# daxiongpro/EPNet

Hardware: AMD Instinct MI355X
Metric: SA-stack points/sec per GPU (16384-pt KITTI scene) + % HBM roofline (higher is better)
Workload: dtype f32; 1 GPU; 256 x 16384-pt kitti scenes per GPU per step through the 4-level SA op stack (4 samplings [FPS + centre gather; levels 2-4 nested in level 1 where tie-free] + 8 ball_query + 8 fused groupings [xyz - centre ; features]), pyramid 16384>4096>1024>256>64, radii [[.1,.5],[.5,1],[1,2],[2,4]], nsample [16,32], C=0/96/256/512, HIP-graph launch; levels=4, scenes_per_gpu=256, software_pipelined=True, pipeline_stages=2, parallelism=scene-parallel x1

## Files before the change

epnet_amd/_lib.py:

```python
import contextlib
import ctypes
import os

_HERE = os.path.dirname(os.path.abspath(__file__))
LIB_PATH = os.environ.get("EPNET_HIP_LIB") or os.path.join(_HERE, "lib", "libepnet_hip.so")

_vp = ctypes.c_void_p
_i = ctypes.c_int
_f = ctypes.c_float
_d = ctypes.c_double
_sz = ctypes.c_size_t
_i64 = ctypes.c_int64

SIGNATURES = {
    "epnet_abi_version": (_i, []),
    "epnet_strerror": (ctypes.c_char_p, [_i]),
    "epnet_last_hip_error": (ctypes.c_char_p, []),
    "epnet_set_tuning": (_i, [ctypes.c_char_p, _i]),
    "epnet_get_tuning": (_i, [ctypes.c_char_p, ctypes.POINTER(_i)]),
    "epnet_furthest_point_sampling": (_i, [_i, _i, _i, _vp, _vp, _vp, _vp]),
    "epnet_gather_points": (_i, [_i, _i, _i, _i, _vp, _vp, _vp, _vp]),
    "epnet_gather_points_grad": (_i, [_i, _i, _i, _i, _vp, _vp, _vp, _vp]),
    "epnet_ball_query": (_i, [_i, _i, _i, _f, _i, _vp, _vp, _vp, _vp]),
    "epnet_ball_query_workspace_bytes": (_sz, [_i, _i, _i]),
    "epnet_ball_query_ws": (_i, [_i, _i, _i, _f, _i, _vp, _vp, _vp, _vp, _sz, _vp]),
    "epnet_group_points": (_i, [_i, _i, _i, _i, _i, _vp, _vp, _vp, _vp]),
    "epnet_group_points_grad": (_i, [_i, _i, _i, _i, _i, _vp, _vp, _vp, _vp]),
    "epnet_group_concat": (_i, [_i, _i, _i, _i, _i, _vp, _vp, _vp, _vp, _vp, _i, _vp]),
    "epnet_group_concat_workspace_bytes": (_sz, [_i, _i, _i, _i, _i]),
    "epnet_group_concat_ws": (_i, [_i, _i, _i, _i, _i, _vp, _vp, _vp, _vp, _vp, _i, _vp, _sz, _vp]),
    "epnet_group_concat_grad": (_i, [_i, _i, _i, _i, _i, _vp, _vp, _vp, _i, _vp]),
    "epnet_group_points_grad_workspace_bytes": (_sz, [_i, _i, _i, _i]),
    "epnet_group_points_grad_ws": (_i, [_i, _i, _i, _i, _i, _vp, _vp, _vp, _vp, _sz, _vp]),
    "epnet_group_concat_grad_ws": (_i, [_i, _i, _i, _i, _i, _vp, _vp, _vp, _i, _vp, _sz, _vp]),
    "epnet_three_nn": (_i, [_i, _i, _i, _vp, _vp, _vp, _vp, _vp]),
    "epnet_three_nn_workspace_bytes": (_sz, [_i, _i, _i]),
    "epnet_three_nn_ws": (_i, [_i, _i, _i, _vp, _vp, _vp, _vp, _vp, _sz, _vp]),
    "epnet_three_interpolate": (_i, [_i, _i, _i, _i, _vp, _vp, _vp, _vp, _vp]),
    "epnet_three_interpolate_grad": (_i, [_i, _i, _i, _i, _vp, _vp, _vp, _vp, _vp]),
    "epnet_three_interpolate_grad_workspace_bytes": (_sz, [_i, _i, _i]),
    "epnet_three_interpolate_grad_ws": (_i, [_i, _i, _i, _i, _vp, _vp, _vp, _vp, _vp, _sz, _vp]),
    "epnet_group_linear": (_i, [_i, _i, _i, _i, _i, _vp, _vp, _vp, _vp, _vp, _vp, _vp, _vp]),
    "epnet_group_linear_grad_w": (_i, [_i, _i, _i, _i, _i, _vp, _vp, _vp, _vp, _vp, _vp]),
    "epnet_feature_gather": (_i, [_i, _i, _i, _i, _i, _i, _i, _vp, _vp, _vp, _vp, _vp, _vp]),
    "epnet_feature_gather_grad": (_i, [_i, _i, _i, _i, _i, _i, _vp, _vp, _vp, _vp]),
    "epnet_gather_points_grad_det_workspace_bytes": (_sz, [_i, _i, _i]),
    "epnet_gather_points_grad_det": (_i, [_i, _i, _i, _i, _vp, _vp, _vp, _vp, _sz, _vp]),
    "epnet_group_points_grad_det_workspace_bytes": (_sz, [_i, _i, _i, _i]),
    "epnet_group_points_grad_det": (_i, [_i, _i, _i, _i, _i, _vp, _vp, _vp, _vp, _sz, _vp]),
    "epnet_group_concat_grad_det_workspace_bytes": (_sz, [_i, _i, _i, _i]),
    "epnet_group_concat_grad_det": (_i, [_i, _i, _i, _i, _i, _vp, _vp, _vp, _i, _vp, _sz, _vp]),
    "epnet_three_interpolate_grad_det_workspace_bytes": (_sz, [_i, _i, _i]),
    "epnet_three_interpolate_grad_det": (_i, [_i, _i, _i, _i, _vp, _vp, _vp, _vp, _vp, _sz, _vp]),
    "epnet_feature_gather_grad_det_workspace_bytes": (_sz, [_i, _i, _i, _i]),
    "epnet_feature_gather_grad_det": (_i, [_i, _i, _i, _i, _i, _i, _vp, _vp, _vp, _vp, _sz, _vp]),
    "epnet_group_linear_grad_w_det_workspace_bytes": (_sz, [_i, _i, _i, _i]),
    "epnet_group_linear_grad_w_det": (_i, [_i, _i, _i, _i, _i, _vp, _vp, _vp, _vp, _vp, _vp, _sz, _vp]),
    "epnet_pool_max": (_i, [ctypes.c_longlong, _i, _vp, _vp, _vp, _vp]),
    "epnet_pool_max_grad": (_i, [ctypes.c_longlong, _i, _vp, _vp, _vp, _vp]),
    "epnet_group_linear_h": (_i, [_i, _i, _i, _i, _i, _vp, _vp, _vp, _vp, _vp, _vp, _vp, _i, _vp]),
    "epnet_pool_max_h": (_i, [ctypes.c_longlong, _i, _vp, _vp, _vp, _i, _vp]),
    "epnet_pool_max_grad_h": (_i, [ctypes.c_longlong, _i, _vp, _vp, _vp, _i, _vp]),
    "epnet_three_interpolate_h": (_i, [_i, _i, _i, _i, _vp, _vp, _vp, _vp, _i, _vp]),
    "epnet_scene_index_bytes": (_sz, [_i, _i]),
    "epnet_scene_index_build": (_i, [_i, _i, _vp, _vp, _sz, _vp]),
    "epnet_scene_index_build_gathered": (_i, [_i, _i, _i, _vp, _vp, _vp, _vp, _sz, _vp]),
    "epnet_furthest_point_sampling_indexed": (_i, [_i, _i, _i, _vp, _vp, _sz, _vp, _vp, _vp]),
    "epnet_sample_centres": (_i, [_i, _i, _i, _vp, _vp, _sz, _vp, _vp, _vp, _vp]),
    "epnet_sample_centres_chain": (_i, [_i, _i, _i, _vp, _vp, _sz, _vp, _vp, _vp, _vp, _vp, _i, _vp]),
    "epnet_group_concat_multi": (_i, [_i, _i, _i, _i, _i, _vp, _vp, _vp, _vp, _vp, _vp, _i, _vp]),
    "epnet_ball_query_indexed_multi": (_i, [_i, _i, _i, _i, _vp, _vp, _vp, _vp, _vp, _sz, _vp, _vp]),
    "epnet_ball_query_ordered": (_i, [_i, _i, _i, _i, _vp, _vp, _vp, _vp, _vp, _sz, _vp, _sz, _vp, _vp]),
    "epnet_three_nn_indexed": (_i, [_i, _i, _i, _vp, _vp, _vp, _sz, _vp, _sz, _vp, _vp, _vp]),
    "epnet_ball_query_indexed": (_i, [_i, _i, _i, _f, _i, _vp, _vp, _vp, _sz, _vp, _vp]),
    "epnet_boxes_overlap_bev": (_i, [_i, _vp, _i, _vp, _vp, _vp]),
    "epnet_boxes_iou_bev": (_i, [_i, _vp, _i, _vp, _vp, _vp]),
    "epnet_boxes_iou3d": (_i, [_i, _vp, _i, _vp, _vp, _vp]),
    "epnet_boxes_iou3d_pairs": (_i, [_i, _vp, _vp, _vp, _vp]),
    "epnet_aug_roi_by_noise": (_i, [_i, _i, _f, _vp, _vp, _vp, _vp, _vp, _vp, _vp, _vp]),
    "epnet_rcnn_sample_rois_workspace_bytes": (_sz, [_i, _i, _i, _i]),
    "epnet_rcnn_sample_rois": (_i, [_i, _i, _i, _i, _i, _i, _f, _f, _f, _d, _i, _vp, _vp, _vp, _vp, _vp, _vp, _vp, _sz, _vp, _vp, _vp,
                                    _vp, _vp, _vp, _vp, _vp, _vp, _vp]),
    "epnet_rpn_proposals_workspace_bytes": (_sz, [_i, _i, _i, _i]),
    "epnet_rpn_proposals": (_i, [_i, _i, _vp, _vp, _vp, _i, _i, _i, _f, _i, _vp, _sz, _vp, _vp, _vp, _vp]),
    "epnet_decode_bbox_target": (_i, [ctypes.c_longlong, _i, _vp, _vp, _i, _i, _i, _d, _d, _d, _d, _i, _vp, _i, _i, _i, _i, _i, _i, _vp, _vp]),
    "epnet_score_order": (_i, [_i, _i, _vp, _vp, _vp]),
    "epnet_rpn_handover_workspace_bytes": (_sz, [_i, _i, _i, _i, _i]),
    "epnet_rpn_handover": (_i, [_i, _i, _i, _vp, _vp, _vp, _i, _i, _d, _d, _d, _d, _i, _vp, _i, _i, _i, _i, _i, _f, _i, _i, _i, _f, _i, _vp,
                                _sz, _vp, _vp, _vp, _vp, _vp, _vp, _vp, _vp]),
    "epnet_rcnn_detections_workspace_bytes": (_sz, [_i, _i]),
    "epnet_rcnn_detections": (_i, [_i, _i, _vp, _vp, _vp, _f, _f, _vp, _sz, _vp, _vp, _vp, _vp]),
    "epnet_eval_recall_workspace_bytes": (_sz, [_i, _i, _i]),
    "epnet_eval_recall": (_i, [_i, _i, _i, _i, _i, _i, _vp, _vp, _vp, _vp, _vp, _vp, _vp, _sz, _vp, _vp, _vp, _vp, _vp, _vp, _vp]),
    "epnet_kitti_records": (_i, [_i, _i, _vp, _vp, _vp, _vp, _vp, _vp, _vp, _vp, _vp, _vp]),
    "epnet_nms_workspace_bytes": (_sz, [_i]),
    "epnet_nms": (_i, [_vp, _i, _f, _vp, _sz, _vp, _vp, _vp]),
    "epnet_nms_normal": (_i, [_vp, _i, _f, _vp, _sz, _vp, _vp, _vp]),
    "epnet_roipool3d_workspace_bytes": (_sz, [_i, _i, _i]),
    "epnet_roipool3d": (_i, [_i, _i, _i, _i, _i, _vp, _vp, _vp, _vp, _vp, _vp, _sz, _vp]),
    "epnet_roipool3d_canonical": (_i, [_i, _i, _i, _i, _i, _f, _vp, _vp, _vp, _vp, _vp, _vp]),
    "epnet_roipool3d_train": (_i, [_i, _i, _i, _i, _i, _f, _f, _f, _f, _vp, _vp, _vp, _vp, _vp, _vp, _vp, _vp, _vp, _vp, _vp, _vp, _vp,
                                   _vp, _vp]),
    "epnet_box_loss_workspace_bytes": (_sz, [ctypes.c_longlong, _i]),
    "epnet_box_loss": (_i, [ctypes.c_longlong, _i, _d, _d, _i, _i, _i, _i, _d, _d, _d, _d, _d, _d, _d, _vp, _vp, _vp, _vp, _vp, _vp, _vp,
                            _vp, _vp, _vp, _vp, _vp, _sz, _vp]),
    "epnet_adam_onecycle_workspace_bytes": (_sz, [ctypes.c_longlong]),
    "epnet_adam_onecycle_step": (_i, [_i, ctypes.c_longlong, ctypes.c_longlong, _vp, _vp, _vp, ctypes.c_longlong, _d, _d, _d, _i, _vp, _vp,
                                      _vp, _vp, _vp, _sz, _vp]),
    "epnet_rpn_targets": (_i, [_i, _i, _i, _f, _vp, _vp, _vp, _vp, _vp, _vp, _vp, _vp, _vp]),
    "epnet_scan_prepare_workspace_bytes": (_sz, [_i, _i, _i]),
    "epnet_scan_prepare": (_i, [_i, _i, _i, _i, _vp, _f, _vp, _vp, _vp, _vp, _vp, _vp, _vp, _vp, _vp, _sz, _vp, _vp, _vp, _vp, _vp, _vp, _vp]),
    "epnet_image_normalise": (_i, [_i, _i, _i, _i, _i, _vp, _vp, _vp, _vp, _vp, _vp]),
    "epnet_kitti_overlaps": (_i, [_i, _i, _i, _i, _i, _vp, _vp, _vp, _vp, _vp, _vp, _vp]),
    "epnet_kitti_match": (_i, [_i, _i, _i, _i, _i, _i, _i, _vp, _vp, _vp, _vp, _vp, _vp, _vp, _vp, _vp, _vp, _vp]),
    "epnet_kitti_pr_workspace_bytes": (_sz, [_i, _i, _i]),
    "epnet_kitti_pr": (_i, [_i, _i, _i, _i, _i, _i, _i, _i, _i, _i, _i, _vp, _vp, _vp, _vp, _vp, _vp, _vp, _vp, _vp, _vp, _vp, _vp,
                            _vp, _vp, _vp, _vp, _vp, _sz, _vp, _vp, _vp]),
    "epnet_kitti_thresholds_host": (_i, [_vp, _i64, _i64, _i, _vp, _i, ctypes.POINTER(_i)]),
    "epnet_pts_in_boxes3d_host": (_i, [_vp, _vp, _vp, _i64, _i64]),
    "epnet_roipool3d_host": (_i, [_vp, _vp, _vp, _vp, _vp, _vp, _i64, _i64, _i64, _i64]),
}

_lib = None


class EpnetError(RuntimeError):
    pass


def lib():
    global _lib
    if _lib is None:
        if not os.path.exists(LIB_PATH):
            raise RuntimeError(
                "epnet_amd: %s not found -- build it with `python -c 'import __graft_entry__ as g; g.build()'` "
                "or `make -C epnet_amd/csrc` (there is no CPU fallback)" % LIB_PATH)
        handle = ctypes.CDLL(LIB_PATH)
        for name, (res, args) in SIGNATURES.items():
            try:
                fn = getattr(handle, name)
            except AttributeError:
                raise RuntimeError("epnet_amd: %s does not export %s (stale build?)" % (LIB_PATH, name))
            fn.restype = res
            fn.argtypes = args
        if handle.epnet_abi_version() != 1:
            raise RuntimeError("epnet_amd: ABI version mismatch in %s" % LIB_PATH)
        _lib = handle
    return _lib


def check(code, what):
    if code != 0:
        l = lib()
        msg = l.epnet_strerror(code).decode()
        hip = l.epnet_last_hip_error().decode()
        raise EpnetError("%s failed: %s%s" % (what, msg, (" [" + hip + "]") if (code == -2 and hip) else ""))


@contextlib.contextmanager
def tuning(**overrides):
    l = lib()
    saved = []
    try:
        for name, value in overrides.items():
            old = _i()
            check(l.epnet_get_tuning(name.encode(), ctypes.byref(old)), "epnet_get_tuning(%s)" % name)
            check(l.epnet_set_tuning(name.encode(), int(value)), "epnet_set_tuning(%s, %r)" % (name, value))
            saved.append((name, old.value))
        yield
    finally:
        for name, old in reversed(saved):
            l.epnet_set_tuning(name.encode(), old)
```

epnet_amd/csrc/ball_query.hip:

```cpp

#include "common.h"
#include "dpp.h"
#include "spatial.h"

namespace epnet {

constexpr int kBqTile = 2048;
constexpr int kBqThreads = 256;

template <int CPW>
__global__ __launch_bounds__(kBqThreads) void ball_query_kernel(int n, int m, float radius2, int nsample,
                                                                const float *__restrict__ new_xyz,
                                                                const float *__restrict__ xyz,
                                                                int *__restrict__ idx) {
    __shared__ float tile[kBqTile * 3];
    const int lane = threadIdx.x & 63, wave = threadIdx.x >> 6;
    const int bs = blockIdx.y;
    xyz += (size_t)bs * n * 3;
    new_xyz += (size_t)bs * m * 3;
    idx += (size_t)bs * m * nsample;

    const int c0 = (blockIdx.x * (kBqThreads / 64) + wave) * CPW;
    float cx[CPW], cy[CPW], cz[CPW];
    int cnt[CPW], first[CPW];
#pragma unroll
    for (int i = 0; i < CPW; ++i) {
        const int ci = c0 + i;
        const bool ok = ci < m;
        cx[i] = ok ? new_xyz[ci * 3 + 0] : 0.f;
        cy[i] = ok ? new_xyz[ci * 3 + 1] : 0.f;
        cz[i] = ok ? new_xyz[ci * 3 + 2] : 0.f;
        cnt[i] = ok ? 0 : nsample;
        first[i] = 0;
    }

    for (int t0 = 0; t0 < n; t0 += kBqTile) {
        const int tn = min(kBqTile, n - t0);
        for (int e = threadIdx.x; e < tn * 3; e += kBqThreads) tile[e] = xyz[(size_t)t0 * 3 + e];
        __syncthreads();

        bool wave_done = true;
#pragma unroll
        for (int i = 0; i < CPW; ++i) wave_done = wave_done && (cnt[i] >= nsample);

        if (!wave_done) {
            for (int p0 = 0; p0 < tn; p0 += 64) {
                const int p = p0 + lane;
                const bool valid = p < tn;
                const float x = valid ? tile[p * 3 + 0] : 0.f;
                const float y = valid ? tile[p * 3 + 1] : 0.f;
                const float z = valid ? tile[p * 3 + 2] : 0.f;
                bool all_full = true;
#pragma unroll
                for (int i = 0; i < CPW; ++i) {
                    if (cnt[i] < nsample) {
                        const float dx = cx[i] - x, dy = cy[i] - y, dz = cz[i] - z;
                        const float d2 = dx * dx + dy * dy + dz * dz;
                        const bool hit = valid && (d2 < radius2);
                        const unsigned long long mask = __ballot(hit);
                        if (mask) {
                            const int pos = cnt[i] + popc_below(mask);
                            if (hit && pos < nsample) idx[(size_t)(c0 + i) * nsample + pos] = t0 + p;
                            if (cnt[i] == 0) first[i] = t0 + p0 + (int)__builtin_ctzll(mask);
                            cnt[i] += (int)__popcll(mask);
                        }
                        all_full = all_full && (cnt[i] >= nsample);
                    }
                }
                if (all_full) {
                    wave_done = true;
                    break;
                }
            }
        }
        if (__syncthreads_and(wave_done ? 1 : 0)) break;
    }

#pragma unroll
    for (int i = 0; i < CPW; ++i) {
        const int ci = c0 + i;
        if (ci < m && cnt[i] < nsample) {
            const int fill = cnt[i] > 0 ? first[i] : 0;
            for (int l = cnt[i] + lane; l < nsample; l += 64) idx[(size_t)ci * nsample + l] = fill;
        }
    }
}



#ifdef EPNET_BQ_STATS
__device__ unsigned long long g_bq_stats[16];
#endif
#ifdef EPNET_IX_STATS
__device__ unsigned long long g_ix_stats[8];
#define EPNET_IX_STAMP(var) const unsigned long long var = __builtin_amdgcn_s_memtime()
#else
#define EPNET_IX_STAMP(var)
#endif

template <int kIxThreads, int BITS>
__global__ __launch_bounds__(kIxThreads) void bq_index_kernel(int n, int np, const float *__restrict__ xyz,
                                                              float4 *__restrict__ sorted, float *__restrict__ boxes,
                                                              float *__restrict__ qboxes, int n_src = 0,
                                                              const int *__restrict__ src_idx = nullptr,
                                                              float *__restrict__ gathered = nullptr) {
    constexpr int kCells = 1 << BITS;
    extern __shared__ int s_hist[];
    __shared__ float s_box[6][16];
    __shared__ int s_part[16];
    const int q = threadIdx.x, lane = q & 63, wave = q >> 6;
    __builtin_amdgcn_s_setprio(3);
    xyz += (size_t)blockIdx.x * (src_idx ? n_src : n) * 3;
    if (src_idx) {
        src_idx += (size_t)blockIdx.x * n;
        gathered += (size_t)blockIdx.x * n * 3;
    }
    sorted += (size_t)blockIdx.x * np;
    boxes += (size_t)blockIdx.x * (np / 64) * 6;
    constexpr int per = kCells / kIxThreads;
    constexpr int per_shift = per == 16 ? 4 : per == 8 ? 3 : per == 4 ? 2 : -1;
    static_assert(per_shift > 0, "scan layout");
    constexpr int kIxPerThread = 16;
    const bool in_regs = n <= kIxThreads * kIxPerThread;
    float px[kIxPerThread], py[kIxPerThread], pz[kIxPerThread];
    float lo[3], ext[3];
    EPNET_IX_STAMP(t_0);
    if (in_regs) {
        float mn[3] = {3.4e38f, 3.4e38f, 3.4e38f}, mx[3] = {-3.4e38f, -3.4e38f, -3.4e38f};
        int row[kIxPerThread];
#pragma unroll
        for (int i = 0; i < kIxPerThread; ++i) {
            const int k = q + i * kIxThreads;
            const int kk = k < n ? k : 0;
            row[i] = src_idx ? src_idx[kk] : kk;
        }
#pragma unroll
        for (int i = 0; i < kIxPerThread; ++i) {
            px[i] = xyz[row[i] * 3 + 0];
            py[i] = xyz[row[i] * 3 + 1];
            pz[i] = xyz[row[i] * 3 + 2];
        }
        if (src_idx) {
#pragma unroll
            for (int i = 0; i < kIxPerThread; ++i) {
                const int k = q + i * kIxThreads;
                if (k < n) {
                    gathered[k * 3 + 0] = px[i];
                    gathered[k * 3 + 1] = py[i];
                    gathered[k * 3 + 2] = pz[i];
                }
            }
        }
#pragma unroll
        for (int i = 0; i < kIxPerThread; ++i) {
            const bool ok = q + i * kIxThreads < n;
            mn[0] = fminf(mn[0], ok ? px[i] : 3.4e38f); mx[0] = fmaxf(mx[0], ok ? px[i] : -3.4e38f);
            mn[1] = fminf(mn[1], ok ? py[i] : 3.4e38f); mx[1] = fmaxf(mx[1], ok ? py[i] : -3.4e38f);
            mn[2] = fminf(mn[2], ok ? pz[i] : 3.4e38f); mx[2] = fmaxf(mx[2], ok ? pz[i] : -3.4e38f);
        }
#pragma unroll
        for (int a = 0; a < 3; ++a) {
            const float l = wave_minf_all(mn[a]), h = wave_maxf_all(mx[a]);
            if (lane == 0) {
                s_box[a][wave] = l;
                s_box[3 + a][wave] = h;
            }
        }
        __syncthreads();
#pragma unroll
        for (int a = 0; a < 3; ++a) {
            float l = s_box[a][0], h = s_box[3 + a][0];
            for (int w = 1; w < kIxThreads / 64; ++w) {
                l = fminf(l, s_box[a][w]);
                h = fmaxf(h, s_box[3 + a][w]);
            }
            lo[a] = l;
            ext[a] = h - l;
        }
    } else {
        block_bbox3(xyz, n, s_box, lo, ext);
    }
    const CellGrid g = make_cell_grid(lo, ext, BITS);
    EPNET_IX_STAMP(t_1);
    for (int i = q; i < kCells + kCells / per + 64; i += kIxThreads) s_hist[i] = 0;
    __syncthreads();
    EPNET_IX_STAMP(t_2);
    int code[kIxPerThread], rank[kIxPerThread];
    if (in_regs) {
#pragma unroll
        for (int i = 0; i < kIxPerThread; ++i) code[i] = hist_at((int)cell_code(g, px[i], py[i], pz[i]), per_shift);
#pragma unroll
        for (int i = 0; i < kIxPerThread; ++i)
            rank[i] = atomicAdd(&s_hist[q + i * kIxThreads < n ? code[i] : kCells + kCells / per + lane], 1);
    } else {
        for (int k = q; k < n; k += kIxThreads)
            atomicAdd(&s_hist[hist_at((int)cell_code(g, xyz[k * 3 + 0], xyz[k * 3 + 1], xyz[k * 3 + 2]), per_shift)], 1);
    }
    __syncthreads();
    EPNET_IX_STAMP(t_3);
    int sum = 0;
    for (int i = 0; i < per; ++i) sum += s_hist[hist_at(q * per + i, per_shift)];
    const int incl = wave_inclusive_scan(sum);
    if (lane == 63) s_part[wave] = incl;
    __syncthreads();
    int base = incl - sum;
    for (int w = 0; w < wave; ++w) base += s_part[w];
    for (int i = 0; i < per; ++i) {
        const int at = hist_at(q * per + i, per_shift);
        const int c = s_hist[at];
        s_hist[at] = base;
        base += c;
    }
    __syncthreads();
    EPNET_IX_STAMP(t_4);
    auto bucket_box = [&](int p, const float4 v) {
        const bool real = p < n;
        const float cx_ = canonical(v.x), cy_ = canonical(v.y), cz_ = canonical(v.z);
        float mnx = real ? cx_ : 3.4e38f, mxx = real ? cx_ : -3.4e38f, mny = real ? cy_ : 3.4e38f, mxy = real ? cy_ : -3.4e38f,
              mnz = real ? cz_ : 3.4e38f, mxz = real ? cz_ : -3.4e38f;
        wave_box(mnx, mxx, mny, mxy, mnz, mxz);
        if (lane == 0) {
            float *bx = boxes + (p >> 6) * 6;
            const bool any = mnx <= mxx;
            bx[0] = any ? mnx : 3.0e38f; bx[1] = any ? mxx : 3.0e38f;
            bx[2] = any ? mny : 3.0e38f; bx[3] = any ? mxy : 3.0e38f;
            bx[4] = any ? mnz : 3.0e38f; bx[5] = any ? mxz : 3.0e38f;
        }
    };
    const bool staged = in_regs && (np & 255) == 0;
    if (staged) {
        float4 *s_stage = reinterpret_cast<float4 *>(s_hist + kCells + kCells / per + 64);
        int pos[kIxPerThread];
#pragma unroll
        for (int i = 0; i < kIxPerThread; ++i) pos[i] = s_hist[code[i]] + rank[i];
        const int quarter = kIxThreads == 256 ? min(np >> 2, 512) : np >> 2;
        for (int h = 0; h * quarter < np; ++h) {
            const int base = h * quarter, len = min(quarter, np - base);
            for (int p = q; p < len; p += kIxThreads)
                if (base + p >= n) s_stage[p] = make_float4(3.0e38f, 3.0e38f, 3.0e38f, __int_as_float(-1));
#pragma unroll
            for (int i = 0; i < kIxPerThread; ++i) {
                const int k = q + i * kIxThreads;
                if (k < n && (unsigned)(pos[i] - base) < (unsigned)quarter)
                    s_stage[pos[i] - base] = make_float4(px[i], py[i], pz[i], __int_as_float(k));
            }
            __syncthreads();
            for (int p = q; p < len; p += kIxThreads) {
                const float4 v = s_stage[p];
                sorted[base + p] = v;
                bucket_box(base + p, v);
            }
            __syncthreads();
        }
    } else {
        if (in_regs) {
#pragma unroll
            for (int i = 0; i < kIxPerThread; ++i) {
                const int k = q + i * kIxThreads;
                if (k < n) sorted[s_hist[code[i]] + rank[i]] = make_float4(px[i], py[i], pz[i], __int_as_float(k));
            }
        } else {
            for (int k = q; k < n; k += kIxThreads) {
                const float x = xyz[k * 3 + 0], y = xyz[k * 3 + 1], z = xyz[k * 3 + 2];
                const int pos = atomicAdd(&s_hist[hist_at((int)cell_code(g, x, y, z), per_shift)], 1);
                sorted[pos] = make_float4(x, y, z, __int_as_float(k));
            }
        }
        for (int p = n + q; p < np; p += kIxThreads)
            sorted[p] = make_float4(3.0e38f, 3.0e38f, 3.0e38f, __int_as_float(-1));
        __threadfence_block();
        __syncthreads();
        for (int p = q; p < np; p += kIxThreads) bucket_box(p, sorted[p]);
    }
#ifdef EPNET_IX_STATS
    {
        EPNET_IX_STAMP(t_6);
        if (q == 0) {
            atomicAdd(&g_ix_stats[0], t_1 - t_0); atomicAdd(&g_ix_stats[1], t_2 - t_1); atomicAdd(&g_ix_stats[2], t_3 - t_2);
            atomicAdd(&g_ix_stats[3], t_4 - t_3); atomicAdd(&g_ix_stats[4], t_6 - t_4);
            atomicAdd(&g_ix_stats[7], 1ull);
        }
    }
#endif
    if (!qboxes) return;
    qboxes += (size_t)blockIdx.x * (np / 256) * 6;
    __threadfence_block();
    __syncthreads();
    for (int g = q; g < np / 256; g += kIxThreads) {
        float mn[3] = {3.4e38f, 3.4e38f, 3.4e38f}, mx[3] = {-3.4e38f, -3.4e38f, -3.4e38f};
        for (int k = 0; k < 4; ++k) {
            const float *bx = boxes + (g * 4 + k) * 6;
            if (bx[0] < 3.0e38f)
#pragma unroll
                for (int a = 0; a < 3; ++a) {
                    mn[a] = fminf(mn[a], bx[2 * a]);
                    mx[a] = fmaxf(mx[a], bx[2 * a + 1]);
                }
        }
        const bool any = mn[0] <= mx[0];
#pragma unroll
        for (int a = 0; a < 3; ++a) {
            qboxes[g * 6 + 2 * a] = any ? mn[a] : 3.0e38f;
            qboxes[g * 6 + 2 * a + 1] = any ? mx[a] : 3.0e38f;
        }
    }
}

constexpr int kQThreads = 256;

__device__ __forceinline__ bool box_near(const float *__restrict__ bx, float cx, float cy, float cz, float radius2) {
    const float2 bxx = *reinterpret_cast<const float2 *>(bx), byy = *reinterpret_cast<const float2 *>(bx + 2),
                 bzz = *reinterpret_cast<const float2 *>(bx + 4);
    const float px = __builtin_amdgcn_fmed3f(cx, bxx.x, bxx.y), py = __builtin_amdgcn_fmed3f(cy, byy.x, byy.y),
                pz = __builtin_amdgcn_fmed3f(cz, bzz.x, bzz.y);
    const float dx = cx - px, dy = cy - py, dz = cz - pz;
    return (dx * dx + dy * dy + dz * dz) < radius2;
}


template <int DPL, typename F>
__device__ __forceinline__ void bq_walk(int lane, int np, float r2, float cx, float cy, float cz,
                                        const float4 *__restrict__ sorted, const float *__restrict__ boxes,
                                        const float *__restrict__ qboxes, int *quads, F &&visit) {
    auto scan_buckets = [&](unsigned long long cand, auto &&bucket_of) {
        while (cand) {
            float4 p[4];
            int nb = 0;
#pragma unroll
            for (int k = 0; k < 4; ++k)
                if (cand) {
                    const int bb = bucket_of((int)__builtin_ctzll(cand));
                    cand &= cand - 1ull;
                    p[k] = sorted[(bb << 6) + lane];
                    nb = k + 1;
                }
#pragma unroll
            for (int k = 0; k < 4; ++k)
                if (k < nb) {
                    const float dx = cx - p[k].x, dy = cy - p[k].y, dz = cz - p[k].z;
                    visit(p[k], dx * dx + dy * dy + dz * dz);
                }
        }
    };
    if constexpr (DPL <= 2) {
        const bool bnear = lane < (np >> 6) && box_near(boxes + lane * 6, cx, cy, cz, r2);
        scan_buckets(__ballot(bnear), [](int l) { return l; });
    } else {
        const int nq = np >> 8;
        for (int q0 = 0; q0 < nq; q0 += 64) {
            const int qd = q0 + lane;
            const bool qnear = qd < nq && box_near(qboxes + qd * 6, cx, cy, cz, r2);
            const unsigned long long qmask = __ballot(qnear);
            if (!qmask) continue;
            const int nqc = (int)__popcll(qmask);
            if (qnear) quads[popc_below(qmask)] = qd;
            __builtin_amdgcn_wave_barrier();
            for (int s0 = 0; s0 < nqc; s0 += 16) {
                const int slot = s0 + (lane >> 2);
                int bid = 0;
                bool bnear = false;
                if (slot < nqc) {
                    bid = quads[slot] * 4 + (lane & 3);
                    bnear = box_near(boxes + bid * 6, cx, cy, cz, r2);
                }
                scan_buckets(__ballot(bnear), [&](int l) { return __builtin_amdgcn_readlane(bid, l); });
            }
            __builtin_amdgcn_wave_barrier();
        }
    }
}

__device__ __forceinline__ void bq_emit_list(int lane, const int *hits, int cnt, int nsample, int *__restrict__ out) {
    __builtin_amdgcn_wave_barrier();
    const int mine = lane < cnt ? hits[lane] : 0x7fffffff;
    int rank = 0;
    for (int j = 0; j < cnt; ++j) rank += __builtin_amdgcn_readlane(mine, j) < mine ? 1 : 0;
    if (lane < cnt && rank < nsample) out[rank] = mine;
    int first = 0;
    if (cnt) first = __builtin_amdgcn_readlane(mine, (int)__builtin_ctzll(__ballot(lane < cnt && rank == 0)));
    for (int l = cnt + lane; l < nsample; l += 64) out[l] = first;
}


__device__ __forceinline__ void bq_emit_shared(int lane, const int *hits, int cnt, int ns_big, int ns_small, int *__restrict__ out_big,
                                               int *__restrict__ out_small) {
    __builtin_amdgcn_wave_barrier();
    const bool valid = lane < cnt;
    const int mine = valid ? hits[lane] : 0x7fffffff;
    int rank = 0, rin = 0;
    for (int j = 0; j < cnt; ++j) {
        const int v = __builtin_amdgcn_readlane(mine, j);
        rank += v < mine ? 1 : 0;
        rin += v < mine ? (v & 1) : 0;
    }
    const bool inner = valid && (mine & 1);
    if (valid && rank < ns_big) out_big[rank] = mine >> 1;
    if (inner && rin < ns_small) out_small[rin] = mine >> 1;
    int first = 0;
    if (cnt) first = __builtin_amdgcn_readlane(mine, (int)__builtin_ctzll(__ballot(valid && rank == 0))) >> 1;
    for (int l = cnt + lane; l < ns_big; l += 64) out_big[l] = first;
    const unsigned long long im = __ballot(inner);
    const int cin = (int)__popcll(im);
    first = 0;
    if (cin) first = __builtin_amdgcn_readlane(mine, (int)__builtin_ctzll(__ballot(inner && rin == 0))) >> 1;
    for (int l = cin + lane; l < ns_small; l += 64) out_small[l] = first;
}

template <int NS>
__device__ __forceinline__ void bq_store_rows(int lane, bool two, const int *ord, int c0, int c1, int ns_rt, int *__restrict__ row0,
                                              int *__restrict__ row1) {
    const int ns = NS ? NS : ns_rt;
    if (NS == 16 && lane >= 32) return;
    const int e = NS == 16 ? lane >> 4 : lane >> 5, s = NS == 16 ? lane & 15 : lane & 31;
    const int c = e ? c1 : c0;
    int v = ord[e * 32 + (s < c ? s : 0)];
    v = c ? v : 0;
    if (e == 0) {
        if (s < ns) row0[s] = v;
    } else if (two) {
        if (s < ns) row1[s] = v;
    }
    if (NS == 0 && ns > 32 && (e == 0 || two)) {
        int *row = e ? row1 : row0;
        const int first = c ? ord[e * 32] : 0;
        for (int l = s + 32; l < ns; l += 32) row[l] = first;
    }
}

template <int NSB, int NSS>
__device__ __forceinline__ void bq_emit_pair(int lane, bool two, int *lists, int c0, int c1, int ns_big, int ns_small,
                                             int *__restrict__ big0, int *__restrict__ big1, int *__restrict__ small0,
                                             int *__restrict__ small1) {
    const int half = lane >> 5, sl = lane & 31;
    const int c = half ? c1 : c0;
    int *raw = lists + half * 64;
    const bool valid = sl < c;
    __builtin_amdgcn_wave_barrier();
    int mine = raw[sl];
    if (!valid) {
        mine = 0x7fffffff;
        raw[sl] = mine;
    }
    __builtin_amdgcn_wave_barrier();
    int rank = 0, rin = 0;
    const int nmax = max(c0, c1);
#pragma unroll 1
    for (int j = 0; j < nmax; j += 4) {
        const int4 v = *reinterpret_cast<const int4 *>(raw + j);
        rank += (v.x < mine ? 1 : 0) + (v.y < mine ? 1 : 0) + (v.z < mine ? 1 : 0) + (v.w < mine ? 1 : 0);
        rin += (v.x < mine ? v.x & 1 : 0) + (v.y < mine ? v.y & 1 : 0) + (v.z < mine ? v.z & 1 : 0) + (v.w < mine ? v.w & 1 : 0);
    }
    const bool inner = valid && (mine & 1);
    if (valid) lists[128 + half * 32 + rank] = mine >> 1;
    if (inner) lists[192 + half * 32 + rin] = mine >> 1;
    const unsigned long long im = __ballot(inner);
    __builtin_amdgcn_wave_barrier();
    bq_store_rows<NSB>(lane, two, lists + 128, c0, c1, ns_big, big0, big1);
    bq_store_rows<NSS>(lane, two, lists + 192, (int)__popc((unsigned)im), (int)__popc((unsigned)(im >> 32)), ns_small, small0, small1);
// ... 140 lines not shown
        const int nwg = gx * (int)gridDim.y, orig = (int)blockIdx.y * gx + (int)blockIdx.x;
        const int xcd = orig & 7, qq = nwg >> 3, rr = nwg & 7;
        const int wgid = (xcd < rr ? xcd * (qq + 1) : rr * (qq + 1) + (xcd - rr) * qq) + (orig >> 3);
        bs = wgid >> __builtin_ctz(gx);
        wg_x = wgid & (gx - 1);
        return;
    }
#endif
    xcd_scene_map(wg_x, bs);
    wg_x = __builtin_amdgcn_readfirstlane(wg_x);
    bs = __builtin_amdgcn_readfirstlane(bs);
}

template <int DPL, int K, bool kStream, bool kSpec = false>
__global__ __launch_bounds__(kQThreads) void bq_query2_kernel(int np, int m, BqScales<K> sc,
                                                              const float *__restrict__ new_xyz,
                                                              const float4 *__restrict__ sorted,
                                                              const float *__restrict__ boxes,
                                                              const float *__restrict__ qboxes,
                                                              const float4 *__restrict__ order, int npc) {
    constexpr int kRowsPerStep = 2;
    constexpr int CAP = kStream ? (K == 1 ? 512 : 256) : 64, kStepAppends = kRowsPerStep * 64;
    static_assert(CAP % 64 == 0, "the lists are selected and emitted in whole waves");
    static_assert(!kStream || CAP - kStepAppends >= 64,
                  "a cut list keeps nsample <= 64 entries (the launcher streams for nsample <= 64 only) and must take a step's appends");
    constexpr int kBitWords = kStream ? 0 : 64 * DPL;
    constexpr bool kShared = K == 2 && !kStream;
    static_assert(!kSpec || kShared, "the compile-time pair is one of the shared-list kernel");
    __shared__ __attribute__((aligned(16))) unsigned s_pool[kQThreads / 64][kBitWords + 2 * K * CAP];
    __shared__ int s_quads[kQThreads / 64][2][64];
    const int lane = threadIdx.x & 63, wave = threadIdx.x >> 6;
    int wg_x, bs;
    xcd_scene_map_uniform(wg_x, bs);
    const int ci0 = (wg_x * (kQThreads / 64) + wave) * 2;
    if (ci0 >= m) return;
    const bool two = ci0 + 1 < m;
    sorted += (size_t)bs * np;
    boxes += (size_t)bs * (np / 64) * 6;
    qboxes += (size_t)bs * (np / 256) * 6;
    float ax, ay, az, bx_, by_, bz_;
    int out0 = ci0, out1 = ci0 + 1;
    if (order) {
        const float4 e0 = order[(size_t)bs * npc + ci0], e1 = order[(size_t)bs * npc + ci0 + (two ? 1 : 0)];
        ax = e0.x; ay = e0.y; az = e0.z;
        bx_ = e1.x; by_ = e1.y; bz_ = e1.z;
        out0 = __float_as_int(e0.w);
        out1 = __float_as_int(e1.w);
    } else {
        const float *c0 = new_xyz + ((size_t)bs * m + ci0) * 3;
        const float *c1 = two ? c0 + 3 : c0;
        ax = c0[0]; ay = c0[1]; az = c0[2];
        bx_ = c1[0]; by_ = c1[1]; bz_ = c1[2];
    }
    auto uniform = [](float v) { return __int_as_float(__builtin_amdgcn_readfirstlane(__float_as_int(v))); };
    ax = uniform(ax); ay = uniform(ay); az = uniform(az);
    bx_ = uniform(bx_); by_ = uniform(by_); bz_ = uniform(bz_);
    out0 = __builtin_amdgcn_readfirstlane(out0);
    out1 = __builtin_amdgcn_readfirstlane(out1);
    const int half = lane >> 5;
    const float hx = half ? bx_ : ax, hy = half ? by_ : ay, hz = half ? bz_ : az;
    float r2max = sc.r2[0];
#pragma unroll
    for (int k = 1; k < K; ++k) r2max = fmaxf(r2max, sc.r2[k]);
    const bool big1 = kSpec || (kShared && (sc.r2[K - 1] >= sc.r2[0] || sc.r2[0] != sc.r2[0]));
    const float r2small = kShared ? (big1 ? sc.r2[0] : sc.r2[K - 1]) : r2max;
    if constexpr (kShared) r2max = big1 ? sc.r2[K - 1] : sc.r2[0];
    int cnt[2][K];
    int below[2][K];
#pragma unroll
    for (int e = 0; e < 2; ++e)
#pragma unroll
        for (int k = 0; k < K; ++k) {
            cnt[e][k] = 0;
            below[e][k] = 0x7fffffff;
        }
    int *hits_of = reinterpret_cast<int *>(s_pool[wave]) + kBitWords;
#ifdef EPNET_BQ_STATS
    const unsigned long long st_0 = __builtin_amdgcn_s_memtime();
    unsigned st_rows = 0;
    bool st_sel = false, st_again = false;
#endif

    auto visit = [&](int e, const float4 &p) {
#ifdef EPNET_BQ_STATS
        ++st_rows;
#endif
        const float cx = e ? bx_ : ax, cy = e ? by_ : ay, cz = e ? bz_ : az;
        const float dx = cx - p.x, dy = cy - p.y, dz = cz - p.z;
        const float d2 = dx * dx + dy * dy + dz * dz;
        if constexpr (kShared) {
            const bool hit = d2 < r2max;
            const unsigned long long hm = __ballot(hit);
            if (!hm) return;
            const int pos = cnt[e][0] + popc_below(hm);
            if (hit && pos < 64) hits_of[e * 64 + pos] = (__float_as_int(p.w) << 1) | (d2 < r2small ? 1 : 0);
            cnt[e][0] += (int)__popcll(hm);
            return;
        }
        if (!__ballot(d2 < r2max)) return;
#pragma unroll
        for (int k = 0; k < K; ++k) {
            const bool hit = d2 < sc.r2[k] && (!kStream || __float_as_int(p.w) < below[e][k]);
            const unsigned long long hm = __ballot(hit);
            if (hm) {
                const int pos = cnt[e][k] + popc_below(hm);
                if (hit && pos < CAP) hits_of[(e * K + k) * CAP + pos] = __float_as_int(p.w);
                cnt[e][k] += (int)__popcll(hm);
            }
        }
    };
    auto make_room = [&]() {
        if constexpr (kStream) {
#pragma unroll
            for (int e = 0; e < 2; ++e)
#pragma unroll
                for (int k = 0; k < K; ++k)
                    if (cnt[e][k] > CAP - kStepAppends) {
                        below[e][k] = bq_select_smallest<CAP / 64>(lane, hits_of + (e * K + k) * CAP, cnt[e][k], sc.nsample[k], np);
                        cnt[e][k] = sc.nsample[k];
#ifdef EPNET_BQ_STATS
                        st_sel = true;
#endif
                    }
        }
    };
    auto row_of = [&](int bucket) { return (sorted + ((size_t)(unsigned)bucket << 6))[(unsigned)lane]; };
    auto scan_pairs = [&](unsigned long long cand0, unsigned long long cand1, auto &&bucket_of) {
        static_assert(kRowsPerStep == 2, "the step below loads two rows of each centre");
        while (cand0 | cand1) {
            make_room();
            float4 p0, p1, p2, p3;
            const bool h0 = cand0 != 0ull, h1 = cand1 != 0ull;
            if (h0) { p0 = row_of(bucket_of(0, (int)__builtin_ctzll(cand0))); cand0 &= cand0 - 1ull; }
            if (h1) { p1 = row_of(bucket_of(1, (int)__builtin_ctzll(cand1))); cand1 &= cand1 - 1ull; }
            const bool h2 = cand0 != 0ull, h3 = cand1 != 0ull;
            if (h2) { p2 = row_of(bucket_of(0, (int)__builtin_ctzll(cand0))); cand0 &= cand0 - 1ull; }
            if (h3) { p3 = row_of(bucket_of(1, (int)__builtin_ctzll(cand1))); cand1 &= cand1 - 1ull; }
            if (h0) visit(0, p0);
            if (h1) visit(1, p1);
            if (h2) visit(0, p2);
            if (h3) visit(1, p3);
            __builtin_amdgcn_s_waitcnt(0x0F70);
        }
    };
    if constexpr (DPL <= 2) {
        bool n0 = false, n1 = false;
        if (lane < (np >> 6)) {
            n0 = box_near(boxes + lane * 6, ax, ay, az, r2max);
            n1 = box_near(boxes + lane * 6, bx_, by_, bz_, r2max);
        }
        scan_pairs(__ballot(n0), __ballot(n1), [](int, int bit) { return bit; });
    } else {
        const int nq = np >> 8;
        for (int q0 = 0; q0 < nq; q0 += 64) {
            const int qd = q0 + lane;
            const float *qb = qboxes + __umul24(min(qd, nq - 1), 6);
            const bool n0 = box_near(qb, ax, ay, az, r2max) && qd < nq, n1 = box_near(qb, bx_, by_, bz_, r2max) && qd < nq;
            const unsigned long long qm0 = __builtin_amdgcn_ballot_w64(n0), qm1 = __builtin_amdgcn_ballot_w64(n1);
            if (!(qm0 | qm1)) continue;
            const int nq0 = (int)__popcll(qm0), nq1 = (int)__popcll(qm1);
            if (n0) s_quads[wave][0][popc_below(qm0)] = qd;
            if (n1) s_quads[wave][1][popc_below(qm1)] = qd;
            __builtin_amdgcn_wave_barrier();
            const int nmine = half ? nq1 : nq0;
            for (int s0 = 0; s0 < max(nq0, nq1); s0 += 8) {
                const int slot = s0 + ((lane & 31) >> 2);
                int bid = 0;
                bool bnear = false;
                if (slot < nmine) {
                    bid = s_quads[wave][half][slot] * 4 + (lane & 3);
                    bnear = box_near(boxes + __umul24(bid, 6), hx, hy, hz, r2max);
                }
                const unsigned long long cand = __builtin_amdgcn_ballot_w64(bnear);
                scan_pairs(cand & 0xFFFFFFFFull, cand >> 32,
                           [&](int e, int bit) { return __builtin_amdgcn_readlane(bid, bit + 32 * e); });
            }
            __builtin_amdgcn_wave_barrier();
        }
    }
#ifdef EPNET_BQ_STATS
    const unsigned long long st_1 = __builtin_amdgcn_s_memtime();
#endif
    if constexpr (kShared) {
        const int ns0 = kSpec ? 16 : sc.nsample[0], ns1 = kSpec ? 32 : sc.nsample[K - 1];
        const int ns_big = big1 ? ns1 : ns0, ns_small = big1 ? ns0 : ns1;
        int *idx_big = big1 ? sc.idx[K - 1] : sc.idx[0], *idx_small = big1 ? sc.idx[0] : sc.idx[K - 1];
        const size_t row0 = (size_t)bs * m + out0, row1 = (size_t)bs * m + out1;
        const int c0 = cnt[0][0], c1 = cnt[1][0];
        if (c0 <= 32 && c1 <= 32) {
            bq_emit_pair<kSpec ? 32 : 0, kSpec ? 16 : 0>(lane, two, hits_of, c0, c1, ns_big, ns_small, idx_big + row0 * ns_big,
                                                         idx_big + row1 * ns_big, idx_small + row0 * ns_small, idx_small + row1 * ns_small);
        } else {
#pragma unroll
            for (int e = 0; e < 2; ++e) {
                if (e == 1 && !two) break;
                const size_t row = e ? row1 : row0;
                if (cnt[e][0] <= 64) {
                    bq_emit_shared(lane, hits_of + e * 64, cnt[e][0], ns_big, ns_small, idx_big + row * ns_big, idx_small + row * ns_small);
                } else {
#ifdef EPNET_BQ_STATS
                    st_again = true;
#endif
                    const float cx = e ? bx_ : ax, cy = e ? by_ : ay, cz = e ? bz_ : az;
                    bq_bitmap_search<DPL>(lane, np, r2max, ns_big, cx, cy, cz, sorted, boxes, qboxes, idx_big + row * ns_big, s_pool[wave],
                                          s_quads[wave][0]);
                    bq_bitmap_search<DPL>(lane, np, r2small, ns_small, cx, cy, cz, sorted, boxes, qboxes, idx_small + row * ns_small,
                                          s_pool[wave], s_quads[wave][0]);
                }
            }
        }
    } else {
#pragma unroll
        for (int e = 0; e < 2; ++e) {
            if (e == 1 && !two) break;
            const float cx = e ? bx_ : ax, cy = e ? by_ : ay, cz = e ? bz_ : az;
#pragma unroll
            for (int k = 0; k < K; ++k) {
                int *out = sc.idx[k] + ((size_t)bs * m + (e ? out1 : out0)) * sc.nsample[k];
                int *hits = hits_of + (e * K + k) * CAP;
                if constexpr (kStream) {
                    if (cnt[e][k] > 64) {
                        bq_select_smallest<CAP / 64>(lane, hits, cnt[e][k], sc.nsample[k], np);
                        cnt[e][k] = sc.nsample[k];
#ifdef EPNET_BQ_STATS
                        st_sel = true;
#endif
                    }
                    bq_emit_list(lane, hits, cnt[e][k], sc.nsample[k], out);
                } else {
                    if (cnt[e][k] <= 64) {
                        bq_emit_list(lane, hits, cnt[e][k], sc.nsample[k], out);
                    } else {
#ifdef EPNET_BQ_STATS
                        st_again = true;
#endif
                        bq_bitmap_search<DPL>(lane, np, sc.r2[k], sc.nsample[k], cx, cy, cz, sorted, boxes, qboxes, out, s_pool[wave],
                                              s_quads[wave][0]);
                    }
                }
            }
        }
    }
#ifdef EPNET_BQ_STATS
    {
        const unsigned long long st_3 = __builtin_amdgcn_s_memtime();
        if (lane == 0) {
            const int o = st_again ? 8 : (st_sel ? 4 : 0);
            atomicAdd(&g_bq_stats[o + 0], 1ull);
            atomicAdd(&g_bq_stats[o + 1], st_1 - st_0);
            atomicAdd(&g_bq_stats[o + 2], st_3 - st_1);
            atomicAdd(&g_bq_stats[o + 3], (unsigned long long)st_rows);
            atomicMax(&g_bq_stats[12], st_3 - st_0);
        }
    }
#endif
}

}

using namespace epnet;

extern "C" int epnet_ball_query(int b, int n, int m, float radius, int nsample, const float *new_xyz,
                                const float *xyz, int *idx, epnet_stream_t stream) {
    EPNET_REQUIRE(b >= 0 && n >= 0 && m >= 0 && nsample >= 0);
    if (b == 0 || m == 0 || nsample == 0) return EPNET_OK;
    EPNET_REQUIRE(new_xyz && xyz && idx);
    EPNET_REQUIRE(b <= 65535);
    const float radius2 = radius * radius;
    hipStream_t s = (hipStream_t)stream;
    constexpr int waves = kBqThreads / 64;
    if ((long long)m * b >= 8192) {
        dim3 grid(div_up(m, waves * 2), b);
        hipLaunchKernelGGL(ball_query_kernel<2>, grid, dim3(kBqThreads), 0, s, n, m, radius2, nsample, new_xyz, xyz, idx);
    } else {
        dim3 grid(div_up(m, waves), b);
        hipLaunchKernelGGL(ball_query_kernel<1>, grid, dim3(kBqThreads), 0, s, n, m, radius2, nsample, new_xyz, xyz, idx);
    }
    return check_launch("ball_query");
}


int epnet::spatial_index_launch(int b, int n, int np, const float *xyz, float4 *sorted, float *boxes, float *qboxes,
                                hipStream_t s, int n_src, const int *src_idx, float *gathered) {
    if (n <= 4096) {
        constexpr int T = 256, cells = 1 << 12;
        const size_t stage = (np & 255) == 0 ? (size_t)(np / 4 < 512 ? np / 4 : 512) * sizeof(float4) : 0;
        hipLaunchKernelGGL((bq_index_kernel<T, 12>), dim3(b), dim3(T), (size_t)(cells + cells / (cells / T) + 64) * sizeof(int) + stage, s,
                           n, np, xyz, sorted, boxes, qboxes, n_src, src_idx, gathered);
    } else {
        constexpr int T = 1024, cells = 1 << 14;
        const size_t stage = (n <= T * 16 && (np & 255) == 0) ? (size_t)(np / 4) * sizeof(float4) : 0;
        hipLaunchKernelGGL((bq_index_kernel<T, 14>), dim3(b), dim3(T), (size_t)(cells + cells / (cells / T) + 64) * sizeof(int) + stage, s,
                           n, np, xyz, sorted, boxes, qboxes, n_src, src_idx, gathered);
    }
    return check_launch("spatial index");
}

template <int K>
static int bq_query_launch(int b, int np, int m, const BqScales<K> &sc, const float *new_xyz, const float4 *sorted,
                           hipStream_t s, const float4 *order = nullptr, int npc = 0) {
    const float *boxes = (const float *)(sorted + (size_t)b * np);
    const float *qboxes = boxes + (size_t)b * (np / 64) * 6;
    const int pair_force = tuning(kBqPair);
    const bool pair = pair_force >= 0 ? pair_force != 0 : (long long)b * m >= 65536;
    if (pair) {
        dim3 grid(div_up(div_up(m, 2), kQThreads / 64), b);
        const int stream_force = tuning(kBqStream);
        bool stream = stream_force >= 0 ? stream_force != 0 : np > 16384;
        for (int k = 0; k < K; ++k) stream = stream && sc.nsample[k] <= 64;
        const bool spec = K == 2 && !stream && sc.nsample[0] == 16 && sc.nsample[K - 1] == 32 && sc.r2[0] <= sc.r2[K - 1];
#define EPNET_BQ2(D_)                                                                                                                   \
    do {                                                                                                                                \
        if (stream)                                                                                                                     \
            hipLaunchKernelGGL((bq_query2_kernel<D_, K, true>), grid, dim3(kQThreads), 0, s, np, m, sc, new_xyz, sorted, boxes, qboxes,   \
                               order, npc);                                                                                             \
        else if (spec)                                                                                                                  \
            hipLaunchKernelGGL((bq_query2_kernel<D_, K, false, K == 2>), grid, dim3(kQThreads), 0, s, np, m, sc, new_xyz, sorted, boxes, \
                               qboxes, order, npc);                                                                                     \
        else                                                                                                                            \
            hipLaunchKernelGGL((bq_query2_kernel<D_, K, false>), grid, dim3(kQThreads), 0, s, np, m, sc, new_xyz, sorted, boxes,         \
                               qboxes, order, npc);                                                                                     \
    } while (0)
        switch (np / 2048) {
            case 1: EPNET_BQ2(1); break;
            case 2: EPNET_BQ2(2); break;
            case 4: EPNET_BQ2(4); break;
// ... 155 lines not shown
```

epnet_amd/csrc/fps.hip:

```cpp
#include <math.h>

#include <type_traits>

#include "common.h"
#include "dpp.h"
#include "spatial.h"

extern "C" __device__ int epnet_llvm_writelane_i32(int, int, int) __asm("llvm.amdgcn.writelane.i32");

namespace epnet {

__device__ __forceinline__ int writelane_i32(int value, int lane, int old) {
    return epnet_llvm_writelane_i32(value, lane, old);
}

__device__ __forceinline__ unsigned bitrev_lg(unsigned v, int lg) {
    return lg == 0 ? 0u : (__brev(v) >> (32 - lg));
}

__device__ __forceinline__ int wave_max_i32(int v) {
    const int r = row16_max(v);
    const int a = __builtin_amdgcn_readlane(r, 0), b = __builtin_amdgcn_readlane(r, 16);
    const int c = __builtin_amdgcn_readlane(r, 32), d = __builtin_amdgcn_readlane(r, 48);
    return max(max(a, b), max(c, d));
// ... 134 lines not shown
        int slot;
        float sx, sy, sz;
        find_slot<PPT>(t, x, y, z, g, wl, wbest, slot, sx, sy, sz);
        const int code = ((wave * 64 + wl) << 8) | slot;
        if constexpr (W == 1) {
            x1 = sx;
            y1 = sy;
            z1 = sz;
            s_idx[it & (kIdxBuf - 1)] = code;
        } else {
            const int buf = it & 1;
            if (lane == 0) {
                s_val[buf][wave] = wbest;
                s_rec[buf][wave] = make_float4(sx, sy, sz, __int_as_float(code));
            }
            __syncthreads();
            const int wv = s_val[buf][lane & 15];
            const float4 rec = s_rec[buf][lane & 15];
            const int bm = row16_max(wv);
            const unsigned long long wtied = __ballot(wv == bm) & 0xFFFFull;
            const int ww = (int)__builtin_ctzll(wtied);
            x1 = __int_as_float(__builtin_amdgcn_readlane(__float_as_int(rec.x), ww));
            y1 = __int_as_float(__builtin_amdgcn_readlane(__float_as_int(rec.y), ww));
            z1 = __int_as_float(__builtin_amdgcn_readlane(__float_as_int(rec.z), ww));
            const int wcode = __builtin_amdgcn_readlane(__float_as_int(rec.w), ww);
            if (wave == 0) s_idx[it & (kIdxBuf - 1)] = wcode;
        }
        if ((it & (kIdxBuf - 1)) == kIdxBuf - 1 && wave == 0) {
            const int base = it - (kIdxBuf - 1);
            for (int e = lane; e < kIdxBuf; e += 64) {
                const int c = s_idx[e];
                const int k = fps_point_of(c >> 8, c & 0xFF, R, J, lg_bs);
                idxs[base + e] = k;
                if (new_xyz) {
                    float *dst = new_xyz + (size_t)(base + e) * 3;
                    dst[0] = xyz[k * 3 + 0];
                    dst[1] = xyz[k * 3 + 1];
                    dst[2] = xyz[k * 3 + 2];
                }
            }
        }
    }
    if (wave == 0) {
        const int base = (m - 1) & ~(kIdxBuf - 1);
        for (int e = lane; base + e < m; e += 64) {
            const int c = s_idx[e];
            const int k = fps_point_of(c >> 8, c & 0xFF, R, J, lg_bs);
            idxs[base + e] = k;
            if (new_xyz) {
                float *dst = new_xyz + (size_t)(base + e) * 3;
                dst[0] = xyz[k * 3 + 0];
                dst[1] = xyz[k * 3 + 1];
                dst[2] = xyz[k * 3 + 2];
            }
        }
    }
    if (temp) {
#pragma unroll
        for (int s = 0; s < PPT; ++s) {
            const int k = s < used ? fps_point_of(q, s, R, J, lg_bs) : n;
            if (k < n) temp[k] = __int_as_float(t[s]);
        }
    }
}

namespace pruned {

#ifndef EPNET_FPS_PRIO
#define EPNET_FPS_PRIO 3
#endif

#ifdef EPNET_FPS_STATS
__device__ unsigned long long g_stats[16];
#define EPNET_STAMP(var) const unsigned long long var = __builtin_amdgcn_s_memtime()
#define EPNET_ACC(slot, a, b) st_acc[slot] += (unsigned long long)((b) - (a))
#define EPNET_CNT(slot, v) st_acc[slot] += (unsigned long long)(v)
#define EPNET_STATS_BEGIN unsigned long long st_acc[8] = {0, 0, 0, 0, 0, 0, 0, 0}
#define EPNET_STATS_END if ((threadIdx.x & 63) == 0) for (int s_ = 0; s_ < 8; ++s_) atomicAdd(&g_stats[s_], st_acc[s_])
#else
#define EPNET_STAMP(var)
#define EPNET_ACC(slot, a, b)
#define EPNET_CNT(slot, v)
#define EPNET_STATS_BEGIN
#define EPNET_STATS_END
#endif

__device__ __forceinline__ unsigned rank14(int k) { return (bitrev_lg((unsigned)k & 1023u, 10) << 4) | ((unsigned)k >> 10); }
__device__ __forceinline__ int unrank14(unsigned r) { return (int)(bitrev_lg(r >> 4, 10) + ((r & 15u) << 10)); }

template <int G>
__device__ __forceinline__ int group_max(int v) {
    v = max(v, dpp_i32<0xB1>(v));
    v = max(v, dpp_i32<0x4E>(v));
    v = max(v, dpp_i32<0x141>(v));
    if (G >= 16) v = max(v, dpp_i32<0x140>(v));
    if (G >= 32) {
        const auto a = __builtin_amdgcn_permlane16_swap((unsigned)v, (unsigned)v, false, false);
        v = max((int)a[0], (int)a[1]);
    }
    return v;
}
template <int G>
__device__ __forceinline__ float group_minf(float v) {
    v = fminf(v, __int_as_float(dpp_i32<0xB1>(__float_as_int(v))));
    v = fminf(v, __int_as_float(dpp_i32<0x4E>(__float_as_int(v))));
    v = fminf(v, __int_as_float(dpp_i32<0x141>(__float_as_int(v))));
    if (G >= 16) v = fminf(v, __int_as_float(dpp_i32<0x140>(__float_as_int(v))));
    if (G >= 32) {
        const auto a = __builtin_amdgcn_permlane16_swap(__float_as_uint(v), __float_as_uint(v), false, false);
        v = fminf(__uint_as_float(a[0]), __uint_as_float(a[1]));
    }
    return v;
}
template <int G>
__device__ __forceinline__ float group_maxf(float v) { return -group_minf<G>(-v); }

template <int P>
__device__ __forceinline__ int period_max(int v) {
    if (P > 1) v = max(v, dpp_i32<0xB1>(v));
    if (P > 2) v = max(v, dpp_i32<0x4E>(v));
    if (P > 4) v = max(v, dpp_i32<0x124>(v));
    if (P > 8) v = max(v, dpp_i32<0x128>(v));
    return v;
}
template <int P>
__device__ __forceinline__ unsigned period_min(unsigned v) {
    if (P > 1) v = min(v, dpp_u32<0xB1>(v));
    if (P > 2) v = min(v, dpp_u32<0x4E>(v));
    if (P > 4) v = min(v, dpp_u32<0x124>(v));
    if (P > 8) v = min(v, dpp_u32<0x128>(v));
    return v;
}

template <int PPT>
__device__ __forceinline__ unsigned fold_parts(unsigned long long a) {
    if (PPT <= 32) a |= a >> 32;
    if (PPT <= 16) a |= a >> 16;
    if (PPT <= 8) a |= a >> 8;
    return (unsigned)a & (PPT >= 32 ? 0xFFFFFFFFu : ((1u << PPT) - 1u));
}

constexpr int kIdxBufP = 1024;

template <typename VH>
__device__ __forceinline__ unsigned rank_of(const VH &rk2, int j) {
    return ((unsigned)rk2[j >> 1] >> ((j & 1) << 4)) & 0xFFFFu;
}
template <typename VH>
__device__ __forceinline__ void set_rank(VH &rk2, int j, unsigned r) {
    rk2[j >> 1] = (j & 1) ? (int)(((unsigned)rk2[j >> 1] & 0xFFFFu) | (r << 16)) : (int)r;
}

template <int kW, int PPT, typename VF, typename VI, typename VH>
__device__ __forceinline__ void fps_rounds(int m, const VF &x, const VF &y, const VF &z, VI &t, const VH &rk2,
                                           float cx, float cy, float cz, int *__restrict__ idxs,
                                           int *__restrict__ tie_free = nullptr, int known = 0,
                                           const float *__restrict__ xyz_in_order = nullptr, int detect_upto = 0x7fffffff) {
    __shared__ unsigned long long s_key[3];
    __shared__ float4 s_rec[2][64 * kW];
    __shared__ int s_idx[kIdxBufP];
    const int q = threadIdx.x;
    const int lane = q & 63, wave = q >> 6;
    const int sub = lane & (PPT - 1);
    const int kNeg1 = __float_as_int(-1.f);

    int bm = kNeg1;
    float lox = 0.f, hix = 0.f, loy = 0.f, hiy = 0.f, loz = 0.f, hiz = 0.f;
    for (int j = 0; j < PPT; ++j) {
        const float xj = x[j], yj = y[j], zj = z[j];
        const int tj = t[j];
        const bool real = tj != kNeg1;
        const float mnx = group_minf<PPT>(real ? xj : 3.4e38f), mxx = group_maxf<PPT>(real ? xj : -3.4e38f);
        const float mny = group_minf<PPT>(real ? yj : 3.4e38f), mxy = group_maxf<PPT>(real ? yj : -3.4e38f);
        const float mnz = group_minf<PPT>(real ? zj : 3.4e38f), mxz = group_maxf<PPT>(real ? zj : -3.4e38f);
        const int gm = group_max<PPT>(tj);
        if (sub == j) {
            const bool any = gm != kNeg1;
            bm = gm;
            lox = any ? mnx : 0.f; hix = any ? mxx : 0.f;
            loy = any ? mny : 0.f; hiy = any ? mxy : 0.f;
            loz = any ? mnz : 0.f; hiz = any ? mxz : 0.f;
        }
    }
    if (q < 3) s_key[q] = 0ull;
    if (q == 0) s_idx[0] = 0;
    if (known > kIdxBufP || known > m || !xyz_in_order) known = 0;
    for (int i = q; i < known; i += 64 * kW) s_idx[i] = (int)rank14(i);
    __syncthreads();
    for (int it = 1; it < known; ++it) {
        const float px = __builtin_amdgcn_fmed3f(cx, lox, hix), py = __builtin_amdgcn_fmed3f(cy, loy, hiy),
                    pz = __builtin_amdgcn_fmed3f(cz, loz, hiz);
        const float bdx = px - cx, bdy = py - cy, bdz = pz - cz;
        const float L = bdx * bdx + bdy * bdy + bdz * bdz;
        unsigned active = fold_parts<PPT>(__ballot(__float_as_int(L) < bm));
        const float nx = xyz_in_order[it * 3 + 0], ny = xyz_in_order[it * 3 + 1], nz = xyz_in_order[it * 3 + 2];
        while (active) {
            const int j = (int)__builtin_ctz(active);
            active &= active - 1u;
            const float xj = x[j], yj = y[j], zj = z[j];
            const int told = t[j];
            __builtin_amdgcn_sched_barrier(0);
            const float dx = xj - cx, dy = yj - cy, dz = zj - cz;
            const float d = dx * dx + dy * dy + dz * dz;
            const int tj = min(__float_as_int(d), told);
            t[j] = tj;
            const int gm = group_max<PPT>(tj);
            bm = (sub == j) ? gm : bm;
        }
        cx = nx;
        cy = ny;
        cz = nz;
    }

    __builtin_amdgcn_s_setprio(EPNET_FPS_PRIO);
    EPNET_STATS_BEGIN;
    EPNET_STAMP(t_loop0);
    bool stale = true;
    int wbest = kNeg1;
    unsigned long long hbuckets = 0ull;
    unsigned racc = 0xFFFFFFFFu;
    float xa = 0.f, ya = 0.f, za = 0.f;
    int kb = 1;
    bool wave_multi = false;
    int tied_v = 0x7fffffff;
    auto round = [&](auto ties_tag, const int it) __attribute__((always_inline)) {
        constexpr bool kTies = decltype(ties_tag)::value;
        EPNET_STAMP(t0);
        const float px = __builtin_amdgcn_fmed3f(cx, lox, hix), py = __builtin_amdgcn_fmed3f(cy, loy, hiy),
                    pz = __builtin_amdgcn_fmed3f(cz, loz, hiz);
        const float bdx = px - cx, bdy = py - cy, bdz = pz - cz;
        const float L = bdx * bdx + bdy * bdy + bdz * bdz;
        const unsigned long long act64 = __ballot(__float_as_int(L) < bm);
        unsigned active = fold_parts<PPT>(act64);
        EPNET_CNT(0, __popc(active));
        stale = stale || __ballot((hbuckets & act64) != 0ull) != 0ull;
        EPNET_STAMP(t1);
        while (active) {
            const int j = (int)__builtin_ctz(active);
            active &= active - 1u;
            const float xj = x[j], yj = y[j], zj = z[j];
            const int told = t[j];
            __builtin_amdgcn_sched_barrier(0);
            const float dx = xj - cx, dy = yj - cy, dz = zj - cz;
            const float d = dx * dx + dy * dy + dz * dz;
            const int tj = min(__float_as_int(d), told);
            t[j] = tj;
            const int gm = group_max<PPT>(tj);
            bm = (sub == j) ? gm : bm;
        }
        EPNET_STAMP(t2);
        if (stale) {
            stale = false;
            wbest = wave_max_all(bm);
            unsigned cand = fold_parts<PPT>(__ballot(bm == wbest));
            racc = 0xFFFFFFFFu;
            hbuckets = 0ull;
            do {
                const int j = (int)__builtin_ctz(cand);
                cand &= cand - 1u;
                const int tj = t[j];
                const float xj = x[j], yj = y[j], zj = z[j];
                const unsigned rw = (unsigned)rk2[j >> 1];
                __builtin_amdgcn_sched_barrier(0);
                const unsigned r = tj == wbest ? ((rw >> ((j & 1) << 4)) & 0xFFFFu) : 0xFFFFFFFFu;
                if (r != 0xFFFFFFFFu) hbuckets |= 1ull << ((lane & ~(PPT - 1)) | j);
                const bool take = r < racc;
                racc = take ? r : racc;
                xa = take ? xj : xa;
                ya = take ? yj : ya;
                za = take ? zj : za;
            } while (cand);
            if (wbest == kNeg1) {
                racc = 0xFFFFFFFFu;
                hbuckets = 0ull;
            }
            if (kTies) {
                const unsigned long long holders = __ballot(hbuckets != 0ull);
                wave_multi = (holders & (holders - 1ull)) != 0ull || __ballot((hbuckets & (hbuckets - 1ull)) != 0ull) != 0ull;
            }
        }
        const int buf = it & 1;
        if (racc != 0xFFFFFFFFu) {
            s_rec[buf][q] = make_float4(xa, ya, za, 0.f);
            const unsigned long long key =
                ((unsigned long long)(unsigned)wbest << 32) | (unsigned long long)(((0x3FFFu - racc) << 10) | (unsigned)q);
            __hip_atomic_fetch_max(&s_key[kb], key, __ATOMIC_RELAXED, __HIP_MEMORY_SCOPE_WORKGROUP);
        }
        EPNET_STAMP(t3);
        __syncthreads();
        EPNET_STAMP(t4);
        const unsigned long long kfull = s_key[kb];
        const unsigned klo = (unsigned)kfull;
        const float4 rec = s_rec[buf][klo & 1023u];
        cx = rec.x;
        cy = rec.y;
        cz = rec.z;
        if (kTies) {
            const bool mine = (int)((klo & 1023u) >> 6) == wave;
            const int wd = (int)(unsigned)(kfull >> 32);
            const bool suspect = (wbest == wd && (!mine || wave_multi)) || wd == 0;
            if (__builtin_amdgcn_readfirstlane(suspect ? 1 : 0)) {
                bool differs = false;
                const unsigned mine_slots = (unsigned)((hbuckets >> (lane & ~(PPT - 1))) & ((1ull << PPT) - 1ull));
                unsigned any_slots = mine_slots;
                for (int off = 32; off >= 1; off >>= 1) any_slots |= (unsigned)__shfl_xor((int)any_slots, off, 64);
#pragma unroll 1
                while (any_slots) {
                    const int j = (int)__builtin_ctz(any_slots);
                    any_slots &= any_slots - 1u;
                    const float xj = x[j], yj = y[j], zj = z[j];
                    __builtin_amdgcn_sched_barrier(0);
                    differs = differs || (((mine_slots >> j) & 1u) && (xj != cx || yj != cy || zj != cz));
                }
                if (wd == 0 || __ballot(differs)) tied_v = min(tied_v, it);
            }
        }
        const int kb2 = kb == 0 ? 2 : kb - 1;
        kb = kb == 2 ? 0 : kb + 1;
        if (wave == 0) {
            s_idx[it & (kIdxBufP - 1)] = (int)(0x3FFFu - (klo >> 10));
            if (lane == 0) s_key[kb2] = 0ull;
            if ((it & (kIdxBufP - 1)) == kIdxBufP - 1) {
                const int base = it - (kIdxBufP - 1);
                for (int e = lane; e < kIdxBufP; e += 64) idxs[base + e] = unrank14((unsigned)s_idx[e]);
            }
        }
        EPNET_STAMP(t5);
        EPNET_ACC(1, t0, t1); EPNET_ACC(2, t1, t2); EPNET_ACC(3, t2, t3); EPNET_ACC(4, t3, t4); EPNET_ACC(5, t4, t5);
    };
    int it0 = max(1, known);
    if (tie_free) {
        const int upto = min(m, detect_upto);
        for (; it0 < upto; ++it0) round(std::true_type{}, it0);
    }
    for (; it0 < m; ++it0) round(std::false_type{}, it0);
    EPNET_STAMP(t_loop1);
    EPNET_ACC(6, t_loop0, t_loop1);
    EPNET_STATS_END;
    if (tie_free && lane == 0) atomicMin(tie_free, min(min(tied_v, m), detect_upto));
    if (wave == 0) {
        const int base = (m - 1) & ~(kIdxBufP - 1);
        for (int e = lane; base + e < m; e += 64) idxs[base + e] = unrank14((unsigned)s_idx[e]);
    }
}

template <int kW, int PPT>
__global__ __launch_bounds__(64 * kW) void fps_pruned_kernel(int n, int m, const float *__restrict__ xyz,
                                                             float *__restrict__ temp, int *__restrict__ idxs,
                                                             const int *__restrict__ skip, int *__restrict__ prefix_out,
                                                             int prefix_cap) {
    if (skip && skip[blockIdx.x] >= m) return;
    typedef float vecf __attribute__((ext_vector_type(PPT)));
    typedef int veci __attribute__((ext_vector_type(PPT)));
    constexpr int kT = 64 * kW;
    extern __shared__ int s_dyn[];
    int *hist = s_dyn;
    unsigned short *perm = reinterpret_cast<unsigned short *>(s_dyn + kCells + kCells / (kCells / kT) + 64);
    __shared__ int s_part[16];
    __shared__ float s_box[6][16];
    const int q = threadIdx.x;
    const int lane = q & 63, wave = q >> 6;
    xyz += (size_t)blockIdx.x * n * 3;
    if (temp) temp += (size_t)blockIdx.x * n;
    idxs += (size_t)blockIdx.x * m;

    float lo[3], ext[3];
    block_bbox3(xyz, n, s_box, lo, ext);
    const CellGrid grid = make_cell_grid(lo, ext);
    cell_sort_lds(xyz, n, grid, hist, s_part, perm);

    veci kk;
#pragma unroll
    for (int j = 0; j < PPT; ++j) {
        const int p = ((j * kW + wave) << 6) | lane;
        kk[j] = p < n ? (int)perm[p] : -1;
    }
    typedef int vech __attribute__((ext_vector_type(PPT / 2)));
    vecf x, y, z;
    veci t;
    vech rk2;
#pragma unroll
    for (int j = 0; j < PPT; ++j) {
        const int k = kk[j];
        if (k >= 0) {
            x[j] = xyz[k * 3 + 0];
            y[j] = xyz[k * 3 + 1];
            z[j] = xyz[k * 3 + 2];
            t[j] = __float_as_int(temp ? temp[k] : 1e10f);
            set_rank(rk2, j, rank14(k));
        } else {
            x[j] = y[j] = z[j] = 0.f;
            t[j] = __float_as_int(-1.f);
            set_rank(rk2, j, 0xFFFFu);
        }
    }
    fps_rounds<kW, PPT>(m, x, y, z, t, rk2, xyz[0], xyz[1], xyz[2], idxs, prefix_out ? prefix_out + blockIdx.x : nullptr, 0,
                        nullptr, prefix_cap);
    if (temp) {
#pragma unroll
        for (int j = 0; j < PPT; ++j) {
            const unsigned r = rank_of(rk2, j);
            if (r != 0xFFFFu) temp[unrank14(r)] = __int_as_float(t[j]);
        }
    }
}

template <int kW, int PPT>
__global__ __launch_bounds__(64 * kW) void fps_indexed_kernel(int n, int m, const float4 *__restrict__ sorted,
                                                              float *__restrict__ temp, int *__restrict__ idxs,
                                                              const int *__restrict__ prefix_in,
                                                              int *__restrict__ prefix_out, const float *__restrict__ xyz,
                                                              int prefix_cap, int prologue_init) {
    typedef float vecf __attribute__((ext_vector_type(PPT)));
    typedef int veci __attribute__((ext_vector_type(PPT)));
    constexpr int NP = 64 * kW * PPT;
    __shared__ float s_first[4];
    const int q = threadIdx.x;
    const int lane = q & 63, wave = q >> 6;
    const int known = prefix_in ? prefix_in[blockIdx.x] : 0;
    if (fps_prologue(m, prefix_in, idxs + (size_t)blockIdx.x * m, prefix_out, prologue_init)) return;
    sorted += (size_t)blockIdx.x * NP;
    if (temp) temp += (size_t)blockIdx.x * n;
    idxs += (size_t)blockIdx.x * m;
    typedef int vech __attribute__((ext_vector_type(PPT / 2)));
    vecf x, y, z;
    veci t;
    vech rk2;
#pragma unroll
    for (int j = 0; j < PPT; ++j) {
        const float4 v = sorted[((j * kW + wave) << 6) | lane];
        const int k = __float_as_int(v.w);
        if (k >= 0) {
            x[j] = v.x;
            y[j] = v.y;
            z[j] = v.z;
            t[j] = __float_as_int(temp ? temp[k] : 1e10f);
            set_rank(rk2, j, rank14(k));
            if (k == 0) {
                s_first[0] = v.x;
                s_first[1] = v.y;
                s_first[2] = v.z;
            }
        } else {
            x[j] = y[j] = z[j] = 0.f;
            t[j] = __float_as_int(-1.f);
            set_rank(rk2, j, 0xFFFFu);
        }
    }
    __syncthreads();
    fps_rounds<kW, PPT>(m, x, y, z, t, rk2, s_first[0], s_first[1], s_first[2], idxs, prefix_out ? prefix_out + blockIdx.x : nullptr,
                        known, xyz ? xyz + (size_t)blockIdx.x * n * 3 : nullptr, prefix_cap);
    if (temp) {
#pragma unroll
        for (int j = 0; j < PPT; ++j) {
            const unsigned r = rank_of(rk2, j);
            if (r != 0xFFFFu) temp[unrank14(r)] = __int_as_float(t[j]);
        }
    }
}

__device__ __forceinline__ unsigned rank16(int k) { return (bitrev_lg((unsigned)k & 1023u, 10) << 6) | ((unsigned)k >> 10); }
__device__ __forceinline__ int unrank16(unsigned r) { return (int)(bitrev_lg(r >> 6, 10) + ((r & 63u) << 10)); }

template <int kW>
__global__ __launch_bounds__(64 * kW) void fps_bigscene_kernel(int n, int np, int m, const float *__restrict__ xyz,
                                                               const float4 *__restrict__ sorted,
                                                               const float *__restrict__ boxes,
                                                               float *__restrict__ temp, float *__restrict__ tsort,
                                                               int *__restrict__ idxs, const int *__restrict__ skip) {
    if (skip && skip[blockIdx.x] >= m) return;
    constexpr int kT = 64 * kW;
    constexpr int kBPL = 1024 / kT;
    constexpr int kLgW = kW == 16 ? 4 : (kW == 8 ? 3 : 2);
    static_assert(kW == 4 || kW == 8 || kW == 16, "bucket dealing assumes 4, 8 or 16 waves");
    __shared__ unsigned long long s_key[3];
    __shared__ float4 s_rec[2][kW];
    __shared__ int s_idx[kIdxBufP];
    const int q = threadIdx.x;
    const int lane = q & 63, wave = q >> 6;
    const int nb = np >> 6;
    xyz += (size_t)blockIdx.x * n * 3;
    sorted += (size_t)blockIdx.x * np;
    boxes += (size_t)blockIdx.x * nb * 6;
    temp += (size_t)blockIdx.x * n;
    tsort += (size_t)blockIdx.x * np;
    idxs += (size_t)blockIdx.x * m;
    const int kNeg1 = __float_as_int(-1.f);
    auto bid = [&](int e) { return (e << kLgW) | wave; };

    float lox[kBPL], hix[kBPL], loy[kBPL], hiy[kBPL], loz[kBPL], hiz[kBPL];
    bool own[kBPL];
    int bm[kBPL];
    unsigned brank[kBPL];
    float bxx[kBPL], byy[kBPL], bzz[kBPL];
#pragma unroll
    for (int s_ = 0; s_ < kBPL; ++s_) {
        const int b_ = bid(s_ * 64 + lane);
        own[s_] = b_ < nb;
        lox[s_] = hix[s_] = loy[s_] = hiy[s_] = loz[s_] = hiz[s_] = 0.f;
        if (own[s_]) {
            const float *bx = boxes + b_ * 6;
            lox[s_] = bx[0]; hix[s_] = bx[1]; loy[s_] = bx[2]; hiy[s_] = bx[3]; loz[s_] = bx[4]; hiz[s_] = bx[5];
        }
        bm[s_] = kNeg1;
        brank[s_] = 0xFFFFu;
        bxx[s_] = byy[s_] = bzz[s_] = 0.f;
    }
    const int nmine = 64 * kBPL;

    for (int e = 0; e < nmine; ++e) {
        const int pos = (bid(e) << 6) + lane;
        if (pos < n) tsort[pos] = temp[__float_as_int(sorted[pos].w)];
    }

    struct Row {
        float4 p;
        int t;
    };
    auto load_row = [&](int e) {
        Row r;
        const int pos = (bid(e) << 6) + lane;
        r.p = sorted[pos];
        r.t = pos < n ? __float_as_int(tsort[pos]) : kNeg1;
        return r;
    };
    auto finish = [&](int e, Row r, bool update, float cx, float cy, float cz) {
        const int pos = (bid(e) << 6) + lane;
        const int k = __float_as_int(r.p.w);
        const bool real = pos < n;
        int t = r.t;
        if (real && update) {
            const float dx = r.p.x - cx, dy = r.p.y - cy, dz = r.p.z - cz;
            const float d = dx * dx + dy * dy + dz * dz;
            const int tn = min(__float_as_int(d), t);
            if (tn != t) tsort[pos] = __int_as_float(tn);
            t = tn;
        }
        const int mx = wave_max_all(t);
        const unsigned rk = (t == mx && real) ? rank16(k) : 0xFFFFFFFFu;
        unsigned long long holders = __ballot(rk != 0xFFFFFFFFu);
        unsigned rwin = 0xFFFFu;
        int wl = 0;
        if (holders) {
            if (holders & (holders - 1ull)) holders = __ballot(rk == wave_min_all(rk));
            wl = (int)__builtin_ctzll(holders);
            rwin = (unsigned)__builtin_amdgcn_readlane((int)rk, wl);
        }
        const float wx = __int_as_float(__builtin_amdgcn_readlane(__float_as_int(r.p.x), wl));
        const float wy = __int_as_float(__builtin_amdgcn_readlane(__float_as_int(r.p.y), wl));
        const float wz = __int_as_float(__builtin_amdgcn_readlane(__float_as_int(r.p.z), wl));
        const bool mine = lane == (e & 63);
        const int slot = e >> 6;
#pragma unroll
        for (int s_ = 0; s_ < kBPL; ++s_)
            if (mine && s_ == slot) {
                bm[s_] = mx;
                brank[s_] = rwin;
                bxx[s_] = wx; byy[s_] = wy; bzz[s_] = wz;
            }
    };

    for (int e = 0; e < nmine; ++e)
        if (bid(e) < nb) finish(e, load_row(e), false, 0.f, 0.f, 0.f);
    if (q < 3) s_key[q] = 0ull;
    if (q == 0) s_idx[0] = 0;
    float cx = xyz[0], cy = xyz[1], cz = xyz[2];
    __syncthreads();

    __builtin_amdgcn_s_setprio(EPNET_FPS_PRIO);
    bool stale = true;
    int wbest = kNeg1;
    bool publisher = false;
    unsigned pub_rank = 0xFFFFu;
    float pub_x = 0.f, pub_y = 0.f, pub_z = 0.f;
    int kb = 1;
    for (int it = 1; it < m; ++it) {
        unsigned long long active[kBPL];
        bool any = false;
#pragma unroll
        for (int s_ = 0; s_ < kBPL; ++s_) {
            const float px = __builtin_amdgcn_fmed3f(cx, lox[s_], hix[s_]), py = __builtin_amdgcn_fmed3f(cy, loy[s_], hiy[s_]),
                        pz = __builtin_amdgcn_fmed3f(cz, loz[s_], hiz[s_]);
            const float bdx = px - cx, bdy = py - cy, bdz = pz - cz;
            const float L = bdx * bdx + bdy * bdy + bdz * bdz;
            active[s_] = __ballot(own[s_] && __float_as_int(L) < bm[s_]);
            any = any || active[s_] != 0ull;
        }
        stale = stale || any;
#pragma unroll
        for (int s_ = 0; s_ < kBPL; ++s_) {
            unsigned long long act = active[s_];
            while (act) {
                const int e0 = s_ * 64 + (int)__builtin_ctzll(act);
                act &= act - 1ull;
                const bool two = act != 0ull;
                const int e1 = two ? s_ * 64 + (int)__builtin_ctzll(act) : e0;
                act &= act - 1ull;
                const Row r0 = load_row(e0);
                Row r1 = r0;
                if (two) r1 = load_row(e1);
                finish(e0, r0, true, cx, cy, cz);
                if (two) finish(e1, r1, true, cx, cy, cz);
            }
        }
        if (stale) {
            stale = false;
            int lmax = bm[0];
#pragma unroll
            for (int s_ = 1; s_ < kBPL; ++s_) lmax = max(lmax, bm[s_]);
// ... 120 lines not shown

static int ref_block_lg(int work_size) {
    int pow_2 = (int)(std::log(static_cast<double>(work_size)) / std::log(2.0));
    if (pow_2 > 10) pow_2 = 10;
    if (pow_2 < 0) pow_2 = 0;
    return pow_2;
}

}

using namespace epnet;

__global__ void fps_prefix_kernel(int m, const int *__restrict__ skip, int *__restrict__ idx, int *__restrict__ prefix_out, int init);

static bool fps_prune_applies(int n, int m) {
    return tuning(kFpsPrune) != 0 && n > 1024 && n > tuning(kFpsPruneMin) && n <= 16384 && m > 1;
}

static int fps_plain(int b, int n, int m, const float *xyz, float *temp, int *idx, const int *skip, int *prefix_out,
                     epnet_stream_t stream, int prefix_cap = 0x7fffffff, int prologue_init = -1, float *new_xyz = nullptr,
                     bool *wrote_centres = nullptr) {
    if (wrote_centres) *wrote_centres = false;
    EPNET_REQUIRE(b >= 0 && n >= 1 && m >= 0);
    if (b == 0 || m == 0) return EPNET_OK;
    EPNET_REQUIRE(xyz && idx);
    if ((long long)n > (1ll << 20) * 1024) return EPNET_ELIMIT;
    hipStream_t s = (hipStream_t)stream;
    const int lg = ref_block_lg(n);
    const int bs_ref = 1 << lg;
    dim3 grid(b);
    const int J = div_up(n, bs_ref);
    auto prefix_first = [&]() -> int {
        if (prologue_init < 0) return EPNET_OK;
        hipLaunchKernelGGL(fps_prefix_kernel, dim3(b), dim3(256), 0, s, m, skip, idx, prefix_out, prologue_init);
        return check_launch("sampling prefix");
    };
    if (fps_prune_applies(n, m)) {
        if (int rc = prefix_first()) return rc;
        int waves = n > 8192 ? 8 : 4;
        const int w = tuning(kFpsPwaves);
        if (w > 0 && div_up(n, 64 * w) <= 32) waves = w;
        const int ppt_need = div_up(n, 64 * waves);
        const int ppt = ppt_need <= 8 ? 8 : ppt_need <= 16 ? 16 : 32;
        const size_t lds = (size_t)(kCells + kCells / (kCells / (64 * waves)) + 64) * sizeof(int) + (size_t)64 * waves * ppt * 2;
#define EPNET_FPS_PRUNED(W_, P_) \
    hipLaunchKernelGGL((pruned::fps_pruned_kernel<W_, P_>), grid, dim3(64 * W_), lds, s, n, m, xyz, temp, idx, skip, prefix_out, prefix_cap)
        if (waves == 8) {
            if (ppt == 8) EPNET_FPS_PRUNED(8, 8);
            else if (ppt == 16) EPNET_FPS_PRUNED(8, 16);
            else EPNET_FPS_PRUNED(8, 32);
        } else {
            if (ppt == 8) EPNET_FPS_PRUNED(4, 8);
            else if (ppt == 16) EPNET_FPS_PRUNED(4, 16);
            else EPNET_FPS_PRUNED(4, 32);
        }
#undef EPNET_FPS_PRUNED
        return check_launch("furthest_point_sampling");
    }
    if (bs_ref >= 64 && J <= 16) {
        int waves = bs_ref / 64;
        for (int w = 1; w <= bs_ref / 64; w *= 2)
            if ((bs_ref / (64 * w)) * J <= 16) {
                waves = w;
                break;
            }
        if (n > 512 && b <= 512 && bs_ref / 64 >= 8 && waves < 8) waves = 8;
        const int w = tuning(kFpsWaves);
        if (w >= 1 && w <= bs_ref / 64 && (bs_ref / (64 * w)) * J <= 16) waves = w;
        const int ppt = (bs_ref / (64 * waves)) * J;
#define EPNET_FPS_LAUNCH(W_, P_) \
    hipLaunchKernelGGL((fps_wave_kernel<W_, P_>), grid, dim3(64 * W_), 0, s, n, m, lg, xyz, temp, idx, skip, prefix_out, prologue_init, \
                       new_xyz)
#define EPNET_FPS_PPT(W_)                      \
    do {                                       \
        if (ppt <= 1) EPNET_FPS_LAUNCH(W_, 1); \
        else if (ppt <= 2) EPNET_FPS_LAUNCH(W_, 2); \
        else if (ppt <= 4) EPNET_FPS_LAUNCH(W_, 4); \
        else if (ppt <= 8) EPNET_FPS_LAUNCH(W_, 8); \
        else EPNET_FPS_LAUNCH(W_, 16);         \
    } while (0)
        switch (waves) {
            case 1: EPNET_FPS_PPT(1); break;
            case 2: EPNET_FPS_PPT(2); break;
            case 4: EPNET_FPS_PPT(4); break;
            case 8: EPNET_FPS_PPT(8); break;
            default: EPNET_FPS_PPT(16); break;
        }
#undef EPNET_FPS_PPT
#undef EPNET_FPS_LAUNCH
        if (wrote_centres) *wrote_centres = new_xyz != nullptr;
        return check_launch("furthest_point_sampling");
    }
    float *tbuf = temp;
    if (!tbuf) return EPNET_EINVAL;
    if (int rc = prefix_first()) return rc;
    const int bs = bs_ref < 64 ? 64 : bs_ref;
    hipLaunchKernelGGL(fps_stream_kernel, grid, dim3(bs), 0, s, n, m, lg, xyz, tbuf, idx, skip);
    return check_launch("furthest_point_sampling");
}

extern "C" int epnet_furthest_point_sampling(int b, int n, int m, const float *xyz, float *temp, int *idx,
                                             epnet_stream_t stream) {
    return fps_plain(b, n, m, xyz, temp, idx, nullptr, nullptr, stream, 0x7fffffff);
}

static bool fps_detects_ties(int n, int m, bool indexed) {
    if (indexed) return m > 1 && n > 1024 && n <= 16384;
    return fps_prune_applies(n, m);
}

__global__ __launch_bounds__(256) void fps_prefix_kernel(int m, const int *__restrict__ skip, int *__restrict__ idx,
                                                         int *__restrict__ prefix_out, int init) {
    const int bs = blockIdx.x;
    const int have = skip ? skip[bs] : 0;
    const bool known = have >= m;
    if (threadIdx.x == 0 && prefix_out) prefix_out[bs] = known ? have : init;
    for (int i = threadIdx.x; i < min(have, m); i += 256) idx[(size_t)bs * m + i] = i;
}

__global__ __launch_bounds__(256) void gather_centres_kernel(int n, int m, const float *__restrict__ xyz,
                                                             const int *__restrict__ idx, float *__restrict__ out) {
    const int bs = blockIdx.y;
    const int e = blockIdx.x * 256 + threadIdx.x;
    if (e >= m * 3) return;
    const int i = e / 3, a = e - i * 3;
    out[(size_t)bs * m * 3 + e] = xyz[((size_t)bs * n + idx[(size_t)bs * m + i]) * 3 + a];
}

__global__ __launch_bounds__(256) void gather_centres4_kernel(int n, int m, const float *__restrict__ xyz,
                                                              const int *__restrict__ idx, float *__restrict__ out) {
    const int bs = blockIdx.y;
    const int i4 = blockIdx.x * 256 + threadIdx.x;
    if (i4 * 4 >= m) return;
    const int4 ids = reinterpret_cast<const int4 *>(idx + (size_t)bs * m)[i4];
    const float *src = xyz + (size_t)bs * n * 3;
    const float *p0 = src + (size_t)ids.x * 3, *p1 = src + (size_t)ids.y * 3, *p2 = src + (size_t)ids.z * 3, *p3 = src + (size_t)ids.w * 3;
    const float a0 = p0[0], a1 = p0[1], a2 = p0[2], b0 = p1[0], b1 = p1[1], b2 = p1[2];
    const float c0 = p2[0], c1 = p2[1], c2 = p2[2], d0 = p3[0], d1 = p3[1], d2 = p3[2];
    float4 *dst = reinterpret_cast<float4 *>(out + ((size_t)bs * m + (size_t)i4 * 4) * 3);
    dst[0] = make_float4(a0, a1, a2, b0);
    dst[1] = make_float4(b1, b2, c0, c1);
    dst[2] = make_float4(c2, d0, d1, d2);
}

static void launch_gather_centres(int b, int n, int m, const float *xyz, const int *idx, float *new_xyz, hipStream_t s) {
    if ((m & 3) == 0 && (((uintptr_t)idx | (uintptr_t)new_xyz) & 15) == 0)
        hipLaunchKernelGGL(gather_centres4_kernel, dim3(div_up(m / 4, 256), b), dim3(256), 0, s, n, m, xyz, idx, new_xyz);
    else
        hipLaunchKernelGGL(gather_centres_kernel, dim3(div_up(m * 3, 256), b), dim3(256), 0, s, n, m, xyz, idx, new_xyz);
}

static int fps_over_index(int b, int n, int m, const float *xyz, void *index, size_t index_bytes, float *temp, int *idx,
                          float *new_xyz, hipStream_t s, const int *skip = nullptr, int *prefix_out = nullptr,
                          int prefix_cap = 0x7fffffff) {
    const size_t need = scene_index_bytes(b, n);
    int rc;
    const bool plain = need == 0 || !index || n <= 1024 || m <= 1 || (n > 16384 && !temp);
    int fold_init = -1;
    bool wrote_centres = false;
    if (skip || prefix_out) {
        EPNET_REQUIRE(idx && b <= 65535);
        if (prefix_cap < 1) prefix_cap = 0x7fffffff;
        fold_init = fps_detects_ties(n, m, !plain) ? m : 0;
    }
    if (fold_init >= 0 && m == 0) {
        hipLaunchKernelGGL(fps_prefix_kernel, dim3(b), dim3(256), 0, s, m, skip, idx, prefix_out, fold_init);
        return check_launch("sampling prefix");
    }
    if (plain) {
        rc = fps_plain(b, n, m, xyz, temp, idx, skip, prefix_out, (epnet_stream_t)s, prefix_cap, fold_init, new_xyz, &wrote_centres);
    } else {
        EPNET_REQUIRE(idx);
        if (index_bytes < need) return EPNET_ENOMEM;
        const float4 *sorted = (const float4 *)index;
        dim3 grid(b);
        if (n > 16384) {
            EPNET_REQUIRE(xyz);
            if (fold_init >= 0) {
                hipLaunchKernelGGL(fps_prefix_kernel, dim3(b), dim3(256), 0, s, m, skip, idx, prefix_out, fold_init);
                rc = check_launch("sampling prefix");
                if (rc) return rc;
            }
            const int np = scene_index_np(n);
            const float *bucket_boxes = (const float *)(sorted + (size_t)b * np);
            float *tsort = scene_index_sampling_scratch(b, n, index);
            hipLaunchKernelGGL(pruned::fps_bigscene_kernel<16>, grid, dim3(1024), 0, s, n, np, m, xyz, sorted, bucket_boxes, temp, tsort, idx, skip);
        } else {
#define EPNET_FPS_INDEXED(W_, P_)                                                                                                     \
    hipLaunchKernelGGL((pruned::fps_indexed_kernel<W_, P_>), grid, dim3(64 * W_), 0, s, n, m, sorted, temp, idx, skip, prefix_out, xyz, \
                       prefix_cap, fold_init)
            switch (scene_index_np(n)) {
                case 2048: EPNET_FPS_INDEXED(4, 8); break;
                case 4096: EPNET_FPS_INDEXED(4, 16); break;
                case 8192: EPNET_FPS_INDEXED(4, 32); break;
                default: EPNET_FPS_INDEXED(8, 32); break;
            }
#undef EPNET_FPS_INDEXED
        }
        rc = check_launch("furthest_point_sampling");
    }
    if (rc || !new_xyz || wrote_centres) return rc;
    if (m == 0) return EPNET_OK;
    EPNET_REQUIRE(xyz && b <= 65535);
    launch_gather_centres(b, n, m, xyz, idx, new_xyz, s);
    return check_launch("sample_centres gather");
}

extern "C" int epnet_furthest_point_sampling_indexed(int b, int n, int m, const float *xyz, void *index,
                                                     size_t index_bytes, float *temp, int *idx,
                                                     epnet_stream_t stream) {
    return fps_over_index(b, n, m, xyz, index, index_bytes, temp, idx, nullptr, (hipStream_t)stream);
}

extern "C" int epnet_sample_centres(int b, int n, int m, const float *xyz, void *index, size_t index_bytes,
                                    float *temp, int *idx, float *new_xyz, epnet_stream_t stream) {
    EPNET_REQUIRE(b >= 0 && n >= 1 && m >= 0);
    if (b == 0 || m == 0) return EPNET_OK;
    EPNET_REQUIRE(xyz && idx && new_xyz);
    return fps_over_index(b, n, m, xyz, index, index_bytes, temp, idx, new_xyz, (hipStream_t)stream);
}

extern "C" int epnet_sample_centres_chain(int b, int n, int m, const float *xyz, void *index, size_t index_bytes,
                                          float *temp, int *idx, float *new_xyz, const int *prefix_in, int *prefix_out,
                                          int prefix_cap, epnet_stream_t stream) {
    EPNET_REQUIRE(b >= 0 && n >= 1 && m >= 0);
    if (b == 0 || m == 0) return EPNET_OK;
    EPNET_REQUIRE(xyz && idx);
    if (m > n) prefix_in = nullptr;
    return fps_over_index(b, n, m, xyz, index, index_bytes, temp, idx, new_xyz, (hipStream_t)stream, prefix_in, prefix_out,
                          prefix_cap);
}
```

epnet_amd/csrc/spatial.h:

```cpp
#pragma once
#include "common.h"

namespace epnet {

__device__ __forceinline__ unsigned spread10(unsigned v) {
    v &= 0x3FFu;
    v = (v | (v << 16)) & 0x030000FFu;
    v = (v | (v << 8)) & 0x0300F00Fu;
    v = (v | (v << 4)) & 0x030C30C3u;
    v = (v | (v << 2)) & 0x09249249u;
    return v;
}

__device__ __forceinline__ unsigned morton30(float px, float py, float pz, const float (&lo)[3], float scale) {
    const unsigned ix = (unsigned)fminf((px - lo[0]) * scale, 1023.f);
    const unsigned iy = (unsigned)fminf((py - lo[1]) * scale, 1023.f);
    const unsigned iz = (unsigned)fminf((pz - lo[2]) * scale, 1023.f);
    return spread10(ix) | (spread10(iy) << 1) | (spread10(iz) << 2);
}

__device__ __forceinline__ void bitonic_sort_lds(unsigned long long *keys, int np) {
    const int q = threadIdx.x, T = blockDim.x;
    for (int k2 = 2; k2 <= np; k2 <<= 1)
        for (int j2 = k2 >> 1; j2 > 0; j2 >>= 1) {
            for (int i = q; i < np / 2; i += T) {
                const int a = ((i & ~(j2 - 1)) << 1) | (i & (j2 - 1));
                const int b = a | j2;
                const unsigned long long ka = keys[a], kb = keys[b];
                const bool up = (a & k2) == 0;
                if ((ka > kb) == up) {
                    keys[a] = kb;
                    keys[b] = ka;
                }
            }
            __syncthreads();
        }
}

__device__ __forceinline__ int wave_inclusive_scan(int v) {
    v += __builtin_amdgcn_update_dpp(0, v, 0x111, 0xF, 0xF, true);
    v += __builtin_amdgcn_update_dpp(0, v, 0x112, 0xF, 0xF, true);
    v += __builtin_amdgcn_update_dpp(0, v, 0x114, 0xF, 0xF, true);
    v += __builtin_amdgcn_update_dpp(0, v, 0x118, 0xF, 0xF, true);
    v += __builtin_amdgcn_update_dpp(0, v, 0x142, 0xA, 0xF, true);
    v += __builtin_amdgcn_update_dpp(0, v, 0x143, 0xC, 0xF, true);
    return v;
}

__device__ __forceinline__ void block_bbox3(const float *__restrict__ xyz, int n, float (*s_box)[16], float (&lo)[3],
                                            float (&ext)[3]) {
    const int q = threadIdx.x, T = blockDim.x, lane = q & 63, wave = q >> 6, nw = T >> 6;
    float hi[3] = {-3.4e38f, -3.4e38f, -3.4e38f};
    lo[0] = lo[1] = lo[2] = 3.4e38f;
    for (int k = q; k < n; k += T)
#pragma unroll
        for (int a = 0; a < 3; ++a) {
            const float v = xyz[k * 3 + a];
            lo[a] = fminf(lo[a], v);
            hi[a] = fmaxf(hi[a], v);
        }
#pragma unroll
    for (int a = 0; a < 3; ++a) {
#pragma unroll
        for (int off = 32; off >= 1; off >>= 1) {
            lo[a] = fminf(lo[a], __shfl_xor(lo[a], off, 64));
            hi[a] = fmaxf(hi[a], __shfl_xor(hi[a], off, 64));
        }
        if (lane == 0) {
            s_box[a][wave] = lo[a];
            s_box[3 + a][wave] = hi[a];
        }
    }
    __syncthreads();
#pragma unroll
    for (int a = 0; a < 3; ++a) {
        float l = s_box[a][0], h = s_box[3 + a][0];
        for (int w = 1; w < nw; ++w) {
            l = fminf(l, s_box[a][w]);
            h = fmaxf(h, s_box[3 + a][w]);
        }
        lo[a] = l;
        ext[a] = h - l;
    }
}

constexpr int kCellBits = 14;
constexpr int kCells = 1 << kCellBits;

struct CellGrid {
    float lo[3];
    float inv;
    int bits[3];
};

__device__ __forceinline__ CellGrid make_cell_grid(const float (&lo)[3], const float (&ext)[3], int max_bits = kCellBits) {
    CellGrid g;
    const float big = fmaxf(ext[0], fmaxf(ext[1], ext[2]));
    float cell = big > 0.f ? big / 64.f : 1.f;
    for (int iter = 0; iter < 8; ++iter) {
        int total = 0;
#pragma unroll
        for (int a = 0; a < 3; ++a) {
            const int cells = (int)(ext[a] / cell) + 1;
            int b = 0;
            while ((1 << b) < cells && b < 6) ++b;
            g.bits[a] = b;
            total += b;
        }
        if (total <= max_bits) break;
        cell *= 1.26f;
    }
    g.lo[0] = lo[0]; g.lo[1] = lo[1]; g.lo[2] = lo[2];
    g.inv = 1.f / cell;
    return g;
}

__device__ __forceinline__ unsigned cell_code(const CellGrid &g, float px, float py, float pz) {
    const float p[3] = {px, py, pz};
    unsigned c[3];
#pragma unroll
    for (int a = 0; a < 3; ++a) {
        const int hi = (1 << g.bits[a]) - 1;
        const int v = (int)((p[a] - g.lo[a]) * g.inv);
        c[a] = (unsigned)min(max(v, 0), hi);
    }
    unsigned code = 0;
    int pos = 0;
#pragma unroll
    for (int b = 0; b < 6; ++b)
#pragma unroll
        for (int a = 0; a < 3; ++a)
            if (b < g.bits[a]) {
                code |= ((c[a] >> b) & 1u) << pos;
                ++pos;
            }
    return code;
}

__device__ __forceinline__ int hist_at(int b, int per_shift) { return b + (b >> per_shift); }
__device__ __forceinline__ int cell_hist_words(int threads) { return kCells + kCells / (kCells / threads) + 64; }

__device__ __forceinline__ void cell_sort_lds(const float *__restrict__ xyz, int n, const CellGrid &g, int *hist,
                                              int *s_part, unsigned short *perm) {
    const int q = threadIdx.x, T = blockDim.x, lane = q & 63, wave = q >> 6, nw = T >> 6;
    const int per = kCells / T;
    int per_shift = 0;
    while ((1 << per_shift) < per) ++per_shift;
    for (int i = q; i < cell_hist_words(T); i += T) hist[i] = 0;
    __syncthreads();
    for (int k = q; k < n; k += T)
        atomicAdd(&hist[hist_at((int)cell_code(g, xyz[k * 3 + 0], xyz[k * 3 + 1], xyz[k * 3 + 2]), per_shift)], 1);
    __syncthreads();
    int sum = 0;
    for (int i = 0; i < per; ++i) sum += hist[hist_at(q * per + i, per_shift)];
    const int incl = wave_inclusive_scan(sum);
    if (lane == 63) s_part[wave] = incl;
    __syncthreads();
    int base = incl - sum;
    for (int w = 0; w < wave; ++w) base += s_part[w];
    (void)nw;
    for (int i = 0; i < per; ++i) {
        const int at = hist_at(q * per + i, per_shift);
        const int c = hist[at];
        hist[at] = base;
        base += c;
    }
    __syncthreads();
    for (int k = q; k < n; k += T) {
        const int pos = atomicAdd(&hist[hist_at((int)cell_code(g, xyz[k * 3 + 0], xyz[k * 3 + 1], xyz[k * 3 + 2]), per_shift)], 1);
        perm[pos] = (unsigned short)k;
    }
    __syncthreads();
}

inline int scene_index_np(int n) {
    int np = 2048;
    while (np < n) np <<= 1;
    return np;
}
inline size_t scene_index_bytes(int b, int n) {
    if (b <= 0 || n < 1024 || n > 65536) return 0;
    const size_t np = (size_t)scene_index_np(n);
    return (size_t)b * (np * sizeof(float4) + (np / 64 + np / 256) * 6 * sizeof(float) + (n > 16384 ? np * sizeof(float) : 0));
}
inline float *scene_index_sampling_scratch(int b, int n, void *index) {
    const size_t np = (size_t)scene_index_np(n);
    return (float *)((char *)index + (size_t)b * (np * sizeof(float4) + (np / 64 + np / 256) * 6 * sizeof(float)));
}

int spatial_index_launch(int b, int n, int np, const float *xyz, float4 *sorted, float *boxes, float *qboxes, hipStream_t s,
                         int n_src = 0, const int *src_idx = nullptr, float *gathered = nullptr);

}
```

epnet_amd/pointnet2_cuda.py:

```python
import torch

from . import _lib
from ._tensor import ROWS16, dev_ptr, dev_ptr16, need, on_device_of, writes

_F, _I = torch.float32, torch.int32


def _deterministic():
    return torch.are_deterministic_algorithms_enabled()


def _det_call(l, name, ws_bytes, like, args, s, what):
    ws = torch.empty((max(int(ws_bytes), 1),), dtype=torch.uint8, device=like.device)
    _lib.check(getattr(l, "epnet_%s_det" % name)(*args, ws.data_ptr(), int(ws_bytes), s), "%s (deterministic)" % what)


@writes("idx")
def ball_query_wrapper(b, n, m, radius, nsample, new_xyz, xyz, idx):
    pn, px, pi = dev_ptr(new_xyz, "new_xyz", _F), dev_ptr(xyz, "xyz", _F), dev_ptr(idx, "idx", _I)
    need(new_xyz, b * m * 3, "new_xyz"); need(xyz, b * n * 3, "xyz"); need(idx, b * m * nsample, "idx")
    l = _lib.lib()
    ws_bytes = l.epnet_ball_query_workspace_bytes(b, n, m)
    with on_device_of(xyz) as s:
        if ws_bytes:
# ... 55 lines not shown
                      (b, c, n, npoints, pg, pi, pp), s, "gather_points_grad")
        return 1
    with on_device_of(grad_out) as s:
        _lib.check(_lib.lib().epnet_gather_points_grad(b, c, n, npoints, pg, pi, pp, s), "gather_points_grad")
    return 1


@writes("temp", "idx")
def furthest_point_sampling_wrapper(b, n, m, points, temp, idx):
    pp, pt, pi = dev_ptr(points, "points", _F), dev_ptr(temp, "temp", _F), dev_ptr(idx, "idx", _I)
    need(points, b * n * 3, "points"); need(temp, b * n, "temp"); need(idx, b * m, "idx")
    l = _lib.lib()
    with on_device_of(points) as s:
        if 16384 < n <= 65536:
            nbytes = l.epnet_scene_index_bytes(b, n)
            index = torch.empty((nbytes,), dtype=torch.uint8, device=points.device)
            _lib.check(l.epnet_scene_index_build(b, n, pp, index.data_ptr(), nbytes, s), "scene_index_build")
            _lib.check(l.epnet_furthest_point_sampling_indexed(b, n, m, pp, index.data_ptr(), nbytes, pt, pi, s),
                       "furthest_point_sampling")
        else:
            _lib.check(l.epnet_furthest_point_sampling(b, n, m, pp, pt, pi, s), "furthest_point_sampling")
    return 1


@writes("dist2", "idx")
def three_nn_wrapper(b, n, m, unknown, known, dist2, idx):
    pu, pk = dev_ptr(unknown, "unknown", _F), dev_ptr(known, "known", _F)
    pd, pi = dev_ptr(dist2, "dist2", _F), dev_ptr(idx, "idx", _I)
    need(unknown, b * n * 3, "unknown"); need(known, b * m * 3, "known"); need(dist2, b * n * 3, "dist2"); need(idx, b * n * 3, "idx")
    l = _lib.lib()
    ws_bytes = l.epnet_three_nn_workspace_bytes(b, n, m)
    with on_device_of(unknown) as s:
        if ws_bytes:
            ws = torch.empty((ws_bytes,), dtype=torch.uint8, device=unknown.device)
            _lib.check(l.epnet_three_nn_ws(b, n, m, pu, pk, pd, pi, ws.data_ptr(), ws_bytes, s), "three_nn")
        else:
            _lib.check(l.epnet_three_nn(b, n, m, pu, pk, pd, pi, s), "three_nn")


@writes("out")
def three_interpolate_wrapper(b, c, m, n, points, idx, weight, out):
    pp, pi = dev_ptr(points, "points", _F), dev_ptr(idx, "idx", _I)
    pw, po = dev_ptr(weight, "weight", _F), dev_ptr(out, "out", _F)
    need(points, b * c * m, "points"); need(idx, b * n * 3, "idx"); need(weight, b * n * 3, "weight"); need(out, b * c * n, "out")
    with on_device_of(points) as s:
        _lib.check(_lib.lib().epnet_three_interpolate(b, c, m, n, pp, pi, pw, po, s), "three_interpolate")


@writes("grad_points")
def three_interpolate_grad_wrapper(b, c, n, m, grad_out, idx, weight, grad_points):
    pg, pi = dev_ptr(grad_out, "grad_out", _F), dev_ptr(idx, "idx", _I)
    pw, pp = dev_ptr(weight, "weight", _F), dev_ptr(grad_points, "grad_points", _F)
    need(grad_out, b * c * n, "grad_out"); need(idx, b * n * 3, "idx"); need(weight, b * n * 3, "weight")
    need(grad_points, b * c * m, "grad_points")
    l = _lib.lib()
    if _deterministic():
        with on_device_of(grad_out) as s:
            _det_call(l, "three_interpolate_grad", l.epnet_three_interpolate_grad_det_workspace_bytes(b, n, m), grad_out,
                      (b, c, n, m, pg, pi, pw, pp), s, "three_interpolate_grad")
        return
    ws_bytes = l.epnet_three_interpolate_grad_workspace_bytes(b, n, m)
    with on_device_of(grad_out) as s:
        if ws_bytes:
            ws = torch.empty((ws_bytes,), dtype=torch.uint8, device=grad_out.device)
            _lib.check(l.epnet_three_interpolate_grad_ws(b, c, n, m, pg, pi, pw, pp, ws.data_ptr(), ws_bytes, s),
                       "three_interpolate_grad")
        else:
            _lib.check(l.epnet_three_interpolate_grad(b, c, n, m, pg, pi, pw, pp, s), "three_interpolate_grad")




def scene_index_bytes(b, n):
    return int(_lib.lib().epnet_scene_index_bytes(b, n))


def scene_index(xyz):
    b, n = xyz.shape[0], xyz.shape[1]
    l = _lib.lib()
    nbytes = l.epnet_scene_index_bytes(b, n)
    if not nbytes:
        return None
    px = dev_ptr(xyz, "xyz", _F)
    need(xyz, b * n * 3, "xyz")
    index = torch.empty((nbytes,), dtype=torch.uint8, device=xyz.device)
    with on_device_of(xyz) as s:
        _lib.check(l.epnet_scene_index_build(b, n, px, index.data_ptr(), nbytes, s), "scene_index_build")
    return index


@writes("index")
def scene_index_build_wrapper(b, n, xyz, index):
    px = dev_ptr(xyz, "xyz", _F)
    need(xyz, b * n * 3, "xyz")
    with on_device_of(xyz) as s:
        _lib.check(_lib.lib().epnet_scene_index_build(b, n, px, index.data_ptr(), index.numel(), s), "scene_index_build")
    return 1


@writes("new_xyz", "index")
def scene_index_build_gathered_wrapper(b, n_src, n, xyz_src, idx, new_xyz, index):
    px, pi, pn = dev_ptr(xyz_src, "xyz_src", _F), dev_ptr(idx, "idx", _I), dev_ptr(new_xyz, "new_xyz", _F)
    need(xyz_src, b * n_src * 3, "xyz_src")
    need(idx, b * n, "idx")
    need(new_xyz, b * n * 3, "new_xyz")
    with on_device_of(xyz_src) as s:
        _lib.check(_lib.lib().epnet_scene_index_build_gathered(b, n_src, n, px, pi, pn, index.data_ptr(), index.numel(), s),
                   "scene_index_build_gathered")
    return 1


def _index_args(index, like):
    if index is None:
        return None, 0
    if index.dtype != torch.uint8 or not index.is_contiguous() or index.device != like.device:
        raise RuntimeError("scene index must be the contiguous uint8 tensor scene_index() returned, on the points' device")
    return index.data_ptr(), index.numel()


@writes("temp", "idx")
def furthest_point_sampling_indexed_wrapper(b, n, m, points, index, temp, idx):
    pp, pt, pi = dev_ptr(points, "points", _F), dev_ptr(temp, "temp", _F), dev_ptr(idx, "idx", _I)
    need(points, b * n * 3, "points"); need(temp, b * n, "temp"); need(idx, b * m, "idx")
    px, nb = _index_args(index, points)
    with on_device_of(points) as s:
        _lib.check(_lib.lib().epnet_furthest_point_sampling_indexed(b, n, m, pp, px, nb, pt, pi, s), "furthest_point_sampling")
    return 1


@writes("idx", "new_xyz", "prefix_out")
def sample_centres_wrapper(b, n, m, points, index, idx, new_xyz, prefix_in=None, prefix_out=None, prefix_cap=0):
    pp, pi = dev_ptr(points, "points", _F), dev_ptr(idx, "idx", _I)
    pn = dev_ptr(new_xyz, "new_xyz", _F) if new_xyz is not None else None
    need(points, b * n * 3, "points"); need(idx, b * m, "idx")
    if new_xyz is not None:
        need(new_xyz, b * m * 3, "new_xyz")
    elif prefix_in is None and prefix_out is None:
        raise RuntimeError("new_xyz may be None only with prefix_in / prefix_out (epnet_sample_centres_chain)")
    px, nb = _index_args(index, points)
    temp = None if 64 <= n <= 16384 else torch.full((b, n), 1e10, dtype=_F, device=points.device)
    pt = None if temp is None else temp.data_ptr()
    with on_device_of(points) as s:
        if prefix_in is None and prefix_out is None:
            _lib.check(_lib.lib().epnet_sample_centres(b, n, m, pp, px, nb, pt, pi, pn, s), "sample_centres")
        else:
            pin = dev_ptr(prefix_in, "prefix_in", _I) if prefix_in is not None else None
            pout = dev_ptr(prefix_out, "prefix_out", _I) if prefix_out is not None else None
            if prefix_in is not None:
                need(prefix_in, b, "prefix_in")
            if prefix_out is not None:
                need(prefix_out, b, "prefix_out")
            _lib.check(_lib.lib().epnet_sample_centres_chain(b, n, m, pp, px, nb, pt, pi, pn, pin, pout, int(prefix_cap), s),
                       "sample_centres")
    return 1


@writes("idxs")
def ball_query_multi_wrapper(b, n, m, radii, nsamples, new_xyz, xyz, index, idxs):
    import ctypes
    pn, pxyz = dev_ptr(new_xyz, "new_xyz", _F), dev_ptr(xyz, "xyz", _F)
    need(new_xyz, b * m * 3, "new_xyz"); need(xyz, b * n * 3, "xyz")
    k = len(radii)
    assert len(nsamples) == k and len(idxs) == k
    ptrs = []
    for ns, t in zip(nsamples, idxs):
        ptrs.append(dev_ptr(t, "idx", _I))
        need(t, b * m * ns, "idx")
    px, nb = _index_args(index, xyz)
    c_r = (ctypes.c_float * k)(*[float(r) for r in radii])
    c_n = (ctypes.c_int * k)(*[int(x) for x in nsamples])
    c_p = (ctypes.c_void_p * k)(*ptrs)
    with on_device_of(xyz) as s:
        _lib.check(_lib.lib().epnet_ball_query_indexed_multi(b, n, m, k, ctypes.cast(c_r, ctypes.c_void_p),
                                                             ctypes.cast(c_n, ctypes.c_void_p), pn, pxyz, px, nb,
                                                             ctypes.cast(c_p, ctypes.c_void_p), s), "ball_query")
    return 1


@writes("idxs")
def ball_query_ordered_wrapper(b, n, m, radii, nsamples, new_xyz, xyz, index, centre_index, idxs):
    import ctypes
    pn, pxyz = dev_ptr(new_xyz, "new_xyz", _F), dev_ptr(xyz, "xyz", _F)
    need(new_xyz, b * m * 3, "new_xyz"); need(xyz, b * n * 3, "xyz")
    k = len(radii)
    assert len(nsamples) == k and len(idxs) == k
    ptrs = []
    for ns, t in zip(nsamples, idxs):
        ptrs.append(dev_ptr(t, "idx", _I))
        need(t, b * m * ns, "idx")
    px, nb = _index_args(index, xyz)
    pc, nc = _index_args(centre_index, new_xyz)
    c_r = (ctypes.c_float * k)(*[float(r) for r in radii])
    c_n = (ctypes.c_int * k)(*[int(x) for x in nsamples])
    c_p = (ctypes.c_void_p * k)(*ptrs)
    with on_device_of(xyz) as s:
        _lib.check(_lib.lib().epnet_ball_query_ordered(b, n, m, k, ctypes.cast(c_r, ctypes.c_void_p), ctypes.cast(c_n, ctypes.c_void_p),
                                                     pn, pxyz, px, nb, pc, nc, ctypes.cast(c_p, ctypes.c_void_p), s), "ball_query")
    return 1


@writes("dist2", "idx")
def three_nn_indexed_wrapper(b, n, m, unknown, known, unknown_index, known_index, dist2, idx):
    pu, pk = dev_ptr(unknown, "unknown", _F), dev_ptr(known, "known", _F)
    pd, pi = dev_ptr(dist2, "dist2", _F), dev_ptr(idx, "idx", _I)
    need(unknown, b * n * 3, "unknown"); need(known, b * m * 3, "known"); need(dist2, b * n * 3, "dist2"); need(idx, b * n * 3, "idx")
    pux, nu = _index_args(unknown_index, unknown)
    pkx, nk = _index_args(known_index, known)
    with on_device_of(unknown) as s:
        _lib.check(_lib.lib().epnet_three_nn_indexed(b, n, m, pu, pk, pux, nu, pkx, nk, pd, pi, s), "three_nn")
    return 1


@writes("idx")
def ball_query_indexed_wrapper(b, n, m, radius, nsample, new_xyz, xyz, index, idx):
    pn, pxyz, pi = dev_ptr(new_xyz, "new_xyz", _F), dev_ptr(xyz, "xyz", _F), dev_ptr(idx, "idx", _I)
    need(new_xyz, b * m * 3, "new_xyz"); need(xyz, b * n * 3, "xyz"); need(idx, b * m * nsample, "idx")
    px, nb = _index_args(index, xyz)
    with on_device_of(xyz) as s:
        _lib.check(_lib.lib().epnet_ball_query_indexed(b, n, m, radius, nsample, pn, pxyz, px, nb, pi, s), "ball_query")
    return 1

@writes("out")
def group_concat_wrapper(b, c, n, npoints, nsample, xyz, new_xyz, features, idx, out, use_xyz, workspace=None):
    px = dev_ptr(xyz, "xyz", _F) if use_xyz else None
    pn = dev_ptr(new_xyz, "new_xyz", _F) if use_xyz else None
    pf = dev_ptr(features, "features", _F) if c else None
    pi, po = dev_ptr(idx, "idx", _I), dev_ptr(out, "out", _F)
    need(idx, b * npoints * nsample, "idx"); need(out, b * ((3 if use_xyz else 0) + c) * npoints * nsample, "out")
    if use_xyz:
        need(xyz, b * n * 3, "xyz"); need(new_xyz, b * npoints * 3, "new_xyz")
    if c:
        need(features, b * c * n, "features")
    l = _lib.lib()
    ws_bytes = l.epnet_group_concat_workspace_bytes(b, c, n, npoints, nsample) if c else 0
    with on_device_of(idx) as s:
        if ws_bytes:
            ws = workspace if workspace is not None else torch.empty((ws_bytes,), dtype=torch.uint8, device=idx.device)
            if ws.dtype != torch.uint8 or ws.numel() < ws_bytes or ws.device != idx.device or not ws.is_contiguous():
                raise RuntimeError("group_concat workspace: a contiguous uint8 tensor of >= %d bytes on the tensors' device" % ws_bytes)
            _lib.check(l.epnet_group_concat_ws(b, c, n, npoints, nsample, px, pn, pf, pi, po, int(bool(use_xyz)), ws.data_ptr(),
                                               ws.numel(), s), "group_concat")
        else:
            _lib.check(l.epnet_group_concat(b, c, n, npoints, nsample, px, pn, pf, pi, po, int(bool(use_xyz)), s), "group_concat")
    return 1


def group_concat_workspace_bytes(b, c, n, npoints, nsample):
    return int(_lib.lib().epnet_group_concat_workspace_bytes(b, c, n, npoints, nsample)) if c else 0


@writes("outs")
def group_concat_multi_wrapper(b, c, n, npoints, nsamples, xyz, new_xyz, features, idxs, outs, use_xyz):
    import ctypes
    k = len(nsamples)
    assert len(idxs) == k and len(outs) == k
    px = dev_ptr(xyz, "xyz", _F) if use_xyz else None
    pn = dev_ptr(new_xyz, "new_xyz", _F) if use_xyz else None
    pf = dev_ptr(features, "features", _F) if c else None
    pis, pos = [], []
    for ns, i, o in zip(nsamples, idxs, outs):
        pis.append(dev_ptr(i, "idx", _I)); pos.append(dev_ptr(o, "out", _F))
        need(i, b * npoints * ns, "idx"); need(o, b * ((3 if use_xyz else 0) + c) * npoints * ns, "out")
    if use_xyz:
        need(xyz, b * n * 3, "xyz"); need(new_xyz, b * npoints * 3, "new_xyz")
    if c:
        need(features, b * c * n, "features")
    c_n = (ctypes.c_int * k)(*[int(x) for x in nsamples])
    c_i = (ctypes.c_void_p * k)(*pis)
    c_o = (ctypes.c_void_p * k)(*pos)
    with on_device_of(idxs[0]) as s:
        _lib.check(_lib.lib().epnet_group_concat_multi(b, c, n, npoints, k, ctypes.cast(c_n, ctypes.c_void_p), px, pn, pf,
                                                       ctypes.cast(c_i, ctypes.c_void_p), ctypes.cast(c_o, ctypes.c_void_p),
                                                       int(bool(use_xyz)), s), "group_concat")
    return 1


@writes("grad_features")
def group_concat_grad_wrapper(b, c, n, npoints, nsample, grad_out, idx, grad_features, use_xyz):
    pg, pi, pp = dev_ptr(grad_out, "grad_out", _F), dev_ptr(idx, "idx", _I), dev_ptr(grad_features, "grad_features", _F)
    need(grad_out, b * ((3 if use_xyz else 0) + c) * npoints * nsample, "grad_out"); need(grad_features, b * c * n, "grad_features")
    l = _lib.lib()
    if _deterministic():
        with on_device_of(grad_out) as s:
            _det_call(l, "group_concat_grad", l.epnet_group_concat_grad_det_workspace_bytes(b, n, npoints, nsample), grad_out,
                      (b, c, n, npoints, nsample, pg, pi, pp, int(bool(use_xyz))), s, "group_concat_grad")
        return 1
    ws_bytes = l.epnet_group_points_grad_workspace_bytes(b, n, npoints, nsample)
    with on_device_of(grad_out) as s:
        if ws_bytes:
            ws = torch.empty((ws_bytes,), dtype=torch.uint8, device=grad_out.device)
            _lib.check(l.epnet_group_concat_grad_ws(b, c, n, npoints, nsample, pg, pi, pp, int(bool(use_xyz)),
                                                    ws.data_ptr(), ws_bytes, s), "group_concat_grad")
        else:
            _lib.check(l.epnet_group_concat_grad(b, c, n, npoints, nsample, pg, pi, pp, int(bool(use_xyz)), s),
                       "group_concat_grad")
    return 1


@writes("out", "arg")
def pool_max_wrapper(rows, nsample, x, out, arg):
    px, po = dev_ptr(x, "x", _F), dev_ptr(out, "out", _F)
    pa = dev_ptr(arg, "arg", _I) if arg is not None else None
    need(x, rows * nsample, "x"); need(out, rows, "out")
    if arg is not None:
        need(arg, rows, "arg")
    with on_device_of(x) as s:
# ... 123 lines not shown
```

epnet_amd/sa_stack.py:

```python
import os

import torch

from . import pointnet2_cuda as ext

RPN_NPOINTS = (4096, 1024, 256, 64)
RPN_RADII = ((0.1, 0.5), (0.5, 1.0), (1.0, 2.0), (2.0, 4.0))
RPN_NSAMPLES = ((16, 32), (16, 32), (16, 32), (16, 32))
RPN_FEAT_CHANNELS = (0, 96, 256, 512)
RPN_FP = ((1024, 64, 256), (512, 256, 1024), (512, 1024, 4096), (256, 4096, 16384))


CONFIGS = {
    2: dict(n=16384, npoints=RPN_NPOINTS, radii=RPN_RADII, nsamples=RPN_NSAMPLES, feat_channels=RPN_FEAT_CHANNELS),
    5: dict(n=65536, npoints=(16384,), radii=((0.5,),), nsamples=((64,),), feat_channels=(64,)),
}


def sa_algorithmic_bytes(n=16384, npoints=RPN_NPOINTS, nsamples=RPN_NSAMPLES, feat_channels=RPN_FEAT_CHANNELS):
    out = {"fps": 0, "gather": 0, "ball_query": 0, "group_xyz": 0, "group_feat": 0}
    cur = n
    for lvl, m in enumerate(npoints):
        out["fps"] += cur * 12 + m * 4
        out["gather"] += m * 4 + 3 * cur * 4 + 3 * m * 4
        for ns in nsamples[lvl]:
            out["ball_query"] += cur * 12 + m * 12 + m * ns * 4
            out["group_xyz"] += m * ns * 4 + 3 * cur * 4 + 3 * m * ns * 4
            c = feat_channels[lvl]
            if c:
                out["group_feat"] += m * ns * 4 + c * cur * 4 + c * m * ns * 4
        cur = m
    out["total"] = sum(out.values())
    return out


def fp_algorithmic_bytes(fp=RPN_FP):
    out = {"three_nn": 0, "three_interpolate": 0}
    for c, m, n in fp:
        out["three_nn"] += n * 12 + m * 12 + n * 24
        out["three_interpolate"] += c * m * 4 + n * 24 + c * n * 4
    out["total"] = sum(out.values())
    return out


class SAStack:
    def __init__(self, batch, n=16384, device="cuda", npoints=RPN_NPOINTS, radii=RPN_RADII, nsamples=RPN_NSAMPLES,
                 feat_channels=RPN_FEAT_CHANNELS, with_fp=False, fp=RPN_FP, seed=0, overlap=True, fused=True,
                 shared_index=True, pipelined=False, fused_sampling=False, queries_in_s=None, s_query_levels=None, stages=None):
        self.batch, self.n = batch, n
        if stages is None:
            stages = int(os.environ.get("EPNET_SA_STAGES", "2"))
        self.stages = 3 if (pipelined and stages == 3 and fused_sampling and fused and shared_index) else (2 if pipelined else 1)
        self.ring = self.stages
        self.overlap = overlap
        self.fused = fused
        self.shared_index = shared_index
        self.pipelined = pipelined
        self.fused_sampling = fused_sampling
        env_q = int(os.environ.get("EPNET_SA_QUERIES_IN_S", "1"))
        env_lv = os.environ.get("EPNET_SA_S_QUERY_LEVELS")
        every = frozenset(range(len(npoints)))
        if not pipelined:
            chosen = frozenset()
        elif s_query_levels is not None:
            chosen = frozenset(int(v) for v in s_query_levels)
        elif queries_in_s is not None:
            chosen = every if queries_in_s else frozenset()
        elif env_lv is not None:
            chosen = frozenset(int(v) for v in env_lv.split(",") if v.strip())
        elif self.stages == 3:
            chosen = every
        elif env_q == 2 or (env_q == 1 and with_fp):
            chosen = every
        elif env_q == 1 and batch * n >= 240 * 16384:
            chosen = every - {0}
        else:
            chosen = frozenset()
        self.s_query_levels = chosen & every
        self.queries_in_s = self.s_query_levels == every
        self.chain = bool(int(os.environ.get("EPNET_SA_CHAIN", "1"))) and fused_sampling
        self.fuse_gather = bool(int(os.environ.get("EPNET_SA_FUSE_GATHER", "1")))
        self._deferred = None
        self.s_first = bool(int(os.environ.get("EPNET_SA_S_FIRST", "0" if self.s_query_levels else "1")))
        self.tail_scales = int(os.environ.get("EPNET_SA_TAIL_SCALES", "0"))
        self.multi_query = bool(int(os.environ.get("EPNET_SA_MULTI_QUERY", "1")))
        self.multi_group = bool(int(os.environ.get("EPNET_SA_MULTI_GROUP", "1")))
        self.ordered_query = bool(int(os.environ.get("EPNET_SA_ORDERED_QUERY", "1")))
        self.side = None
        self.npoints, self.radii, self.nsamples, self.feat_channels = npoints, radii, nsamples, feat_channels
        self.with_fp, self.fp = with_fp, fp
        dev = torch.device(device)
        g = torch.Generator().manual_seed(seed)
        f32, i32 = torch.float32, torch.int32
        self.levels = []
        cur = n
        for lvl, m in enumerate(npoints):
            c = feat_channels[lvl]
            index_bytes = ext.scene_index_bytes(batch, cur) if shared_index else 0
            L = {
                "n": cur, "m": m, "c": c,
                "xyz_t_sets": [torch.empty((batch, 3, cur), dtype=f32, device=dev) for _ in range(self.ring if not fused else 1)],
                "temp": torch.empty((batch, cur), dtype=f32, device=dev),
                "fps_idx_sets": ([torch.empty((batch, m), dtype=i32, device=dev) for _ in range(3)] if self.stages == 3 else None),
                "fps_idx": None,
                "new_xyz_t": torch.empty((batch, 3, m), dtype=f32, device=dev),
                "sets": [{"new_xyz": torch.empty((batch, m, 3), dtype=f32, device=dev),
                          "index": (torch.empty((index_bytes,), dtype=torch.uint8, device=dev) if index_bytes else None),
                          "prefix": torch.zeros((batch,), dtype=i32, device=dev),
                          "centre_index": (torch.empty((ext.scene_index_bytes(batch, m),), dtype=torch.uint8, device=dev)
                                           if (shared_index and lvl + 1 == len(npoints) and ext.scene_index_bytes(batch, m)) else None)}
                         for _ in range(self.ring)],
                "features": (torch.randn((batch, c, cur), generator=g, dtype=f32).to(dev) if c else None),
                "scales": [],
            }
            for radius, ns in zip(radii[lvl], nsamples[lvl]):
                S = {"radius": radius, "ns": ns, "idx": torch.empty((batch, m, ns), dtype=i32, device=dev)}
                S["idx_sets"] = [S["idx"]] + ([torch.empty((batch, m, ns), dtype=i32, device=dev) for _ in range(self.ring - 1)]
                                              if lvl in self.s_query_levels else [])
                if fused:
                    S["grouped"] = torch.empty((batch, 3 + c, m, ns), dtype=f32, device=dev)
                    ws_bytes = ext.group_concat_workspace_bytes(batch, c, cur, m, ns)
                    S["workspace"] = torch.empty((ws_bytes,), dtype=torch.uint8, device=dev) if ws_bytes else None
                else:
                    S["grouped_xyz"] = torch.empty((batch, 3, m, ns), dtype=f32, device=dev)
                    S["grouped_feat"] = torch.empty((batch, c, m, ns), dtype=f32, device=dev) if c else None
                L["scales"].append(S)
            if L["fps_idx_sets"] is None:
                one = torch.empty((batch, m), dtype=i32, device=dev)
                L["fps_idx_sets"] = [one] * self.ring
            L["fps_idx"] = L["fps_idx_sets"][0]
            self.levels.append(L)
            cur = m
        self.fp_bufs = []
        if with_fp:
            for c, m, nn_ in fp:
                sets = [{"dist2": torch.empty((batch, nn_, 3), dtype=f32, device=dev),
                         "idx": torch.empty((batch, nn_, 3), dtype=i32, device=dev),
                         "weight": torch.empty((batch, nn_, 3), dtype=f32, device=dev)} for _ in range(self.ring)]
                self.fp_bufs.append({
                    "c": c, "m": m, "n": nn_,
                    "known_feats": torch.randn((batch, c, m), generator=g, dtype=f32).to(dev),
                    "sets": sets,
                    "dist2": sets[0]["dist2"], "idx": sets[0]["idx"],
                    "out": torch.empty((batch, c, nn_), dtype=f32, device=dev),
                })
        self.graphs = []
        self.replays = 0
        self.inputs = []
        self._prev_xyz = None

    @property
    def static_xyz(self):
        if self.pipelined and self.inputs:
            raise AttributeError("a pipelined stack has one input buffer per parity: use stack.inputs / stack.input_buffer()")
        return self.inputs[0] if self.inputs else None

    def input_buffer(self, step=None):
        step = self.replays if step is None else step
        return self.inputs[step % len(self.inputs)]

    def owners(self):
        if self.stages == 3:
            raise RuntimeError("three stages: see owners3()")
        p = (self.replays - 1) & 1 if self.pipelined else 0
        return p, (1 - p if self.pipelined else 0)

    def owners3(self):
        k = self.replays - 1
        return k % 3, (k - 1) % 3, (k - 2) % 3

    def chain_identity_share(self, parity=None):
        if not self.chain:
            return None
        if parity is None:
            parity = self.owners3()[1] if self.stages == 3 else self.owners()[0]
        out = []
        for lvl in range(1, len(self.levels)):
            known = self.levels[lvl - 1]["sets"][parity if self.pipelined else 0]["prefix"]
            out.append(round(float((known >= self.levels[lvl]["m"]).float().mean().item()), 4))
        return out

    def _sample_level(self, L, cur_xyz, parity, index_built=False, defer_ok=False):
        b, n, m = self.batch, L["n"], L["m"]
        P = L["sets"][parity]
        lvl = self.levels.index(L)
        pending, self._deferred = self._deferred, None
        if pending is not None and pending[1:] == (lvl - 1, parity):
            src_xyz, _, _ = pending
            prev = self.levels[lvl - 1]
            ext.scene_index_build_gathered_wrapper(b, prev["n"], n, src_xyz, prev["fps_idx_sets"][parity], cur_xyz, P["index"])
        elif P["index"] is not None and not index_built:
            ext.scene_index_build_wrapper(b, n, cur_xyz, P["index"])
        if self.fused_sampling:
            if not self.fused:
                L["xyz_t_sets"][parity].copy_(cur_xyz.transpose(1, 2))
            if self.chain:
                prefix_in = self.levels[lvl - 1]["sets"][parity]["prefix"] if lvl > 0 else None
                nxt = self.levels[lvl + 1]["m"] if lvl + 1 < len(self.levels) else 1
                nxt_L = self.levels[lvl + 1] if lvl + 1 < len(self.levels) else None
                defer = (defer_ok and self.fuse_gather and self.fused and nxt_L is not None
                         and nxt_L["sets"][parity]["index"] is not None and 1024 <= m <= 16384)
                ext.sample_centres_wrapper(b, n, m, cur_xyz, P["index"], L["fps_idx_sets"][parity], None if defer else P["new_xyz"],
                                           prefix_in, P["prefix"], nxt)
                if defer:
                    self._deferred = (cur_xyz, lvl, parity)
            else:
                ext.sample_centres_wrapper(b, n, m, cur_xyz, P["index"], L["fps_idx_sets"][parity], P["new_xyz"])
        else:
            L["xyz_t_sets"][parity if not self.fused else 0].copy_(cur_xyz.transpose(1, 2))
            L["temp"].fill_(1e10)
            if P["index"] is not None:
                ext.furthest_point_sampling_indexed_wrapper(b, n, m, cur_xyz, P["index"], L["temp"], L["fps_idx_sets"][parity])
            else:
                ext.furthest_point_sampling_wrapper(b, n, m, cur_xyz, L["temp"], L["fps_idx_sets"][parity])
            ext.gather_points_wrapper(b, 3, n, m, L["xyz_t_sets"][parity if not self.fused else 0], L["fps_idx_sets"][parity], L["new_xyz_t"])
            P["new_xyz"].copy_(L["new_xyz_t"].transpose(1, 2))
        return P["new_xyz"]

    def _idx(self, S, parity):
        return S["idx_sets"][parity] if len(S["idx_sets"]) > 1 else S["idx"]

    def _query_scale(self, L, S, cur_xyz, parity):
        b, n, m = self.batch, L["n"], L["m"]
        P = L["sets"][parity]
        if P["index"] is not None:
            ext.ball_query_indexed_wrapper(b, n, m, S["radius"], S["ns"], P["new_xyz"], cur_xyz, P["index"], self._idx(S, parity))
        else:
            ext.ball_query_wrapper(b, n, m, S["radius"], S["ns"], P["new_xyz"], cur_xyz, self._idx(S, parity))

    def _group_scale(self, L, S, cur_xyz, parity):
        b, n, m = self.batch, L["n"], L["m"]
        if self.fused:
            ext.group_concat_wrapper(b, L["c"], n, m, S["ns"], cur_xyz, L["sets"][parity]["new_xyz"], L["features"],
                                     self._idx(S, parity), S["grouped"], True, S.get("workspace"))
        else:
            ext.group_points_wrapper(b, 3, n, m, S["ns"], L["xyz_t_sets"][parity], self._idx(S, parity), S["grouped_xyz"])
            if L["c"]:
                ext.group_points_wrapper(b, L["c"], n, m, S["ns"], L["features"], self._idx(S, parity), S["grouped_feat"])

    def _query_level(self, L, cur_xyz, parity):
        P = L["sets"][parity]
        centre_index = (self._centre_index(L, parity)
                        if (self.ordered_query and L["n"] > 16384 and P["index"] is not None and len(L["scales"]) <= 2) else None)
        if centre_index is not None:
            ext.ball_query_ordered_wrapper(self.batch, L["n"], L["m"], [S["radius"] for S in L["scales"]],
                                         [S["ns"] for S in L["scales"]], P["new_xyz"], cur_xyz, P["index"], centre_index,
                                         [self._idx(S, parity) for S in L["scales"]])
        elif P["index"] is not None and self.multi_query:
            ext.ball_query_multi_wrapper(self.batch, L["n"], L["m"], [S["radius"] for S in L["scales"]],
                                         [S["ns"] for S in L["scales"]], P["new_xyz"], cur_xyz, P["index"],
                                         [self._idx(S, parity) for S in L["scales"]])
        else:
            for S in L["scales"]:
                self._query_scale(L, S, cur_xyz, parity)

    def _centre_index(self, L, parity):
        lvl = self.levels.index(L)
        if lvl + 1 < len(self.levels):
            return self.levels[lvl + 1]["sets"][parity]["index"] if self.shared_index else None
        own = L["sets"][parity].get("centre_index")
        if own is not None:
            ext.scene_index_build_wrapper(self.batch, L["m"], L["sets"][parity]["new_xyz"], own)
        return own

    def _group_scales(self, L, cur_xyz, parity):
        if self.fused and self.multi_group and len(L["scales"]) > 1:
            ext.group_concat_multi_wrapper(self.batch, L["c"], L["n"], L["m"], [S["ns"] for S in L["scales"]], cur_xyz,
                                           L["sets"][parity]["new_xyz"], L["features"], [self._idx(S, parity) for S in L["scales"]],
                                           [S["grouped"] for S in L["scales"]], True)
        else:
            for S in L["scales"]:
                self._group_scale(L, S, cur_xyz, parity)

    def _group_level(self, L, cur_xyz, parity):
        self._query_level(L, cur_xyz, parity)
        self._group_scales(L, cur_xyz, parity)

    def _side_stream(self, device):
        if self.side is None:
            self.side = torch.cuda.Stream(device=device)
        return self.side

    def run(self, xyz):
        main = torch.cuda.current_stream(xyz.device)
        side = self._side_stream(xyz.device) if self.overlap else None
        cur_xyz = xyz
        built = False
        for lvl, L in enumerate(self.levels):
            new_xyz = self._sample_level(L, cur_xyz, 0, index_built=built)
            built = False
            nxt = self.levels[lvl + 1] if lvl + 1 < len(self.levels) else None
            if self.ordered_query and L["n"] > 16384 and nxt is not None and nxt["sets"][0]["index"] is not None:
                ext.scene_index_build_wrapper(self.batch, L["m"], new_xyz, nxt["sets"][0]["index"])
                built = True
            if side is not None:
                side.wait_stream(main)
                with torch.cuda.stream(side):
                    self._group_level(L, cur_xyz, 0)
            else:
                self._group_level(L, cur_xyz, 0)
            cur_xyz = new_xyz
        if side is not None:
            main.wait_stream(side)
        if self.with_fp:
            self._run_fp(xyz, 0)

    def run_pipelined(self, xyz, prev_xyz, step):
        parity = step & 1
        main = torch.cuda.current_stream(xyz.device)
        side = self._side_stream(xyz.device)
        first = self.levels[0]
        if first["sets"][parity]["index"] is not None:
            ext.scene_index_build_wrapper(self.batch, first["n"], xyz, first["sets"][parity]["index"])
        forked = torch.cuda.Event()
        forked.record(main)
        s_cur = xyz
        if self.s_first:
            s_cur = self._sample_level(first, xyz, parity, index_built=True, defer_ok=True)
        side.wait_event(forked)
        with torch.cuda.stream(side):
            inputs = [prev_xyz] + [L["sets"][1 - parity]["new_xyz"] for L in self.levels[:-1]]
            in_s = self.s_query_levels
            deep = list(enumerate(zip(self.levels, inputs)))[1:]
            for lvl, (L, cur) in deep[:1]:
                if lvl not in in_s:
                    self._query_level(L, cur, 1 - parity)
                self._group_scales(L, cur, 1 - parity)
            for lvl, (L, cur) in deep[1:]:
                if lvl not in in_s:
                    self._query_level(L, cur, 1 - parity)
            for lvl, (L, cur) in deep[1:]:
                self._group_scales(L, cur, 1 - parity)
            if 0 in in_s:
                self._group_scales(first, prev_xyz, 1 - parity)
            elif self.tail_scales == 0:
                self._group_level(first, prev_xyz, 1 - parity)
            else:
                for S in first["scales"][self.tail_scales:]:
                    self._query_scale(first, S, prev_xyz, 1 - parity)
                    self._group_scale(first, S, prev_xyz, 1 - parity)
            if self.with_fp:
                self._interpolate_fp(1 - parity)
        for L in self.levels[(1 if self.s_first else 0):]:
            s_cur = self._sample_level(L, s_cur, parity, index_built=L is first, defer_ok=True)
        if self.with_fp:
            self._search_fp(xyz, parity)
        if self.s_query_levels:
            self._queries_of(xyz, parity)
        for S in first["scales"][:(0 if 0 in self.s_query_levels else self.tail_scales)]:
            self._query_scale(first, S, prev_xyz, 1 - parity)
            self._group_scale(first, S, prev_xyz, 1 - parity)
        main.wait_stream(side)

    def run_pipelined3(self, clouds, step):
        p, q, r = step % 3, (step - 1) % 3, (step - 2) % 3
        main = torch.cuda.current_stream(clouds[p].device)
        side = self._side_stream(clouds[p].device)
        third = self._third_stream(clouds[p].device)
        first = self.levels[0]
        ext.scene_index_build_wrapper(self.batch, first["n"], clouds[p], first["sets"][p]["index"])
        forked = torch.cuda.Event()
        forked.record(main)
        self._deferred = None
        self._sample_level(first, clouds[p], p, index_built=True, defer_ok=True)
        s1_deferred = self._deferred is not None
        self._deferred = None
        side.wait_event(forked)
        with torch.cuda.stream(side):
            inputs = [clouds[r]] + [L["sets"][r]["new_xyz"] for L in self.levels[:-1]]
            order = list(zip(self.levels, inputs))
            for lvl, (L, cur) in enumerate(order[1:], start=1):
                if lvl not in self.s_query_levels:
                    self._query_level(L, cur, r)
                self._group_scales(L, cur, r)
            if 0 not in self.s_query_levels:
                self._query_level(first, clouds[r], r)
            self._group_scales(first, clouds[r], r)
            if self.with_fp:
                self._interpolate_fp(r)
        third.wait_event(forked)
        with torch.cuda.stream(third):
            self._deferred = (clouds[q], 0, q) if s1_deferred else None
            cur = first["sets"][q]["new_xyz"]
            for L in self.levels[1:]:
                cur = self._sample_level(L, cur, q, defer_ok=True)
            self._deferred = None
            if self.with_fp:
                self._search_fp(clouds[q], q)
            self._queries_of(clouds[q], q)
        main.wait_stream(side)
        main.wait_stream(third)

    def _third_stream(self, device):
        if getattr(self, "third", None) is None:
            self.third = torch.cuda.Stream(device=device)
        return self.third

    def _queries_of(self, xyz, parity):
        cur = xyz
        for lvl, L in enumerate(self.levels):
            if lvl in self.s_query_levels:
                self._query_level(L, cur, parity)
            cur = L["sets"][parity]["new_xyz"]

    def _search_fp(self, xyz, parity):
        b = self.batch
        xyzs = [xyz] + [L["sets"][parity]["new_xyz"] for L in self.levels]
        indices = [L["sets"][parity]["index"] for L in self.levels] + [None]
        for k, F in enumerate(self.fp_bufs):
            P = F["sets"][parity if len(F["sets"]) > 1 else 0]
            known = xyzs[len(self.levels) - k]
            unknown = xyzs[len(self.levels) - k - 1]
            k_index, u_index = indices[len(self.levels) - k], indices[len(self.levels) - k - 1]
            if k_index is not None:
                ext.three_nn_indexed_wrapper(b, F["n"], F["m"], unknown, known, u_index, k_index, P["dist2"], P["idx"])
            else:
                ext.three_nn_wrapper(b, F["n"], F["m"], unknown, known, P["dist2"], P["idx"])
            inv = 1.0 / (torch.sqrt(P["dist2"]) + 1e-8)
            torch.div(inv, torch.sum(inv, dim=2, keepdim=True), out=P["weight"])
            F["dist2"], F["idx"] = P["dist2"], P["idx"]

    def _interpolate_fp(self, parity):
        b = self.batch
        for F in self.fp_bufs:
            P = F["sets"][parity if len(F["sets"]) > 1 else 0]
            ext.three_interpolate_wrapper(b, F["c"], F["m"], F["n"], F["known_feats"], P["idx"], P["weight"], F["out"])

    def _run_fp(self, xyz, parity):
        self._search_fp(xyz, parity)
        self._interpolate_fp(parity)

    def _prime(self, clouds):
        for parity in range(self.ring):
            xyz = cur = clouds[parity]
            self._deferred = None
            for L in self.levels:
                cur = self._sample_level(L, cur, parity, defer_ok=True)
            self._deferred = None
            if self.with_fp:
                self._search_fp(xyz, parity)
            if self.s_query_levels:
                self._queries_of(xyz, parity)

    def _step_eager(self, k):
        if self.stages == 3:
            self.run_pipelined3(self.inputs, k)
        elif self.pipelined:
            self.run_pipelined(self.inputs[k & 1], self.inputs[1 - (k & 1)], k)
        else:
            self.run(self.inputs[0])

    def capture(self, xyz, xyz_other=None, xyz_third=None):
        self.inputs = [xyz.clone()]
        if self.pipelined:
            self.inputs.append((xyz if xyz_other is None else xyz_other).clone())
        if self.stages == 3:
            self.inputs.append((xyz if xyz_third is None else xyz_third).clone())
        s = torch.cuda.Stream()
        s.wait_stream(torch.cuda.current_stream())
        period = 1
        with torch.cuda.stream(s):
            if self.pipelined:
                self._prime(self.inputs)
        if self.pipelined:
            period = self.ring
        with torch.cuda.stream(s):
            for k in range(max(2, period)):
                self._step_eager(k)
        torch.cuda.current_stream().wait_stream(s)
        torch.cuda.synchronize()
        self.graphs = []
        for k in range(period):
            g = torch.cuda.CUDAGraph()
            with torch.cuda.graph(g):
                self._step_eager(k)
            self.graphs.append(g)
        self.replays = 0
        return self.graphs[0]

    def replay(self, xyz=None):
        if xyz is not None:
            self.input_buffer().copy_(xyz)
        self.graphs[self.replays % len(self.graphs)].replay()
        self.replays += 1

    def step(self, xyz):
        if self.stages == 3:
            if self._prev_xyz is None:
                self._prime([xyz, xyz, xyz])
                self._eager_clouds = [xyz, xyz, xyz]
                self._prev_xyz = xyz
                self.replays = 0
            self._eager_clouds[self.replays % 3] = xyz
            self.run_pipelined3(self._eager_clouds, self.replays)
            self.replays += 1
        elif self.pipelined:
            if self._prev_xyz is None:
                self._prime([xyz, xyz])
                self._prev_xyz = xyz
                self.replays = 0
            self.run_pipelined(xyz, self._prev_xyz, self.replays & 1)
            self._prev_xyz = xyz
            self.replays += 1
        else:
            self.run(xyz)
```

include/epnet_ops.h:

```cpp
#ifndef EPNET_OPS_H
#define EPNET_OPS_H

#include <stddef.h>
#include <stdint.h>

#ifdef __cplusplus
extern "C" {
#endif

#define EPNET_ABI_VERSION 1

#define EPNET_OK 0
#define EPNET_EINVAL (-1)
#define EPNET_ELAUNCH (-2)
#define EPNET_ENOMEM (-3)
#define EPNET_ELIMIT (-4)

typedef void *epnet_stream_t;

int epnet_abi_version(void);
const char *epnet_strerror(int code);
const char *epnet_last_hip_error(void);

int epnet_set_tuning(const char *name, int value);
int epnet_get_tuning(const char *name, int *value);


int epnet_furthest_point_sampling(int b, int n, int m, const float *xyz, float *temp, int *idx,
                                  epnet_stream_t stream);

int epnet_gather_points(int b, int c, int n, int npoints, const float *points, const int *idx,
                        float *out, epnet_stream_t stream);

int epnet_gather_points_grad(int b, int c, int n, int npoints, const float *grad_out, const int *idx,
                             float *grad_points, epnet_stream_t stream);

int epnet_ball_query(int b, int n, int m, float radius, int nsample, const float *new_xyz,
                     const float *xyz, int *idx, epnet_stream_t stream);

size_t epnet_ball_query_workspace_bytes(int b, int n, int m);
int epnet_ball_query_ws(int b, int n, int m, float radius, int nsample, const float *new_xyz, const float *xyz,
                        int *idx, void *workspace, size_t workspace_bytes, epnet_stream_t stream);

int epnet_group_points(int b, int c, int n, int npoints, int nsample, const float *points,
                       const int *idx, float *out, epnet_stream_t stream);

int epnet_group_points_grad(int b, int c, int n, int npoints, int nsample, const float *grad_out,
                            const int *idx, float *grad_points, epnet_stream_t stream);

int epnet_group_concat(int b, int c, int n, int npoints, int nsample, const float *xyz, const float *new_xyz,
                       const float *features, const int *idx, float *out, int use_xyz, epnet_stream_t stream);
size_t epnet_group_concat_workspace_bytes(int b, int c, int n, int npoints, int nsample);
int epnet_group_concat_ws(int b, int c, int n, int npoints, int nsample, const float *xyz, const float *new_xyz,
                          const float *features, const int *idx, float *out, int use_xyz, void *workspace,
                          size_t workspace_bytes, epnet_stream_t stream);

int epnet_group_concat_grad(int b, int c, int n, int npoints, int nsample, const float *grad_out, const int *idx,
                            float *grad_features, int use_xyz, epnet_stream_t stream);

size_t epnet_group_points_grad_workspace_bytes(int b, int n, int npoints, int nsample);
int epnet_group_points_grad_ws(int b, int c, int n, int npoints, int nsample, const float *grad_out, const int *idx,
                               float *grad_points, void *workspace, size_t workspace_bytes, epnet_stream_t stream);
int epnet_group_concat_grad_ws(int b, int c, int n, int npoints, int nsample, const float *grad_out, const int *idx,
                               float *grad_features, int use_xyz, void *workspace, size_t workspace_bytes,
                               epnet_stream_t stream);

int epnet_three_nn(int b, int n, int m, const float *unknown, const float *known, float *dist2,
                   int *idx, epnet_stream_t stream);

size_t epnet_three_nn_workspace_bytes(int b, int n, int m);
int epnet_three_nn_ws(int b, int n, int m, const float *unknown, const float *known, float *dist2, int *idx,
                      void *workspace, size_t workspace_bytes, epnet_stream_t stream);

int epnet_three_interpolate(int b, int c, int m, int n, const float *points, const int *idx,
                            const float *weight, float *out, epnet_stream_t stream);

int epnet_three_interpolate_grad(int b, int c, int n, int m, const float *grad_out, const int *idx,
                                 const float *weight, float *grad_points, epnet_stream_t stream);

int epnet_group_concat_multi(int b, int c, int n, int npoints, int nscales, const int *nsamples, const float *xyz,
                             const float *new_xyz, const float *features, const int *const *idx, float *const *out,
                             int use_xyz, epnet_stream_t stream);

size_t epnet_three_interpolate_grad_workspace_bytes(int b, int n, int m);
int epnet_three_interpolate_grad_ws(int b, int c, int n, int m, const float *grad_out, const int *idx,
                                    const float *weight, float *grad_points, void *workspace, size_t workspace_bytes,
                                    epnet_stream_t stream);

int epnet_group_linear(int b, int c, int n, int npoints, int nsample, const float *xyz, const float *new_xyz, const float *z,
                       const int *idx, const float *w_xyz, const float *bias, float *out, epnet_stream_t stream);

int epnet_group_linear_grad_w(int b, int c, int n, int npoints, int nsample, const float *grad_out, const float *xyz,
                              const float *new_xyz, const int *idx, float *grad_w, epnet_stream_t stream);

int epnet_pool_max(long long rows, int nsample, const float *x, float *out, int *arg, epnet_stream_t stream);
int epnet_pool_max_grad(long long rows, int nsample, const float *grad_out, const int *arg, float *grad_x,
                        epnet_stream_t stream);

#define EPNET_F16 1
#define EPNET_BF16 2
int epnet_group_linear_h(int b, int c, int n, int npoints, int nsample, const float *xyz, const float *new_xyz, const void *z,
                         const int *idx, const float *w_xyz, const float *bias, void *out, int dtype, epnet_stream_t stream);
int epnet_pool_max_h(long long rows, int nsample, const void *x, void *out, int *arg, int dtype, epnet_stream_t stream);
int epnet_pool_max_grad_h(long long rows, int nsample, const void *grad_out, const int *arg, void *grad_x, int dtype,
                          epnet_stream_t stream);
int epnet_three_interpolate_h(int b, int c, int m, int n, const void *points, const int *idx, const float *weight, void *out,
                              int dtype, epnet_stream_t stream);

int epnet_feature_gather(int b, int c, int h, int w, int n_src, int n, int align_corners, const float *feature_map,
                         const float *xy, const int *idx, float *out, float *xy_out, epnet_stream_t stream);
int epnet_feature_gather_grad(int b, int c, int h, int w, int n, int align_corners, const float *grad_out, const float *xy,
                              float *grad_feature_map, epnet_stream_t stream);

size_t epnet_gather_points_grad_det_workspace_bytes(int b, int n, int npoints);
int epnet_gather_points_grad_det(int b, int c, int n, int npoints, const float *grad_out, const int *idx, float *grad_points,
                                 void *workspace, size_t workspace_bytes, epnet_stream_t stream);
size_t epnet_group_points_grad_det_workspace_bytes(int b, int n, int npoints, int nsample);
int epnet_group_points_grad_det(int b, int c, int n, int npoints, int nsample, const float *grad_out, const int *idx,
                                float *grad_points, void *workspace, size_t workspace_bytes, epnet_stream_t stream);
size_t epnet_group_concat_grad_det_workspace_bytes(int b, int n, int npoints, int nsample);
int epnet_group_concat_grad_det(int b, int c, int n, int npoints, int nsample, const float *grad_out, const int *idx,
                                float *grad_features, int use_xyz, void *workspace, size_t workspace_bytes, epnet_stream_t stream);
size_t epnet_three_interpolate_grad_det_workspace_bytes(int b, int n, int m);
int epnet_three_interpolate_grad_det(int b, int c, int n, int m, const float *grad_out, const int *idx, const float *weight,
                                     float *grad_points, void *workspace, size_t workspace_bytes, epnet_stream_t stream);
size_t epnet_feature_gather_grad_det_workspace_bytes(int b, int h, int w, int n);
int epnet_feature_gather_grad_det(int b, int c, int h, int w, int n, int align_corners, const float *grad_out, const float *xy,
                                  float *grad_feature_map, void *workspace, size_t workspace_bytes, epnet_stream_t stream);
size_t epnet_group_linear_grad_w_det_workspace_bytes(int b, int c, int npoints, int nsample);
int epnet_group_linear_grad_w_det(int b, int c, int n, int npoints, int nsample, const float *grad_out, const float *xyz,
                                  const float *new_xyz, const int *idx, float *grad_w, void *workspace, size_t workspace_bytes,
                                  epnet_stream_t stream);

size_t epnet_scene_index_bytes(int b, int n);
int epnet_scene_index_build(int b, int n, const float *xyz, void *index, size_t index_bytes, epnet_stream_t stream);
int epnet_scene_index_build_gathered(int b, int n_src, int n, const float *xyz_src, const int *idx, float *gathered, void *index,
                                     size_t index_bytes, epnet_stream_t stream);
int epnet_furthest_point_sampling_indexed(int b, int n, int m, const float *xyz, void *index,
                                          size_t index_bytes, float *temp, int *idx, epnet_stream_t stream);
int epnet_sample_centres(int b, int n, int m, const float *xyz, void *index, size_t index_bytes, float *temp,
                         int *idx, float *new_xyz, epnet_stream_t stream);
int epnet_sample_centres_chain(int b, int n, int m, const float *xyz, void *index, size_t index_bytes, float *temp,
                               int *idx, float *new_xyz, const int *prefix_in, int *prefix_out, int prefix_cap,
                               epnet_stream_t stream);
int epnet_three_nn_indexed(int b, int n, int m, const float *unknown, const float *known, const void *unknown_index,
                           size_t unknown_index_bytes, const void *known_index, size_t known_index_bytes, float *dist2,
                           int *idx, epnet_stream_t stream);
int epnet_ball_query_indexed(int b, int n, int m, float radius, int nsample, const float *new_xyz, const float *xyz,
                             const void *index, size_t index_bytes, int *idx, epnet_stream_t stream);
int epnet_ball_query_indexed_multi(int b, int n, int m, int nscales, const float *radii, const int *nsamples,
                                   const float *new_xyz, const float *xyz, const void *index, size_t index_bytes,
                                   int *const *idx, epnet_stream_t stream);
int epnet_ball_query_ordered(int b, int n, int m, int nscales, const float *radii, const int *nsamples, const float *new_xyz,
                             const float *xyz, const void *index, size_t index_bytes, const void *centre_index,
                             size_t centre_index_bytes, int *const *idx, epnet_stream_t stream);


int epnet_boxes_overlap_bev(int num_a, const float *boxes_a, int num_b, const float *boxes_b,
                            float *ans_overlap, epnet_stream_t stream);

int epnet_boxes_iou_bev(int num_a, const float *boxes_a, int num_b, const float *boxes_b,
                        float *ans_iou, epnet_stream_t stream);

int epnet_boxes_iou3d(int num_a, const float *boxes_a, int num_b, const float *boxes_b, float *ans_iou3d,
                      epnet_stream_t stream);

int epnet_boxes_iou3d_pairs(int k, const float *boxes_a, const float *boxes_b, float *ans_iou3d, epnet_stream_t stream);

int epnet_aug_roi_by_noise(int k, int aug_times, float pos_thresh, float *roi_boxes3d, const float *gt_boxes3d,
                           const float *iou3d_src, const int *tries, const unsigned char *keep_draw,
                           const float *noise, float *iou_of_rois, epnet_stream_t stream);

size_t epnet_rcnn_sample_rois_workspace_bytes(int b, int m, int g, int r);
int epnet_rcnn_sample_rois(int b, int m, int g, int gc, int r, int fg_per_image, float fg_thresh, float cls_bg_thresh,
                           float cls_bg_thresh_lo, double hard_bg_ratio, int aug_times, const float *rois,
                           const float *gt_boxes3d, const float *fg_key, const float *slot_u,
                           const unsigned char *keep_draw, const float *noise, void *workspace, size_t workspace_bytes,
                           float *batch_rois, float *batch_gt_of_rois, float *batch_roi_iou, int *scene_info, int *src_inds,
                           float *iou_src, int *tries, float *max_overlaps, int *gt_assignment, epnet_stream_t stream);

size_t epnet_rpn_proposals_workspace_bytes(int b, int distance_based, int pre_nms_top_n, int post_nms_top_n);
int epnet_rpn_proposals(int b, int n, const float *proposals, const float *scores, const int64_t *order,
                        int distance_based, int pre_nms_top_n, int post_nms_top_n, float nms_thresh, int rotated,
                        void *workspace, size_t workspace_bytes, float *ret_bbox3d, float *ret_scores, int *ret_count,
                        epnet_stream_t stream);

int epnet_decode_bbox_target(long long rows, int anchor_cols, const float *anchors, const float *pred_reg, int channels,
                             int bins_xz, int bins_y, double loc_scope, double loc_bin_size, double loc_y_scope,
                             double loc_y_bin_size, int num_head_bin, const float *anchor_size, int xz_fine, int y_by_bin,
                             int ry_fine, int avg_by_bin, int ry_with_bin, int y_to_bottom, float *boxes, epnet_stream_t stream);

int epnet_score_order(int b, int n, const float *scores, int64_t *order, epnet_stream_t stream);

size_t epnet_rpn_handover_workspace_bytes(int b, int n, int distance_based, int pre_nms_top_n, int post_nms_top_n);
int epnet_rpn_handover(int b, int n, int channels, const float *scores, const float *rpn_reg, const float *xyz, int bins_xz,
                       int bins_y, double loc_scope, double loc_bin_size, double loc_y_scope, double loc_y_bin_size,
                       int num_head_bin, const float *anchor_size, int xz_fine, int y_by_bin, int ry_fine, int avg_by_bin,
                       int ry_with_bin, float score_thresh, int distance_based, int pre_nms_top_n, int post_nms_top_n,
                       float nms_thresh, int rotated, void *workspace, size_t workspace_bytes, float *ret_bbox3d,
                       float *ret_scores, int *ret_count, float *seg_mask, float *pts_depth, float *proposals, int64_t *order,
                       epnet_stream_t stream);

size_t epnet_rcnn_detections_workspace_bytes(int b, int m);
int epnet_rcnn_detections(int b, int m, const float *boxes3d, const float *raw_scores, const float *norm_scores,
                          float score_thresh, float nms_thresh, void *workspace, size_t workspace_bytes,
                          float *det_boxes3d, float *det_scores, int *det_count, epnet_stream_t stream);

size_t epnet_eval_recall_workspace_bytes(int b, int m, int g);
int epnet_eval_recall(int b, int m, int g, int gc, int n, int nt, const float *thresholds, const float *pred_boxes3d,
                      const float *roi_boxes3d, const float *gt_boxes3d, const int *seg_result, const int *rpn_cls_label,
                      void *workspace, size_t workspace_bytes, int *scene_stats, int64_t *seg_counts, int64_t *totals,
                      float *gt_max_pred, float *gt_max_roi, float *pred_max_iou, epnet_stream_t stream);

int epnet_kitti_records(int b, int m, const float *boxes3d, const float *scores, const int *count, const float *P2,
                        const int *img_shape, double *records, int *rec_count, float *bbox_raw, int *valid,
                        epnet_stream_t stream);

size_t epnet_nms_workspace_bytes(int boxes_num);

int epnet_nms(const float *boxes, int boxes_num, float nms_overlap_thresh, void *workspace,
              size_t workspace_bytes, int64_t *keep, int *num_keep, epnet_stream_t stream);

int epnet_nms_normal(const float *boxes, int boxes_num, float nms_overlap_thresh, void *workspace,
                     size_t workspace_bytes, int64_t *keep, int *num_keep, epnet_stream_t stream);


size_t epnet_roipool3d_workspace_bytes(int batch_size, int boxes_num, int sampled_pts_num);

int epnet_roipool3d(int batch_size, int pts_num, int boxes_num, int feature_in_len,
                    int sampled_pts_num, const float *xyz, const float *boxes3d,
                    const float *pts_feature, float *pooled_features, int *pooled_empty_flag,
                    void *workspace, size_t workspace_bytes, epnet_stream_t stream);

int epnet_roipool3d_canonical(int batch_size, int pts_num, int boxes_num, int feature_in_len, int sampled_pts_num,
                              float pool_extra_width, const float *xyz, const float *rois, const float *pts_feature,
                              float *pooled_features, int *pooled_empty_flag, epnet_stream_t stream);

int epnet_roipool3d_train(int batch_size, int pts_num, int boxes_num, int feature_in_len, int sampled_pts_num,
                          float pool_extra_width, float reg_fg_thresh, float cls_fg_thresh, float cls_bg_thresh,
                          const float *xyz, const float *pts_feature, const float *rois, const float *gt_of_rois,
                          const float *roi_iou, const float *aug, float *sampled_pts, float *pts_feature_out,
                          float *rois_out, float *gt_out, int *cls_label, int *reg_valid_mask, float *mask_score,
                          int *pooled_empty_flag, epnet_stream_t stream);


#define EPNET_BOX_LOSS_TERMS 24
#define EPNET_LOSS_IOU_RAW 0
#define EPNET_LOSS_IOU_CLS_MASK_WITH_BIN 1
#define EPNET_LOSS_CLS_FOCAL 0
#define EPNET_LOSS_CLS_BCE 1
#define EPNET_LOSS_CLS_NONE 2
size_t epnet_box_loss_workspace_bytes(long long rows, int c);
int epnet_box_loss(long long rows, int c, double loc_scope, double loc_bin_size, int num_head_bin, int ry_fine,
                   int iou_loss_type, int cls_loss_type, double focal_alpha, double focal_gamma, double fg_weight,
                   double w_cls, double w_reg, double w_train, double ce_weight, const float *cls_logit,
                   const float *pred_reg, const float *reg_label, const int *cls_label, const int *reg_mask,
                   const float *iou_branch_pred, const float *anchor, float *terms, float *grad_cls, float *grad_reg,
                   float *grad_iou_branch, void *workspace, size_t workspace_bytes, epnet_stream_t stream);


int epnet_rpn_targets(int b, int n, int g, float extra_width, const float *pts, const float *gt_boxes3d,
                      const float *gt_alpha, const float *aug, float *pts_out, float *gt_out, int *cls_label,
                      float *reg_label, epnet_stream_t stream);


size_t epnet_scan_prepare_workspace_bytes(int b, int p, int n);
int epnet_scan_prepare(int b, int p, int n, int reduce_by_range, const double *scope, float near_depth,
                       const float *pts_lidar, const int *num_raw, const float *V2C, const float *R0, const float *P2,
                       const int *img_shape, const int *keys, const int *slot_perm, void *workspace,
                       size_t workspace_bytes, float *pts_rect, float *pts_intensity, float *pts_origin_xy,
                       float *pts_input, int *choice, int *scene_info, epnet_stream_t stream);

int epnet_image_normalise(int b, int h_in, int w_in, int h_out, int w_out, const uint8_t *img, const int *img_shape,
                          const double *mean, const double *std, float *out, epnet_stream_t stream);

#define EPNET_KITTI_MAX_DT 1024
#define EPNET_KITTI_MAX_GT 256
#define EPNET_KITTI_MAX_DC 256
#define EPNET_KITTI_MAX_COMBOS 16
#define EPNET_KITTI_MAX_THRESHOLDS 64

int epnet_kitti_overlaps(int metric, int criterion, int frames, int max_rows, int max_cols, const int *row_off,
                         const int *col_off, const int64_t *ov_off, const double *row_boxes, const double *col_boxes,
                         double *overlaps, epnet_stream_t stream);

int epnet_kitti_match(int frames, int total_gt, int total_dt, int max_gt, int max_dt, int num_difficulty, int combos,
                      const int *combo_difficulty, const double *combo_min_overlap, const int *gt_off, const int *dt_off,
                      const int64_t *ov_off, const double *overlaps, const double *dt_score, const int *ignored_gt,
                      const int *ignored_dt, double *matched, epnet_stream_t stream);

size_t epnet_kitti_pr_workspace_bytes(int frames, int combos, int tstride);

int epnet_kitti_pr(int frames, int total_gt, int total_dt, int max_gt, int max_dt, int max_dc, int num_difficulty, int combos,
                   int tstride, int metric, int compute_aos, const int *combo_difficulty, const double *combo_min_overlap,
                   const int *combo_num_thresholds, const int *gt_off, const int *dt_off, const int *dc_off,
                   const int64_t *ov_off, const double *overlaps, const double *dt_score, const int *ignored_gt,
                   const int *ignored_dt, const double *dt_bbox, const double *dc_bbox, const double *gt_alpha,
// ... 35 lines not shown
```

Before: 1.456 billion points/s.

## Build next level's spatial index inside the FPS sampling kernel epilogue

Adds a sample_centres_chain_index entry point whose FPS kernel, for the kW==8 configuration, writes the sampled centres and then builds the next level's scene spatial index (sort, bucket boxes, quad boxes) in an epilogue that reuses a shared LDS arena. This removes the separate gathered index-build launch and its re-read of the gathered points. The index-build body is factored into a shared device template, the stream-side query levels now exclude level 1, and the ball-query quad scan drops a branch in favour of clamped slots plus a ballot mask. The epilogue costs the sampling workgroup extra LDS and registers, and it serialises index-building work behind FPS on that block.

```diff
diff --git a/epnet_amd/_lib.py b/epnet_amd/_lib.py
--- a/epnet_amd/_lib.py
+++ b/epnet_amd/_lib.py
@@ -68,6 +68,7 @@
     "epnet_furthest_point_sampling_indexed": (_i, [_i, _i, _i, _vp, _vp, _sz, _vp, _vp, _vp]),
     "epnet_sample_centres": (_i, [_i, _i, _i, _vp, _vp, _sz, _vp, _vp, _vp, _vp]),
     "epnet_sample_centres_chain": (_i, [_i, _i, _i, _vp, _vp, _sz, _vp, _vp, _vp, _vp, _vp, _i, _vp]),
+    "epnet_sample_centres_chain_index": (_i, [_i, _i, _i, _vp, _vp, _sz, _vp, _vp, _vp, _vp, _vp, _i, _vp, _sz, _vp]),
     "epnet_group_concat_multi": (_i, [_i, _i, _i, _i, _i, _vp, _vp, _vp, _vp, _vp, _vp, _i, _vp]),
     "epnet_ball_query_indexed_multi": (_i, [_i, _i, _i, _i, _vp, _vp, _vp, _vp, _vp, _sz, _vp, _vp]),
     "epnet_ball_query_ordered": (_i, [_i, _i, _i, _i, _vp, _vp, _vp, _vp, _vp, _sz, _vp, _sz, _vp, _vp]),
diff --git a/epnet_amd/csrc/ball_query.hip b/epnet_amd/csrc/ball_query.hip
--- a/epnet_amd/csrc/ball_query.hip
+++ b/epnet_amd/csrc/ball_query.hip
@@ -93,9 +93,6 @@
 #endif
 #ifdef EPNET_IX_STATS
 __device__ unsigned long long g_ix_stats[8];
-#define EPNET_IX_STAMP(var) const unsigned long long var = __builtin_amdgcn_s_memtime()
-#else
-#define EPNET_IX_STAMP(var)
 #endif
 
 template <int kIxThreads, int BITS>
@@ -104,206 +101,17 @@
                                                               float *__restrict__ qboxes, int n_src = 0,
                                                               const int *__restrict__ src_idx = nullptr,
                                                               float *__restrict__ gathered = nullptr) {
-    constexpr int kCells = 1 << BITS;
     extern __shared__ int s_hist[];
     __shared__ float s_box[6][16];
     __shared__ int s_part[16];
-    const int q = threadIdx.x, lane = q & 63, wave = q >> 6;
     __builtin_amdgcn_s_setprio(3);
-    xyz += (size_t)blockIdx.x * (src_idx ? n_src : n) * 3;
-    if (src_idx) {
-        src_idx += (size_t)blockIdx.x * n;
-        gathered += (size_t)blockIdx.x * n * 3;
-    }
-    sorted += (size_t)blockIdx.x * np;
-    boxes += (size_t)blockIdx.x * (np / 64) * 6;
-    constexpr int per = kCells / kIxThreads;
-    constexpr int per_shift = per == 16 ? 4 : per == 8 ? 3 : per == 4 ? 2 : -1;
-    static_assert(per_shift > 0, "scan layout");
-    constexpr int kIxPerThread = 16;
-    const bool in_regs = n <= kIxThreads * kIxPerThread;
-    float px[kIxPerThread], py[kIxPerThread], pz[kIxPerThread];
-    float lo[3], ext[3];
-    EPNET_IX_STAMP(t_0);
-    if (in_regs) {
-        float mn[3] = {3.4e38f, 3.4e38f, 3.4e38f}, mx[3] = {-3.4e38f, -3.4e38f, -3.4e38f};
-        int row[kIxPerThread];
-#pragma unroll
-        for (int i = 0; i < kIxPerThread; ++i) {
-            const int k = q + i * kIxThreads;
-            const int kk = k < n ? k : 0;
-            row[i] = src_idx ? src_idx[kk] : kk;
-        }
-#pragma unroll
-        for (int i = 0; i < kIxPerThread; ++i) {
-            px[i] = xyz[row[i] * 3 + 0];
-            py[i] = xyz[row[i] * 3 + 1];
-            pz[i] = xyz[row[i] * 3 + 2];
-        }
-        if (src_idx) {
-#pragma unroll
-            for (int i = 0; i < kIxPerThread; ++i) {
-                const int k = q + i * kIxThreads;
-                if (k < n) {
-                    gathered[k * 3 + 0] = px[i];
-                    gathered[k * 3 + 1] = py[i];
-                    gathered[k * 3 + 2] = pz[i];
-                }
-            }
-        }
-#pragma unroll
-        for (int i = 0; i < kIxPerThread; ++i) {
-            const bool ok = q + i * kIxThreads < n;
-            mn[0] = fminf(mn[0], ok ? px[i] : 3.4e38f); mx[0] = fmaxf(mx[0], ok ? px[i] : -3.4e38f);
-            mn[1] = fminf(mn[1], ok ? py[i] : 3.4e38f); mx[1] = fmaxf(mx[1], ok ? py[i] : -3.4e38f);
-            mn[2] = fminf(mn[2], ok ? pz[i] : 3.4e38f); mx[2] = fmaxf(mx[2], ok ? pz[i] : -3.4e38f);
-        }
-#pragma unroll
-        for (int a = 0; a < 3; ++a) {
-            const float l = wave_minf_all(mn[a]), h = wave_maxf_all(mx[a]);
-            if (lane == 0) {
-                s_box[a][wave] = l;
-                s_box[3 + a][wave] = h;
-            }
-        }
-        __syncthreads();
-#pragma unroll
-        for (int a = 0; a < 3; ++a) {
-            float l = s_box[a][0], h = s_box[3 + a][0];
-            for (int w = 1; w < kIxThreads / 64; ++w) {
-                l = fminf(l, s_box[a][w]);
-                h = fmaxf(h, s_box[3 + a][w]);
-            }
-            lo[a] = l;
-            ext[a] = h - l;
-        }
-    } else {
-        block_bbox3(xyz, n, s_box, lo, ext);
-    }
-    const CellGrid g = make_cell_grid(lo, ext, BITS);
-    EPNET_IX_STAMP(t_1);
-    for (int i = q; i < kCells + kCells / per + 64; i += kIxThreads) s_hist[i] = 0;
-    __syncthreads();
-    EPNET_IX_STAMP(t_2);
-    int code[kIxPerThread], rank[kIxPerThread];
-    if (in_regs) {
-#pragma unroll
-        for (int i = 0; i < kIxPerThread; ++i) code[i] = hist_at((int)cell_code(g, px[i], py[i], pz[i]), per_shift);
-#pragma unroll
-        for (int i = 0; i < kIxPerThread; ++i)
-            rank[i] = atomicAdd(&s_hist[q + i * kIxThreads < n ? code[i] : kCells + kCells / per + lane], 1);
-    } else {
-        for (int k = q; k < n; k += kIxThreads)
-            atomicAdd(&s_hist[hist_at((int)cell_code(g, xyz[k * 3 + 0], xyz[k * 3 + 1], xyz[k * 3 + 2]), per_shift)], 1);
-    }
-    __syncthreads();
-    EPNET_IX_STAMP(t_3);
-    int sum = 0;
-    for (int i = 0; i < per; ++i) sum += s_hist[hist_at(q * per + i, per_shift)];
-    const int incl = wave_inclusive_scan(sum);
-    if (lane == 63) s_part[wave] = incl;
-    __syncthreads();
-    int base = incl - sum;
-    for (int w = 0; w < wave; ++w) base += s_part[w];
-    for (int i = 0; i < per; ++i) {
-        const int at = hist_at(q * per + i, per_shift);
-        const int c = s_hist[at];
-        s_hist[at] = base;
-        base += c;
-    }
-    __syncthreads();
-    EPNET_IX_STAMP(t_4);
-    auto bucket_box = [&](int p, const float4 v) {
-        const bool real = p < n;
-        const float cx_ = canonical(v.x), cy_ = canonical(v.y), cz_ = canonical(v.z);
-        float mnx = real ? cx_ : 3.4e38f, mxx = real ? cx_ : -3.4e38f, mny = real ? cy_ : 3.4e38f, mxy = real ? cy_ : -3.4e38f,
-              mnz = real ? cz_ : 3.4e38f, mxz = real ? cz_ : -3.4e38f;
-        wave_box(mnx, mxx, mny, mxy, mnz, mxz);
-        if (lane == 0) {
-            float *bx = boxes + (p >> 6) * 6;
-            const bool any = mnx <= mxx;
-            bx[0] = any ? mnx : 3.0e38f; bx[1] = any ? mxx : 3.0e38f;
-            bx[2] = any ? mny : 3.0e38f; bx[3] = any ? mxy : 3.0e38f;
-            bx[4] = any ? mnz : 3.0e38f; bx[5] = any ? mxz : 3.0e38f;
-        }
-    };
-    const bool staged = in_regs && (np & 255) == 0;
-    if (staged) {
-        float4 *s_stage = reinterpret_cast<float4 *>(s_hist + kCells + kCells / per + 64);
-        int pos[kIxPerThread];
-#pragma unroll
-        for (int i = 0; i < kIxPerThread; ++i) pos[i] = s_hist[code[i]] + rank[i];
-        const int quarter = kIxThreads == 256 ? min(np >> 2, 512) : np >> 2;
-        for (int h = 0; h * quarter < np; ++h) {
-            const int base = h * quarter, len = min(quarter, np - base);
-            for (int p = q; p < len; p += kIxThreads)
-                if (base + p >= n) s_stage[p] = make_float4(3.0e38f, 3.0e38f, 3.0e38f, __int_as_float(-1));
-#pragma unroll
-            for (int i = 0; i < kIxPerThread; ++i) {
-                const int k = q + i * kIxThreads;
-                if (k < n && (unsigned)(pos[i] - base) < (unsigned)quarter)
-                    s_stage[pos[i] - base] = make_float4(px[i], py[i], pz[i], __int_as_float(k));
-            }
-            __syncthreads();
-            for (int p = q; p < len; p += kIxThreads) {
-                const float4 v = s_stage[p];
-                sorted[base + p] = v;
-                bucket_box(base + p, v);
-            }
-            __syncthreads();
-        }
-    } else {
-        if (in_regs) {
-#pragma unroll
-            for (int i = 0; i < kIxPerThread; ++i) {
-                const int k = q + i * kIxThreads;
-                if (k < n) sorted[s_hist[code[i]] + rank[i]] = make_float4(px[i], py[i], pz[i], __int_as_float(k));
-            }
-        } else {
-            for (int k = q; k < n; k += kIxThreads) {
-                const float x = xyz[k * 3 + 0], y = xyz[k * 3 + 1], z = xyz[k * 3 + 2];
-                const int pos = atomicAdd(&s_hist[hist_at((int)cell_code(g, x, y, z), per_shift)], 1);
-                sorted[pos] = make_float4(x, y, z, __int_as_float(k));
-            }
-        }
-        for (int p = n + q; p < np; p += kIxThreads)
-            sorted[p] = make_float4(3.0e38f, 3.0e38f, 3.0e38f, __int_as_float(-1));
-        __threadfence_block();
-        __syncthreads();
-        for (int p = q; p < np; p += kIxThreads) bucket_box(p, sorted[p]);
-    }
 #ifdef EPNET_IX_STATS
-    {
-        EPNET_IX_STAMP(t_6);
-        if (q == 0) {
-            atomicAdd(&g_ix_stats[0], t_1 - t_0); atomicAdd(&g_ix_stats[1], t_2 - t_1); atomicAdd(&g_ix_stats[2], t_3 - t_2);
-            atomicAdd(&g_ix_stats[3], t_4 - t_3); atomicAdd(&g_ix_stats[4], t_6 - t_4);
-            atomicAdd(&g_ix_stats[7], 1ull);
-        }
-    }
-#endif
-    if (!qboxes) return;
-    qboxes += (size_t)blockIdx.x * (np / 256) * 6;
-    __threadfence_block();
-    __syncthreads();
-    for (int g = q; g < np / 256; g += kIxThreads) {
-        float mn[3] = {3.4e38f, 3.4e38f, 3.4e38f}, mx[3] = {-3.4e38f, -3.4e38f, -3.4e38f};
-        for (int k = 0; k < 4; ++k) {
-            const float *bx = boxes + (g * 4 + k) * 6;
-            if (bx[0] < 3.0e38f)
-#pragma unroll
-                for (int a = 0; a < 3; ++a) {
-                    mn[a] = fminf(mn[a], bx[2 * a]);
-                    mx[a] = fmaxf(mx[a], bx[2 * a + 1]);
-                }
-        }
-        const bool any = mn[0] <= mx[0];
-#pragma unroll
-        for (int a = 0; a < 3; ++a) {
-            qboxes[g * 6 + 2 * a] = any ? mn[a] : 3.0e38f;
-            qboxes[g * 6 + 2 * a + 1] = any ? mx[a] : 3.0e38f;
-        }
-    }
+    unsigned long long *const ix_stats = g_ix_stats;
+#else
+    unsigned long long *const ix_stats = nullptr;
+#endif
+    scene_index_build_block<kIxThreads, BITS, 16, kIxThreads == 256 ? 512 : 0, false>(s_hist, s_box, s_part, n, np, xyz, sorted, boxes, qboxes,
+                                                                                      n_src, src_idx, gathered, ix_stats);
 }
 
 constexpr int kQThreads = 256;
@@ -750,6 +558,8 @@
         scan_pairs(__ballot(n0), __ballot(n1), [](int, int bit) { return bit; });
     } else {
         const int nq = np >> 8;
+        s_quads[wave][0][lane] = 0;
+        s_quads[wave][1][lane] = 0;
         for (int q0 = 0; q0 < nq; q0 += 64) {
             const int qd = q0 + lane;
             const float *qb = qboxes + __umul24(min(qd, nq - 1), 6);
@@ -763,13 +573,10 @@
             const int nmine = half ? nq1 : nq0;
             for (int s0 = 0; s0 < max(nq0, nq1); s0 += 8) {
                 const int slot = s0 + ((lane & 31) >> 2);
-                int bid = 0;
-                bool bnear = false;
-                if (slot < nmine) {
-                    bid = s_quads[wave][half][slot] * 4 + (lane & 3);
-                    bnear = box_near(boxes + __umul24(bid, 6), hx, hy, hz, r2max);
-                }
-                const unsigned long long cand = __builtin_amdgcn_ballot_w64(bnear);
+                const unsigned sl = min((unsigned)slot, (unsigned)(nmine - 1));
+                const int bid = s_quads[wave][half][sl] * 4 + (lane & 3);
+                const unsigned long long cand = __builtin_amdgcn_ballot_w64(box_near(boxes + __umul24(bid, 6), hx, hy, hz, r2max)) &
+                                                __builtin_amdgcn_ballot_w64(slot < nmine);
                 scan_pairs(cand & 0xFFFFFFFFull, cand >> 32,
                            [&](int e, int bit) { return __builtin_amdgcn_readlane(bid, bit + 32 * e); });
             }
diff --git a/epnet_amd/csrc/fps.hip b/epnet_amd/csrc/fps.hip
--- a/epnet_amd/csrc/fps.hip
+++ b/epnet_amd/csrc/fps.hip
@@ -310,13 +310,11 @@
 }
 
 template <int kW, int PPT, typename VF, typename VI, typename VH>
-__device__ __forceinline__ void fps_rounds(int m, const VF &x, const VF &y, const VF &z, VI &t, const VH &rk2,
+__device__ __forceinline__ void fps_rounds(unsigned long long *s_key, float4 (*s_rec)[64 * kW], int *s_idx, int m, const VF &x,
+                                           const VF &y, const VF &z, VI &t, const VH &rk2,
                                            float cx, float cy, float cz, int *__restrict__ idxs,
                                            int *__restrict__ tie_free = nullptr, int known = 0,
                                            const float *__restrict__ xyz_in_order = nullptr, int detect_upto = 0x7fffffff) {
-    __shared__ unsigned long long s_key[3];
-    __shared__ float4 s_rec[2][64 * kW];
-    __shared__ int s_idx[kIdxBufP];
     const int q = threadIdx.x;
     const int lane = q & 63, wave = q >> 6;
     const int sub = lane & (PPT - 1);
@@ -516,6 +514,9 @@
     unsigned short *perm = reinterpret_cast<unsigned short *>(s_dyn + kCells + kCells / (kCells / kT) + 64);
     __shared__ int s_part[16];
     __shared__ float s_box[6][16];
+    __shared__ unsigned long long s_key[3];
+    __shared__ float4 s_rec[2][64 * kW];
+    __shared__ int s_idx[kIdxBufP];
     const int q = threadIdx.x;
     const int lane = q & 63, wave = q >> 6;
     xyz += (size_t)blockIdx.x * n * 3;
@@ -552,7 +553,7 @@
             set_rank(rk2, j, 0xFFFFu);
         }
     }
-    fps_rounds<kW, PPT>(m, x, y, z, t, rk2, xyz[0], xyz[1], xyz[2], idxs, prefix_out ? prefix_out + blockIdx.x : nullptr, 0,
+    fps_rounds<kW, PPT>(s_key, s_rec, s_idx, m, x, y, z, t, rk2, xyz[0], xyz[1], xyz[2], idxs, prefix_out ? prefix_out + blockIdx.x : nullptr, 0,
                         nullptr, prefix_cap);
     if (temp) {
 #pragma unroll
@@ -561,6 +562,14 @@
             if (r != 0xFFFFu) temp[unrank14(r)] = __int_as_float(t[j]);
         }
     }
+}
+
+template <int kT, int BITS, int kPer, int kStage>
+__device__ __attribute__((noinline)) void fps_index_epilogue(int *s_hist, float (*s_box)[16], int *s_part, int m, int np,
+                                                             const float *xyz, float4 *sorted, float *boxes, float *qboxes, int n_src,
+                                                             const int *src_idx, float *gathered) {
+    scene_index_build_block<kT, BITS, kPer, kStage, true>(s_hist, s_box, s_part, m, np, xyz, sorted, boxes, qboxes, n_src, src_idx,
+                                                          gathered);
 }
 
 template <int kW, int PPT>
@@ -568,11 +577,27 @@
                                                               float *__restrict__ temp, int *__restrict__ idxs,
                                                               const int *__restrict__ prefix_in,
                                                               int *__restrict__ prefix_out, const float *__restrict__ xyz,
-                                                              int prefix_cap, int prologue_init) {
+                                                              int prefix_cap, int prologue_init, void *next_index,
+                                                              float *__restrict__ new_xyz) {
     typedef float vecf __attribute__((ext_vector_type(PPT)));
     typedef int veci __attribute__((ext_vector_type(PPT)));
     constexpr int NP = 64 * kW * PPT;
-    __shared__ float s_first[4];
+    constexpr bool kEpilogue = kW == 8;
+    constexpr int kRecAt = 0, kIdxAt = kRecAt + 2 * 64 * kW * 16, kKeyAt = kIdxAt + kIdxBufP * 4, kFirstAt = kKeyAt + 32,
+                  kRoundsBytes = kFirstAt + 16;
+    constexpr int kIxBits = 12, kIxPer = 8, kIxStage = 512;
+    constexpr int kIxHistWords = (1 << kIxBits) + (1 << kIxBits) / ((1 << kIxBits) / (64 * kW)) + 64;
+    constexpr int kStageAt = kIxHistWords * 4, kBoxAt = kStageAt + kIxStage * 16, kPartAt = kBoxAt + 6 * 16 * 4,
+                  kIxBytes = kEpilogue ? kPartAt + 16 * 4 : 0;
+    constexpr int kArgsAt = kRoundsBytes;
+    static_assert(kStageAt % 16 == 0 && kIxBytes <= 32768, "the sampling workgroup shares its CU with two 64 KB row gathers");
+    static_assert(!kEpilogue || kArgsAt + 32 <= kIxBytes, "epilogue arguments");
+    __shared__ __attribute__((aligned(16))) unsigned char s_lds[kRoundsBytes > kIxBytes ? kRoundsBytes : kIxBytes];
+    unsigned long long *const s_key = reinterpret_cast<unsigned long long *>(s_lds + kKeyAt);
+    float4(*const s_rec)[64 * kW] = reinterpret_cast<float4(*)[64 * kW]>(s_lds + kRecAt);
+    int *const s_idx = reinterpret_cast<int *>(s_lds + kIdxAt);
+    float *const s_first = reinterpret_cast<float *>(s_lds + kFirstAt);
+    unsigned long long *const s_args = reinterpret_cast<unsigned long long *>(s_lds + kArgsAt);
     const int q = threadIdx.x;
     const int lane = q & 63, wave = q >> 6;
     const int known = prefix_in ? prefix_in[blockIdx.x] : 0;
@@ -605,14 +630,40 @@
             set_rank(rk2, j, 0xFFFFu);
         }
     }
+    if constexpr (kEpilogue) {
+        if (q == 0) {
+            s_args[0] = (unsigned long long)next_index;
+            s_args[1] = (unsigned long long)new_xyz;
+            s_args[2] = (unsigned long long)xyz;
+            s_args[3] = (unsigned long long)(unsigned)n;
+        }
+    }
     __syncthreads();
-    fps_rounds<kW, PPT>(m, x, y, z, t, rk2, s_first[0], s_first[1], s_first[2], idxs, prefix_out ? prefix_out + blockIdx.x : nullptr,
-                        known, xyz ? xyz + (size_t)blockIdx.x * n * 3 : nullptr, prefix_cap);
+    fps_rounds<kW, PPT>(s_key, s_rec, s_idx, m, x, y, z, t, rk2, s_first[0], s_first[1], s_first[2], idxs,
+                        prefix_out ? prefix_out + blockIdx.x : nullptr, known, xyz ? xyz + (size_t)blockIdx.x * n * 3 : nullptr,
+                        prefix_cap);
     if (temp) {
 #pragma unroll
         for (int j = 0; j < PPT; ++j) {
             const unsigned r = rank_of(rk2, j);
             if (r != 0xFFFFu) temp[unrank14(r)] = __int_as_float(t[j]);
+        }
+    }
+    if constexpr (kEpilogue) {
+        void *const next_index_ = (void *)s_args[0];
+        if (next_index_) {
+            float *const new_xyz_ = (float *)s_args[1];
+            const float *const xyz_ = (const float *)s_args[2];
+            const int n_ = (int)s_args[3];
+            __threadfence_block();
+            __syncthreads();
+            const int np2 = m <= 2048 ? 2048 : 4096;
+            float4 *const sorted2 = reinterpret_cast<float4 *>(next_index_);
+            float *const boxes2 = reinterpret_cast<float *>(sorted2 + (size_t)gridDim.x * np2);
+            float *const qboxes2 = boxes2 + (size_t)gridDim.x * (np2 / 64) * 6;
+            fps_index_epilogue<64 * kW, kIxBits, kIxPer, kIxStage>(
+                reinterpret_cast<int *>(s_lds), reinterpret_cast<float(*)[16]>(s_lds + kBoxAt), reinterpret_cast<int *>(s_lds + kPartAt),
+                m, np2, xyz_, sorted2, boxes2, qboxes2, n_, idxs - (size_t)blockIdx.x * m, new_xyz_);
         }
     }
 }
@@ -1039,9 +1090,16 @@
 
 static int fps_over_index(int b, int n, int m, const float *xyz, void *index, size_t index_bytes, float *temp, int *idx,
                           float *new_xyz, hipStream_t s, const int *skip = nullptr, int *prefix_out = nullptr,
-                          int prefix_cap = 0x7fffffff) {
+                          int prefix_cap = 0x7fffffff, void *next_index = nullptr, size_t next_index_bytes = 0) {
     const size_t need = scene_index_bytes(b, n);
     int rc;
+    if (next_index) {
+        const size_t need2 = scene_index_bytes(b, m);
+        EPNET_REQUIRE(need2 != 0 && m <= 16384 && new_xyz && xyz && idx && b <= 65535);
+        if (next_index_bytes < need2) return EPNET_ENOMEM;
+        if (((uintptr_t)next_index & 15) != 0) return EPNET_EINVAL;
+    }
+    bool built_next = false;
     const bool plain = need == 0 || !index || n <= 1024 || m <= 1 || (n > 16384 && !temp);
     int fold_init = -1;
     bool wrote_centres = false;
@@ -1073,9 +1131,12 @@
             float *tsort = scene_index_sampling_scratch(b, n, index);
             hipLaunchKernelGGL(pruned::fps_bigscene_kernel<16>, grid, dim3(1024), 0, s, n, np, m, xyz, sorted, bucket_boxes, temp, tsort, idx, skip);
         } else {
+            const bool epilogue = next_index && !skip && scene_index_np(n) == 16384 && m >= 1024 && m <= 4096;
+            void *const epi_index = epilogue ? next_index : nullptr;
 #define EPNET_FPS_INDEXED(W_, P_)                                                                                                     \
     hipLaunchKernelGGL((pruned::fps_indexed_kernel<W_, P_>), grid, dim3(64 * W_), 0, s, n, m, sorted, temp, idx, skip, prefix_out, xyz, \
-                       prefix_cap, fold_init)
+                       prefix_cap, fold_init, epi_index, new_xyz)
+            built_next = epilogue;
             switch (scene_index_np(n)) {
                 case 2048: EPNET_FPS_INDEXED(4, 8); break;
                 case 4096: EPNET_FPS_INDEXED(4, 16); break;
@@ -1086,7 +1147,14 @@
         }
         rc = check_launch("furthest_point_sampling");
     }
-    if (rc || !new_xyz || wrote_centres) return rc;
+    if (rc || built_next) return rc;
+    if (next_index) {
+        const int np2 = scene_index_np(m);
+        float4 *sorted2 = (float4 *)next_index;
+        float *boxes2 = (float *)(sorted2 + (size_t)b * np2);
+        return spatial_index_launch(b, m, np2, xyz, sorted2, boxes2, boxes2 + (size_t)b * (np2 / 64) * 6, s, n, idx, new_xyz);
+    }
+    if (!new_xyz || wrote_centres) return rc;
     if (m == 0) return EPNET_OK;
     EPNET_REQUIRE(xyz && b <= 65535);
     launch_gather_centres(b, n, m, xyz, idx, new_xyz, s);
@@ -1117,3 +1185,15 @@
     return fps_over_index(b, n, m, xyz, index, index_bytes, temp, idx, new_xyz, (hipStream_t)stream, prefix_in, prefix_out,
                           prefix_cap);
 }
+
+extern "C" int epnet_sample_centres_chain_index(int b, int n, int m, const float *xyz, void *index, size_t index_bytes,
+                                                float *temp, int *idx, float *new_xyz, const int *prefix_in, int *prefix_out,
+                                                int prefix_cap, void *next_index, size_t next_index_bytes,
+                                                epnet_stream_t stream) {
+    EPNET_REQUIRE(b >= 0 && n >= 1 && m >= 0);
+    if (b == 0 || m == 0) return EPNET_OK;
+    EPNET_REQUIRE(xyz && idx && new_xyz && next_index);
+    if (m > n) prefix_in = nullptr;
+    return fps_over_index(b, n, m, xyz, index, index_bytes, temp, idx, new_xyz, (hipStream_t)stream, prefix_in, prefix_out,
+                          prefix_cap, next_index, next_index_bytes);
+}
diff --git a/epnet_amd/csrc/spatial.h b/epnet_amd/csrc/spatial.h
--- a/epnet_amd/csrc/spatial.h
+++ b/epnet_amd/csrc/spatial.h
@@ -1,5 +1,6 @@
 #pragma once
 #include "common.h"
+#include "dpp.h"
 
 namespace epnet {
 
@@ -188,6 +189,215 @@
     return (float *)((char *)index + (size_t)b * (np * sizeof(float4) + (np / 64 + np / 256) * 6 * sizeof(float)));
 }
 
+#ifdef EPNET_IX_STATS
+#define EPNET_IX_STAMP(var) const unsigned long long var = __builtin_amdgcn_s_memtime()
+#else
+#define EPNET_IX_STAMP(var)
+#endif
+
+template <int kIxThreads, int BITS, int kIxPerThread, int kStageCap, bool kRegsOnly>
+__device__ __forceinline__ void scene_index_build_block(int *s_hist, float (*s_box)[16], int *s_part, int n, int np,
+                                                        const float *__restrict__ xyz, float4 *__restrict__ sorted,
+                                                        float *__restrict__ boxes, float *__restrict__ qboxes, int n_src,
+                                                        const int *__restrict__ src_idx, float *__restrict__ gathered,
+                                                        unsigned long long *ix_stats = nullptr) {
+    constexpr int kCells = 1 << BITS;
+    const int q = threadIdx.x, lane = q & 63, wave = q >> 6;
+    xyz += (size_t)blockIdx.x * (src_idx ? n_src : n) * 3;
+    if (src_idx) {
+        src_idx += (size_t)blockIdx.x * n;
+        gathered += (size_t)blockIdx.x * n * 3;
+    }
+    sorted += (size_t)blockIdx.x * np;
+    boxes += (size_t)blockIdx.x * (np / 64) * 6;
+    constexpr int per = kCells / kIxThreads;
+    constexpr int per_shift = per == 16 ? 4 : per == 8 ? 3 : per == 4 ? 2 : -1;
+    static_assert(per_shift > 0, "scan layout");
+    const bool in_regs = kRegsOnly || n <= kIxThreads * kIxPerThread;
+    float px[kIxPerThread], py[kIxPerThread], pz[kIxPerThread];
+    float lo[3], ext[3];
+    EPNET_IX_STAMP(t_0);
+    if (in_regs) {
+        float mn[3] = {3.4e38f, 3.4e38f, 3.4e38f}, mx[3] = {-3.4e38f, -3.4e38f, -3.4e38f};
+        int row[kIxPerThread];
+#pragma unroll
+        for (int i = 0; i < kIxPerThread; ++i) {
+            const int k = q + i * kIxThreads;
+            const int kk = k < n ? k : 0;
+            row[i] = src_idx ? src_idx[kk] : kk;
+        }
+#pragma unroll
+        for (int i = 0; i < kIxPerThread; ++i) {
+            px[i] = xyz[row[i] * 3 + 0];
+            py[i] = xyz[row[i] * 3 + 1];
+            pz[i] = xyz[row[i] * 3 + 2];
+        }
+        if (src_idx) {
+#pragma unroll
+            for (int i = 0; i < kIxPerThread; ++i) {
+                const int k = q + i * kIxThreads;
+                if (k < n) {
+                    gathered[k * 3 + 0] = px[i];
+                    gathered[k * 3 + 1] = py[i];
+                    gathered[k * 3 + 2] = pz[i];
+                }
+            }
+        }
+#pragma unroll
+        for (int i = 0; i < kIxPerThread; ++i) {
+            const bool ok = q + i * kIxThreads < n;
+            mn[0] = fminf(mn[0], ok ? px[i] : 3.4e38f); mx[0] = fmaxf(mx[0], ok ? px[i] : -3.4e38f);
+            mn[1] = fminf(mn[1], ok ? py[i] : 3.4e38f); mx[1] = fmaxf(mx[1], ok ? py[i] : -3.4e38f);
+            mn[2] = fminf(mn[2], ok ? pz[i] : 3.4e38f); mx[2] = fmaxf(mx[2], ok ? pz[i] : -3.4e38f);
+        }
+#pragma unroll
+        for (int a = 0; a < 3; ++a) {
+            const float l = wave_minf_all(mn[a]), h = wave_maxf_all(mx[a]);
+            if (lane == 0) {
+                s_box[a][wave] = l;
+                s_box[3 + a][wave] = h;
+            }
+        }
+        __syncthreads();
+#pragma unroll
+        for (int a = 0; a < 3; ++a) {
+            float l = s_box[a][0], h = s_box[3 + a][0];
+            for (int w = 1; w < kIxThreads / 64; ++w) {
+                l = fminf(l, s_box[a][w]);
+                h = fmaxf(h, s_box[3 + a][w]);
+            }
+            lo[a] = l;
+            ext[a] = h - l;
+        }
+    } else {
+        block_bbox3(xyz, n, s_box, lo, ext);
+    }
+    const CellGrid g = make_cell_grid(lo, ext, BITS);
+    EPNET_IX_STAMP(t_1);
+    for (int i = q; i < kCells + kCells / per + 64; i += kIxThreads) s_hist[i] = 0;
+    __syncthreads();
+    EPNET_IX_STAMP(t_2);
+    int code[kIxPerThread], rank[kIxPerThread];
+    if (in_regs) {
+#pragma unroll
+        for (int i = 0; i < kIxPerThread; ++i) code[i] = hist_at((int)cell_code(g, px[i], py[i], pz[i]), per_shift);
+#pragma unroll
+        for (int i = 0; i < kIxPerThread; ++i)
+            rank[i] = atomicAdd(&s_hist[q + i * kIxThreads < n ? code[i] : kCells + kCells / per + lane], 1);
+    } else {
+        for (int k = q; k < n; k += kIxThreads)
+            atomicAdd(&s_hist[hist_at((int)cell_code(g, xyz[k * 3 + 0], xyz[k * 3 + 1], xyz[k * 3 + 2]), per_shift)], 1);
+    }
+    __syncthreads();
+    EPNET_IX_STAMP(t_3);
+    int sum = 0;
+    for (int i = 0; i < per; ++i) sum += s_hist[hist_at(q * per + i, per_shift)];
+    const int incl = wave_inclusive_scan(sum);
+    if (lane == 63) s_part[wave] = incl;
+    __syncthreads();
+    int base = incl - sum;
+    for (int w = 0; w < wave; ++w) base += s_part[w];
+    for (int i = 0; i < per; ++i) {
+        const int at = hist_at(q * per + i, per_shift);
+        const int c = s_hist[at];
+        s_hist[at] = base;
+        base += c;
+    }
+    __syncthreads();
+    EPNET_IX_STAMP(t_4);
+    auto bucket_box = [&](int p, const float4 v) {
+        const bool real = p < n;
+        const float cx_ = canonical(v.x), cy_ = canonical(v.y), cz_ = canonical(v.z);
+        float mnx = real ? cx_ : 3.4e38f, mxx = real ? cx_ : -3.4e38f, mny = real ? cy_ : 3.4e38f, mxy = real ? cy_ : -3.4e38f,
+              mnz = real ? cz_ : 3.4e38f, mxz = real ? cz_ : -3.4e38f;
+        wave_box(mnx, mxx, mny, mxy, mnz, mxz);
+        if (lane == 0) {
+            float *bx = boxes + (p >> 6) * 6;
+            const bool any = mnx <= mxx;
+            bx[0] = any ? mnx : 3.0e38f; bx[1] = any ? mxx : 3.0e38f;
+            bx[2] = any ? mny : 3.0e38f; bx[3] = any ? mxy : 3.0e38f;
+            bx[4] = any ? mnz : 3.0e38f; bx[5] = any ? mxz : 3.0e38f;
+        }
+    };
+    const bool staged = kRegsOnly || (in_regs && (np & 255) == 0);
+    if (staged) {
+        float4 *s_stage = reinterpret_cast<float4 *>(s_hist + kCells + kCells / per + 64);
+        int pos[kIxPerThread];
+#pragma unroll
+        for (int i = 0; i < kIxPerThread; ++i) pos[i] = s_hist[code[i]] + rank[i];
+        const int quarter = kStageCap ? min(np >> 2, kStageCap) : np >> 2;
+        for (int h = 0; h * quarter < np; ++h) {
+            const int base = h * quarter, len = min(quarter, np - base);
+            for (int p = q; p < len; p += kIxThreads)
+                if (base + p >= n) s_stage[p] = make_float4(3.0e38f, 3.0e38f, 3.0e38f, __int_as_float(-1));
+#pragma unroll
+            for (int i = 0; i < kIxPerThread; ++i) {
+                const int k = q + i * kIxThreads;
+                if (k < n && (unsigned)(pos[i] - base) < (unsigned)quarter)
+                    s_stage[pos[i] - base] = make_float4(px[i], py[i], pz[i], __int_as_float(k));
+            }
+            __syncthreads();
+            for (int p = q; p < len; p += kIxThreads) {
+                const float4 v = s_stage[p];
+                sorted[base + p] = v;
+                bucket_box(base + p, v);
+            }
+            __syncthreads();
+        }
+    } else {
+        if (in_regs) {
+#pragma unroll
+            for (int i = 0; i < kIxPerThread; ++i) {
+                const int k = q + i * kIxThreads;
+                if (k < n) sorted[s_hist[code[i]] + rank[i]] = make_float4(px[i], py[i], pz[i], __int_as_float(k));
+            }
+        } else {
+            for (int k = q; k < n; k += kIxThreads) {
+                const float x = xyz[k * 3 + 0], y = xyz[k * 3 + 1], z = xyz[k * 3 + 2];
+                const int pos = atomicAdd(&s_hist[hist_at((int)cell_code(g, x, y, z), per_shift)], 1);
+                sorted[pos] = make_float4(x, y, z, __int_as_float(k));
+            }
+        }
+        for (int p = n + q; p < np; p += kIxThreads)
+            sorted[p] = make_float4(3.0e38f, 3.0e38f, 3.0e38f, __int_as_float(-1));
+        __threadfence_block();
+        __syncthreads();
+        for (int p = q; p < np; p += kIxThreads) bucket_box(p, sorted[p]);
+    }
+#ifdef EPNET_IX_STATS
+    {
+        EPNET_IX_STAMP(t_6);
+        if (q == 0 && ix_stats) {
+            atomicAdd(&ix_stats[0], t_1 - t_0); atomicAdd(&ix_stats[1], t_2 - t_1); atomicAdd(&ix_stats[2], t_3 - t_2);
+            atomicAdd(&ix_stats[3], t_4 - t_3); atomicAdd(&ix_stats[4], t_6 - t_4);
+            atomicAdd(&ix_stats[7], 1ull);
+        }
+    }
+#endif
+    if (!qboxes) return;
+    qboxes += (size_t)blockIdx.x * (np / 256) * 6;
+    __threadfence_block();
+    __syncthreads();
+    for (int g = q; g < np / 256; g += kIxThreads) {
+        float mn[3] = {3.4e38f, 3.4e38f, 3.4e38f}, mx[3] = {-3.4e38f, -3.4e38f, -3.4e38f};
+        for (int k = 0; k < 4; ++k) {
+            const float *bx = boxes + (g * 4 + k) * 6;
+            if (bx[0] < 3.0e38f)
+#pragma unroll
+                for (int a = 0; a < 3; ++a) {
+                    mn[a] = fminf(mn[a], bx[2 * a]);
+                    mx[a] = fmaxf(mx[a], bx[2 * a + 1]);
+                }
+        }
+        const bool any = mn[0] <= mx[0];
+#pragma unroll
+        for (int a = 0; a < 3; ++a) {
+            qboxes[g * 6 + 2 * a] = any ? mn[a] : 3.0e38f;
+            qboxes[g * 6 + 2 * a + 1] = any ? mx[a] : 3.0e38f;
+        }
+    }
+}
+
 int spatial_index_launch(int b, int n, int np, const float *xyz, float4 *sorted, float *boxes, float *qboxes, hipStream_t s,
                          int n_src = 0, const int *src_idx = nullptr, float *gathered = nullptr);
 
diff --git a/epnet_amd/pointnet2_cuda.py b/epnet_amd/pointnet2_cuda.py
--- a/epnet_amd/pointnet2_cuda.py
+++ b/epnet_amd/pointnet2_cuda.py
@@ -231,6 +231,28 @@
                 need(prefix_out, b, "prefix_out")
             _lib.check(_lib.lib().epnet_sample_centres_chain(b, n, m, pp, px, nb, pt, pi, pn, pin, pout, int(prefix_cap), s),
                        "sample_centres")
+    return 1
+
+
+@writes("idx", "new_xyz", "prefix_out", "next_index")
+def sample_centres_index_wrapper(b, n, m, points, index, idx, new_xyz, next_index, prefix_in=None, prefix_out=None, prefix_cap=0):
+    pp, pi, pn = dev_ptr(points, "points", _F), dev_ptr(idx, "idx", _I), dev_ptr(new_xyz, "new_xyz", _F)
+    need(points, b * n * 3, "points"); need(idx, b * m, "idx"); need(new_xyz, b * m * 3, "new_xyz")
+    px, nb = _index_args(index, points)
+    nx, nnb = _index_args(next_index, points)
+    if nx is None:
+        raise RuntimeError("sample_centres_index_wrapper needs the next level's index buffer")
+    pin = dev_ptr(prefix_in, "prefix_in", _I) if prefix_in is not None else None
+    pout = dev_ptr(prefix_out, "prefix_out", _I) if prefix_out is not None else None
+    if prefix_in is not None:
+        need(prefix_in, b, "prefix_in")
+    if prefix_out is not None:
+        need(prefix_out, b, "prefix_out")
+    temp = None if 64 <= n <= 16384 else torch.full((b, n), 1e10, dtype=_F, device=points.device)
+    pt = None if temp is None else temp.data_ptr()
+    with on_device_of(points) as s:
+        _lib.check(_lib.lib().epnet_sample_centres_chain_index(b, n, m, pp, px, nb, pt, pi, pn, pin, pout, int(prefix_cap), nx, nnb, s),
+                   "sample_centres_index")
     return 1
 
 
diff --git a/epnet_amd/sa_stack.py b/epnet_amd/sa_stack.py
--- a/epnet_amd/sa_stack.py
+++ b/epnet_amd/sa_stack.py
@@ -73,14 +73,15 @@
         elif env_q == 2 or (env_q == 1 and with_fp):
             chosen = every
         elif env_q == 1 and batch * n >= 240 * 16384:
-            chosen = every - {0}
+            chosen = every - {0, 1}
         else:
             chosen = frozenset()
         self.s_query_levels = chosen & every
         self.queries_in_s = self.s_query_levels == every
         self.chain = bool(int(os.environ.get("EPNET_SA_CHAIN", "1"))) and fused_sampling
-        self.fuse_gather = bool(int(os.environ.get("EPNET_SA_FUSE_GATHER", "1")))
+        self.fuse_gather = int(os.environ.get("EPNET_SA_FUSE_GATHER", "1"))
         self._deferred = None
+        self._next_built = None
         self.s_first = bool(int(os.environ.get("EPNET_SA_S_FIRST", "0" if self.s_query_levels else "1")))
         self.tail_scales = int(os.environ.get("EPNET_SA_TAIL_SCALES", "0"))
         self.multi_query = bool(int(os.environ.get("EPNET_SA_MULTI_QUERY", "1")))
@@ -185,10 +186,13 @@
         P = L["sets"][parity]
         lvl = self.levels.index(L)
         pending, self._deferred = self._deferred, None
+        built, self._next_built = self._next_built, None
         if pending is not None and pending[1:] == (lvl - 1, parity):
             src_xyz, _, _ = pending
             prev = self.levels[lvl - 1]
             ext.scene_index_build_gathered_wrapper(b, prev["n"], n, src_xyz, prev["fps_idx_sets"][parity], cur_xyz, P["index"])
+        elif built == (lvl, parity):
+            pass
         elif P["index"] is not None and not index_built:
             ext.scene_index_build_wrapper(b, n, cur_xyz, P["index"])
         if self.fused_sampling:
@@ -200,10 +204,15 @@
                 nxt_L = self.levels[lvl + 1] if lvl + 1 < len(self.levels) else None
                 defer = (defer_ok and self.fuse_gather and self.fused and nxt_L is not None
                          and nxt_L["sets"][parity]["index"] is not None and 1024 <= m <= 16384)
-                ext.sample_centres_wrapper(b, n, m, cur_xyz, P["index"], L["fps_idx_sets"][parity], None if defer else P["new_xyz"],
-                                           prefix_in, P["prefix"], nxt)
-                if defer:
-                    self._deferred = (cur_xyz, lvl, parity)
+                if defer and self.fuse_gather == 1:
+                    ext.sample_centres_index_wrapper(b, n, m, cur_xyz, P["index"], L["fps_idx_sets"][parity], P["new_xyz"],
+                                                     nxt_L["sets"][parity]["index"], prefix_in, P["prefix"], nxt)
+                    self._next_built = (lvl + 1, parity)
+                else:
+                    ext.sample_centres_wrapper(b, n, m, cur_xyz, P["index"], L["fps_idx_sets"][parity], None if defer else P["new_xyz"],
+                                               prefix_in, P["prefix"], nxt)
+                    if defer:
+                        self._deferred = (cur_xyz, lvl, parity)
             else:
                 ext.sample_centres_wrapper(b, n, m, cur_xyz, P["index"], L["fps_idx_sets"][parity], P["new_xyz"])
         else:
@@ -361,10 +370,11 @@
         ext.scene_index_build_wrapper(self.batch, first["n"], clouds[p], first["sets"][p]["index"])
         forked = torch.cuda.Event()
         forked.record(main)
-        self._deferred = None
+        self._deferred = self._next_built = None
         self._sample_level(first, clouds[p], p, index_built=True, defer_ok=True)
         s1_deferred = self._deferred is not None
-        self._deferred = None
+        s1_built = self._next_built is not None
+        self._deferred = self._next_built = None
         side.wait_event(forked)
         with torch.cuda.stream(side):
             inputs = [clouds[r]] + [L["sets"][r]["new_xyz"] for L in self.levels[:-1]]
@@ -381,10 +391,11 @@
         third.wait_event(forked)
         with torch.cuda.stream(third):
             self._deferred = (clouds[q], 0, q) if s1_deferred else None
+            self._next_built = (1, q) if s1_built else None
             cur = first["sets"][q]["new_xyz"]
             for L in self.levels[1:]:
                 cur = self._sample_level(L, cur, q, defer_ok=True)
-            self._deferred = None
+            self._deferred = self._next_built = None
             if self.with_fp:
                 self._search_fp(clouds[q], q)
             self._queries_of(clouds[q], q)
@@ -433,10 +444,10 @@
     def _prime(self, clouds):
         for parity in range(self.ring):
             xyz = cur = clouds[parity]
-            self._deferred = None
+            self._deferred = self._next_built = None
             for L in self.levels:
                 cur = self._sample_level(L, cur, parity, defer_ok=True)
-            self._deferred = None
+            self._deferred = self._next_built = None
             if self.with_fp:
                 self._search_fp(xyz, parity)
             if self.s_query_levels:
diff --git a/include/epnet_ops.h b/include/epnet_ops.h
--- a/include/epnet_ops.h
+++ b/include/epnet_ops.h
@@ -143,6 +143,9 @@
 int epnet_sample_centres_chain(int b, int n, int m, const float *xyz, void *index, size_t index_bytes, float *temp,
                                int *idx, float *new_xyz, const int *prefix_in, int *prefix_out, int prefix_cap,
                                epnet_stream_t stream);
+int epnet_sample_centres_chain_index(int b, int n, int m, const float *xyz, void *index, size_t index_bytes, float *temp,
+                                     int *idx, float *new_xyz, const int *prefix_in, int *prefix_out, int prefix_cap,
+                                     void *next_index, size_t next_index_bytes, epnet_stream_t stream);
 int epnet_three_nn_indexed(int b, int n, int m, const float *unknown, const float *known, const void *unknown_index,
                            size_t unknown_index_bytes, const void *known_index, size_t known_index_bytes, float *dist2,
                            int *idx, epnet_stream_t stream);
```

New measurement: 1.478 billion points/s (median of 6 runs). +1.5%, better.
